# vLAR-group/unMORE

Measured on AMD Instinct MI355X. Metric: images/sec (train fwd+bwd) ObjectnessNet ViT-B/16 384x384, higher is better.
Workload: dtype bf16

## Files before the change

### include/umr.h

```cpp
#ifndef UMR_H
#define UMR_H
#include <stdint.h>

#ifdef __cplusplus
extern "C" {
#endif

typedef void* umr_stream_t;

enum umr_status { UMR_OK = 0, UMR_ERR_INVALID = -1, UMR_ERR_UNSUPPORTED = -2, UMR_ERR_HIP = -1000 };
enum umr_dtype { UMR_F32 = 0, UMR_BF16 = 1, UMR_BF16X3 = 2 };

int umr_version(void);
const char* umr_last_error_string(void);

enum umr_f32_mode { UMR_F32_EXACT = 0, UMR_F32_X3 = 1, UMR_F32_X3_FAST = 2 };
int umr_set_f32_mode(int mode);
int umr_get_f32_mode(void);

int umr_set_cu_budget(int cus);
int umr_get_cu_budget(void);

int umr_set_debug_option(const char* name, const char* value);
int umr_get_debug_option(const char* name, int* value, int* is_set);

enum umr_epi_flags {
    UMR_EPI_BIAS = 1, UMR_EPI_ADD_AUX = 2, UMR_EPI_MASK_RELU = 4, UMR_EPI_MASK_DGELU = 8,
    UMR_EPI_ADD_AUX2 = 16, UMR_EPI_OUT_F32 = 32, UMR_EPI_ROWBIAS = 64,
    UMR_EPI_OUT_X3 = 128,
    UMR_EPI_AUX_X3 = 256, UMR_EPI_AUX2_X3 = 512, UMR_EPI_C2_X3 = 1024
};
enum umr_act { UMR_ACT_NONE = 0, UMR_ACT_RELU = 1, UMR_ACT_GELU = 2, UMR_ACT_TANH = 3, UMR_ACT_SIGMOID = 5  };

typedef struct umr_gemm_desc {
    const void* A;
    const void* B;
    void* C;
    void* C2;
    const float* bias;
    const void* aux;
    const void* aux2;
    const float* rowbias;
    int64_t lda, ldb, ldc, ldc2, ldaux, ldaux2;
    int32_t M, N, K;
    int32_t dtype;
    int32_t flags, act, c2_mode, rows_per_batch;
    int32_t conv;
    int32_t nb, H, W, Cin, Ho, Wo;
    int32_t a_rows_in, a_rows_out, a_row_off;
    int32_t c_rows_in, c_rows_out, c_row_off;
    int32_t aux_mod;
    const float* red_w;
    float* red_out;
    int32_t red_c;
    int32_t no_store;
} umr_gemm_desc;

int umr_gemm_nt(const umr_gemm_desc* d, umr_stream_t stream);
int64_t umr_gemm_nt_workspace(void);
int umr_gemm_nt_splits(const umr_gemm_desc* d, int64_t workspace_bytes);
int64_t umr_gemm_nt_x3_workspace(const umr_gemm_desc* d);
int umr_gemm_nt_ws(const umr_gemm_desc* d, void* workspace, int64_t workspace_bytes, umr_stream_t stream);
int umr_gemm_nt_ws_status(void* workspace, umr_stream_t stream, int* bad_tickets);
int umr_split3(const float* src, void* dst, int64_t rows, int K, int64_t ld_src, int64_t ld_dst, umr_stream_t stream);
int umr_unsplit3(const void* src, float* dst, int64_t rows, int K, int64_t ld_src, int64_t ld_dst, umr_stream_t stream);
int umr_split3_rows(const float* src, void* dst, int64_t rows, int K, int64_t ld_src, int64_t ld_dst, int rows_in, int rows_out,
                    int row_off, umr_stream_t stream);
int umr_gemm_nt_rowreduce_ok(const umr_gemm_desc* d);

typedef struct umr_gemm_tn_desc {
    const void* dY;
    const void* X;
    float* dW;
    float* dbias;
    void* workspace;
    int64_t workspace_bytes;
    int64_t lddy, ldx, lddw;
    int32_t M, N, K;
    int32_t dtype;
    int32_t accumulate;
    int32_t conv, nb, H, W, Cin, Ho, Wo;
    int32_t dy_rows_in, dy_rows_out, dy_row_off;
    int32_t x_rows_in, x_rows_out, x_row_off;
} umr_gemm_tn_desc;

int64_t umr_gemm_tn_workspace(const umr_gemm_tn_desc* d);
int umr_gemm_tn(const umr_gemm_tn_desc* d, umr_stream_t stream);

int umr_layernorm_fwd(const void* x, const float* gamma, const float* beta, void* y, float* mean, float* rstd,
                      int M, int D, float eps, int dtype, umr_stream_t stream);
int64_t umr_layernorm_bwd_workspace(int M, int D);
int umr_layernorm_bwd(const void* dy, const void* x, const float* gamma, const float* mean, const float* rstd,
                      const void* dres, void* dx, float* dgamma, float* dbeta, int accumulate, void* workspace,
                      int64_t workspace_bytes, int M, int D, int dtype, umr_stream_t stream);
int umr_layernorm_bwd_rows(const void* dy, const void* x, const float* gamma, const float* mean, const float* rstd,
                           const void* dres, void* dx, void* workspace, int64_t workspace_bytes, int M, int D, int dtype,
                           umr_stream_t stream);
int umr_layernorm_bwd_params(const void* workspace, int64_t workspace_bytes, float* dgamma, float* dbeta, int accumulate,
                             int M, int D, umr_stream_t stream);

int64_t umr_attention_bwd_workspace(int B, int N, int heads);
int umr_attention_fwd(const void* qkv, void* out, float* lse, int B, int N, int heads, int head_dim, int dtype,
                      umr_stream_t stream);
int umr_attention_bwd(const void* qkv, const void* out, const void* dout, const float* lse, float* dsum_ws, void* dqkv,
                      int B, int N, int heads, int head_dim, int dtype, umr_stream_t stream);

int umr_patchify(const float* images, void* out, int B, int H, int W, int patch, int ldk, int dtype, umr_stream_t stream);
int umr_bilinear_fwd(const void* x, void* y, int B, int Hi, int Wi, int Ho, int Wo, int C, int align_corners, int dtype, umr_stream_t stream);
int umr_bilinear_bwd(const void* dy, void* dx, int B, int Hi, int Wi, int Ho, int Wo, int C, int align_corners, int dtype, umr_stream_t stream);
#define UMR_BILINEAR_RELU 1
#define UMR_BILINEAR_OUT_X3 2
int umr_bilinear_fwd_ex(const void* x, int64_t ldx, void* y, int64_t ldy, int B, int Hi, int Wi, int Ho, int Wo, int C, int align_corners,
                        int flags, int dtype, umr_stream_t stream);
int umr_bilinear_bwd_ex(const void* dy, int64_t lddy, void* dx, int64_t lddx, int B, int Hi, int Wi, int Ho, int Wo, int C,
                        int align_corners, int dtype, umr_stream_t stream);
int umr_pixel_shuffle(const void* src, void* dst, int B, int H, int W, int s, int C, int inverse, int dtype, umr_stream_t stream);
int umr_zero_stuff2(const void* dy, void* out, int B, int H, int W, int Ho, int Wo, int C, int dtype, umr_stream_t stream);
int umr_permute4(const void* src, void* dst, const int32_t* dst_dims, const int64_t* src_strides, int64_t src_offset,
                 int dtype_in, int dtype_out, int accumulate, umr_stream_t stream);
typedef struct umr_perm_entry {
    const void* src; void* dst; int32_t d[4]; int64_t sstride[4]; int64_t soff; int32_t dtype_in, dtype_out; int64_t blk_start;
    int32_t e[4]; int32_t ord[4];
    int64_t rowlen;
} umr_perm_entry;
int umr_permute4_batched(const umr_perm_entry* table_dev, int n, int64_t total_blocks, const int32_t* blk_entry_dev, umr_stream_t stream);
int umr_segsum(const void* x, void* out, int R, int reps, int64_t rep_stride, int64_t seg_stride, int C, int dtype_in,
               int out_f32, int accumulate, umr_stream_t stream);
int umr_fill_cls(void* tokens, const float* cls, const float* pos0, int B, int64_t batch_stride, int D, int dtype, umr_stream_t stream);
int umr_cast(const void* src, void* dst, int64_t n, float scale, int dtype_in, int dtype_out, umr_stream_t stream);
int umr_scale_by_device_scalar(const float* src, const float* scalar, float* dst, int64_t n, umr_stream_t stream);

int umr_head_out_fwd(const void* h, const float* w, const float* bias, float* out, int64_t M, int K, int Cout, int HW, int act,
                     int dtype, umr_stream_t stream);
int umr_head_out_finish(const float* partials, int nparts, const float* bias, float* out, int64_t M, int Cout, int HW, int act,
                        umr_stream_t stream);
int64_t umr_head_out_bwd_workspace(int64_t M, int K);
int umr_head_out_bwd(const void* h, const float* w, const float* dout, const float* yout, void* dh, float* dw, float* db,
                     void* workspace, int64_t workspace_bytes, int64_t M, int K, int Cout, int HW, int act, int relu_mask,
                     int dtype, umr_stream_t stream);

int64_t umr_loss_workspace(void);
int umr_objectness_loss(const float* pred_center, const float* pred_sdf, const float* gt_center, const float* gt_sdf,
                        const float* gt_saliency, float* d_center, float* d_sdf, float* out5, void* workspace, int B, int H,
                        int W, int center_l2, int sdf_l2, int use_grad, int use_bce, float grad_scale, umr_stream_t stream);

int umr_adam_step(float* p, const float* g, float* m, float* v, int64_t n, float lr, float beta1, float beta2, float eps,
                  int step, float grad_scale, umr_stream_t stream);
int umr_adam_set_hyper(float* hyper7_dev, float lr, float beta1, float beta2, float eps, int step, float grad_scale, umr_stream_t stream);
int umr_adam_step_hyper(float* p, const float* g, float* m, float* v, int64_t n, const float* hyper7_dev, umr_stream_t stream);
typedef struct umr_adam_pack_entry {
    float* p; const float* g; float* m; float* v; void* dst_lin; void* dst_t; int64_t n; int32_t N, K; int64_t blk_start;
} umr_adam_pack_entry;
int umr_adam_pack_step(const umr_adam_pack_entry* table_dev, int n_entries, int64_t total_blocks, const int32_t* blk_entry_dev,
                       const float* hyper7_dev, umr_stream_t stream);

int umr_crop_resize_bilinear(const float* image, const int32_t* boxes, float* out, int N, int H, int W, int S, umr_stream_t stream);
int umr_center_peaks(const float* sdf_maps, const float* center_fields, const double* filter50, double* score_out,
                     double* max_values, int64_t* argmax, int B, int H, int W, int border, int erode_kernel, int erode_rounds,
                     umr_stream_t stream);
int umr_center_peaks_certified(const float* sdf_maps, const float* center_fields, const double* filter50, double* max_values,
                               int64_t* argmax, int32_t* certified, int B, int H, int W, int border, int erode_kernel, int erode_rounds,
                               float eps, double singular_threshold, umr_stream_t stream);
int umr_boundary_deltas(const float* sdf_maps, float* deltas, int B, int H, int W, umr_stream_t stream);
int umr_mask_paste_stats(const float* sdf_maps, const float* center_fields, const int32_t* boxes, int N, int S, int H, int W,
                         int32_t* stats, float* maxima, umr_stream_t stream);
int umr_mask_paste(const float* sdf_maps, const float* center_fields, const int32_t* boxes, const int64_t* select, int K, int S, int H, int W,
                   uint8_t* masks, umr_stream_t stream);
int umr_rle_encode(const uint8_t* masks, int K, int H, int W, int64_t* sizes, const int64_t* offsets, uint8_t* chars, int64_t chars_capacity,
                   umr_stream_t stream);
int umr_mask_paste_rle(const float* sdf_maps, const float* center_fields, const int32_t* boxes, const int64_t* select, int K, int S, int H, int W,
                       int64_t* sizes, const int64_t* offsets, uint8_t* chars, int64_t chars_capacity, umr_stream_t stream);
int64_t umr_rle_decode_workspace(int K, int64_t total_chars, int64_t total_segments, int mode);
int umr_rle_decode(const uint8_t* chars, const int64_t* char_offsets, int K, int64_t total_chars, const int64_t* out_desc,
                   const int32_t* group_start, const int64_t* seg_offsets, int G, int64_t max_pixels, int64_t total_segments, uint8_t* out,
                   int64_t out_bytes, int value, int mode, int32_t* status, int32_t* info, void* workspace, int64_t workspace_bytes,
                   umr_stream_t stream);
int64_t umr_poly_rle_workspace(int64_t n_vertices, int n_polygons, int n_annotations, int64_t crossing_capacity);
int umr_poly_rle(const double* xy, const int64_t* poly_offsets, const int64_t* ann_polys, const int64_t* ann_sizes,
                 const int64_t* cross_offsets, int64_t n_vertices, int n_polygons, int n_annotations, int64_t crossing_capacity, int phases,
                 int64_t* sizes, const int64_t* offsets, uint8_t* chars, int64_t chars_capacity, void* workspace, int64_t workspace_bytes,
                 umr_stream_t stream);
int64_t umr_mask_iou_workspace(int K, int64_t total_chars, int64_t total_words);
int umr_mask_iou(const uint8_t* chars, const int64_t* char_offsets, int K, int64_t total_chars, const int64_t* unit_size,
                 const int32_t* unit_start, const int32_t* unit_nd, const int64_t* pair_offsets, const int64_t* word_offsets,
                 const uint8_t* crowd, int U, int64_t max_pixels, int max_d, int max_g, int64_t total_pairs, int64_t total_words,
                 int32_t* inter, double* iou, int32_t* area, int32_t* status, void* workspace, int64_t workspace_bytes,
                 umr_stream_t stream);
int umr_box_iou(const double* boxes, const int32_t* unit_start, const int32_t* unit_nd, const int64_t* pair_offsets, const uint8_t* crowd,
                int U, int K, int64_t max_pairs, int64_t total_pairs, double* iou, umr_stream_t stream);
int umr_coco_match(const double* iou, const int64_t* pair_offsets, int64_t total_pairs, const int32_t* unit_nd, const int32_t* unit_ng,
                   const int64_t* det_offsets, int64_t total_dets, const int64_t* gt_offsets, int64_t total_gts, const double* dt_area,
                   const double* gt_area, const uint8_t* gt_crowd, const double* area_rng, int A, const double* thr, int T, int max_det,
                   int U, uint8_t* dt_matched, int32_t* dt_gt, uint8_t* dt_ignore, uint8_t* gt_ignore, uint8_t* gt_matched,
                   umr_stream_t stream);
int umr_mask_components(const float* sdf_maps, const float* center_fields, int B, int S, int max_components, int32_t* counts, int32_t* boxes,
                        umr_stream_t stream);
int64_t umr_nms_workspace(int n);
int umr_nms(const float* boxes, const int64_t* order, int n, float iou_threshold, void* workspace, int64_t workspace_bytes,
            int64_t* keep, int32_t* n_keep, umr_stream_t stream);

int umr_linear_head_fwd(const void* x, const float* kw, const float* tapbias10, float* out, int B, int H, int W, int C, int act,
                        int dtype, umr_stream_t stream);
int umr_linear_head_bwd_data(const float* dout, const float* yout, const float* kw, void* dx, int B, int H, int W, int C, int act,
                             int accumulate, int dtype, umr_stream_t stream);
int64_t umr_linear_head_bwd_weight_workspace(int64_t M, int C);
int umr_linear_head_bwd_weight(const void* x, const float* dout, const float* yout, float* out, void* workspace,
                               int64_t workspace_bytes, int B, int H, int W, int C, int act, int dtype, umr_stream_t stream);
int64_t umr_linear_head_shift9_workspace(int64_t M);
int umr_linear_head_shift9(const float* dout, const float* yout, void* s9, float* nd, void* workspace, int64_t workspace_bytes,
                           int B, int H, int W, int act, int dtype, umr_stream_t stream);
int umr_linear_head_gather9(const float* taps, int64_t ldt, const float* tapbias10, float* out, int B, int H, int W, int act,
                            umr_stream_t stream);
int umr_small_gemm_f32(const float* A, const float* B, float* C, int M, int N, int K, int64_t sa_m, int64_t sa_k, int64_t sb_k,
                       int64_t sb_n, int64_t sc_m, int64_t sc_n, int accumulate, umr_stream_t stream);

int umr_im2col_nchw(const float* images, void* out, int B, int C, int H, int W, int KH, int KW, int stride, int pad, int ldk,
                    int dtype, umr_stream_t stream);
int umr_maxpool3x3s2(const void* x, void* y, int B, int H, int W, int C, int dtype, umr_stream_t stream);
int umr_bn_fold(const float* w, const float* gamma, const float* beta, const float* mean, const float* var, float eps, void* w_out,
                float* b_out, int Co, int K, int ldk, int dtype, umr_stream_t stream);

// ... 200 lines not shown
```

### unmore_amd/_lib.py

```python
import ctypes
import os
import re
import subprocess

_HERE = os.path.dirname(os.path.abspath(__file__))
HEADER = os.path.join(_HERE, "..", "include", "umr.h")
LIB_PATH = os.environ.get("UMR_LIB") or os.path.join(_HERE, "lib", "libumr.so")
CSRC = os.path.join(_HERE, "csrc")

F32, BF16, BF16X3 = 0, 1, 2
EPI_BIAS, EPI_ADD_AUX, EPI_MASK_RELU, EPI_MASK_DGELU, EPI_ADD_AUX2, EPI_OUT_F32, EPI_ROWBIAS, EPI_OUT_X3 = 1, 2, 4, 8, 16, 32, 64, 128
EPI_AUX_X3, EPI_AUX2_X3, EPI_C2_X3 = 256, 512, 1024
ACT_NONE, ACT_RELU, ACT_GELU, ACT_TANH = 0, 1, 2, 3
ACT_SIGMOID = 5
F32_EXACT, F32_X3, F32_X3_FAST = 0, 1, 2

_vp, _i32, _i64 = ctypes.c_void_p, ctypes.c_int32, ctypes.c_int64


class GemmDesc(ctypes.Structure):
    _fields_ = [("A", _vp), ("B", _vp), ("C", _vp), ("C2", _vp), ("bias", _vp), ("aux", _vp),
                ("aux2", _vp), ("rowbias", _vp),
                ("lda", _i64), ("ldb", _i64), ("ldc", _i64), ("ldc2", _i64), ("ldaux", _i64), ("ldaux2", _i64),
                ("M", _i32), ("N", _i32), ("K", _i32), ("dtype", _i32),
                ("flags", _i32), ("act", _i32), ("c2_mode", _i32), ("rows_per_batch", _i32),
                ("conv", _i32), ("nb", _i32), ("H", _i32), ("W", _i32), ("Cin", _i32), ("Ho", _i32), ("Wo", _i32),
                ("a_rows_in", _i32), ("a_rows_out", _i32), ("a_row_off", _i32),
                ("c_rows_in", _i32), ("c_rows_out", _i32), ("c_row_off", _i32), ("aux_mod", _i32),
                ("red_w", _vp), ("red_out", _vp), ("red_c", _i32), ("no_store", _i32)]


class GemmTnDesc(ctypes.Structure):
    _fields_ = [("dY", _vp), ("X", _vp), ("dW", _vp), ("dbias", _vp), ("workspace", _vp),
                ("workspace_bytes", _i64), ("lddy", _i64), ("ldx", _i64), ("lddw", _i64),
                ("M", _i32), ("N", _i32), ("K", _i32), ("dtype", _i32), ("accumulate", _i32),
                ("conv", _i32), ("nb", _i32), ("H", _i32), ("W", _i32), ("Cin", _i32), ("Ho", _i32), ("Wo", _i32),
                ("dy_rows_in", _i32), ("dy_rows_out", _i32), ("dy_row_off", _i32),
                ("x_rows_in", _i32), ("x_rows_out", _i32), ("x_row_off", _i32)]


class AdamPackEntry(ctypes.Structure):
    _fields_ = [("p", _vp), ("g", _vp), ("m", _vp), ("v", _vp), ("dst_lin", _vp), ("dst_t", _vp), ("n", _i64), ("N", _i32), ("K", _i32),
                ("blk_start", _i64)]


class BnBwdDesc(ctypes.Structure):
    _fields_ = [("dy", _vp), ("dpool", _vp), ("y", _vp), ("z", _vp * 2), ("mean", _vp * 2), ("rstd", _vp * 2), ("gamma", _vp * 2),
                ("dgamma", _vp * 2), ("dbeta", _vp * 2), ("dz", _vp * 2), ("g_out", _vp), ("workspace", _vp), ("workspace_bytes", _i64),
                ("rows_per_batch", _i64), ("pool_scale", ctypes.c_float), ("M", _i32), ("C", _i32), ("nbranch", _i32), ("dtype", _i32)]


class RaggedSrc(ctypes.Structure):
    _fields_ = [("f32", _vp), ("u8", _vp), ("H", _i32), ("W", _i32)]


class CpPair(ctypes.Structure):
    _fields_ = [("l_image", _vp), ("l_masks", _vp), ("l_boxes", _vp), ("u_image", _vp), ("u_masks", _vp), ("out_image", _vp), ("out_masks", _vp),
                ("word_off", _i64), ("inter_off", _i64), ("row_off", _i64), ("choice_off", _i64),
                ("Hl", _i32), ("Wl", _i32), ("Nl", _i32), ("Hu", _i32), ("Wu", _i32), ("Nu", _i32), ("nc", _i32), ("h_new", _i32), ("w_new", _i32),
                ("h_shift", _i32), ("w_shift", _i32), ("rh", ctypes.c_float), ("rw", ctypes.c_float), ("sx", ctypes.c_float), ("sy", ctypes.c_float),
                ("reserved", _i32)]


class MlImage(ctypes.Structure):
    _fields_ = [("masks", _vp), ("boxes", _vp), ("index", _vp), ("H", _i32), ("W", _i32), ("G", _i32), ("first", _i32), ("R", _i32),
                ("index64", _i32)]


class BlImage(ctypes.Structure):
    _fields_ = [("boxes", _vp), ("gt_boxes", _vp), ("gt_classes", _vp), ("gt_scores", _vp), ("first", _i32), ("R", _i32), ("G", _i32),
                ("chunk_first", _i32), ("height", ctypes.c_float), ("width", ctypes.c_float)]


class DpImage(ctypes.Structure):
    _fields_ = [("boxes", _vp), ("scores", _vp), ("mat_first", _i64), ("R", _i32), ("cand_first", _i32), ("out_first", _i32), ("cap", _i32),
                ("height", ctypes.c_float), ("width", ctypes.c_float)]


class PermEntry(ctypes.Structure):
    _fields_ = [("src", _vp), ("dst", _vp), ("d", _i32 * 4), ("sstride", _i64 * 4), ("soff", _i64), ("dtype_in", _i32), ("dtype_out", _i32),
                ("blk_start", _i64), ("e", _i32 * 4), ("ord", _i32 * 4), ("rowlen", _i64)]


MIRRORS = {"umr_gemm_desc": GemmDesc, "umr_gemm_tn_desc": GemmTnDesc, "umr_adam_pack_entry": AdamPackEntry, "umr_bn_bwd_desc": BnBwdDesc,
           "umr_ragged_src": RaggedSrc, "umr_cp_pair": CpPair, "umr_ml_image": MlImage, "umr_bl_image": BlImage, "umr_dp_image": DpImage,
           "umr_perm_entry": PermEntry}


def build(verbose=False, jobs=8):
    r = subprocess.run(["make", "-C", CSRC, f"-j{jobs}"], capture_output=True, text=True)
    if verbose or r.returncode != 0:
        print(r.stdout[-4000:])
        print(r.stderr[-8000:])
    if r.returncode != 0:
        raise RuntimeError("building libumr.so failed")
    return LIB_PATH


_lib = None
_count = [0]

_ARG = {"int": _i32, "int32_t": _i32, "int64_t": _i64, "float": ctypes.c_float, "double": ctypes.c_double, "umr_stream_t": _vp,
        "const char*": ctypes.c_char_p, "int*": ctypes.POINTER(ctypes.c_int)}
_RET = {"int": None, "int64_t": _i64, "const char*": ctypes.c_char_p}


def _ctype(decl, table, proto):
    c = re.sub(r"\s*\*\s*", "*", " ".join(decl.split()))
    if c not in table and not (table is _ARG and c.endswith("*")):
        raise RuntimeError(f"{HEADER}: no ctypes type for '{c}' in '{' '.join(proto.split())}'")
    return table.get(c, _vp)


def _read_header():
    if not os.path.exists(HEADER):
        raise RuntimeError(f"{HEADER} is missing: the ctypes binding of libumr.so is read from it")
    text = re.sub(r"/\*.*?\*/", " ", open(HEADER).read(), flags=re.S)
    text = re.sub(r"^[ \t]*#.*$", "", text, flags=re.M)
    text = re.sub(r"typedef\s+struct\s+\w+\s*\{.*?\}\s*\w+\s*;", "", text, flags=re.S)
    args, rets = {}, {}
    for proto in text.split(";"):
        if "(" not in proto:
            continue
        m = re.fullmatch(r"\s*(.*?)\b(umr_\w+)\s*\(([^()]*)\)\s*", proto, flags=re.S)
        if m is None:
            raise RuntimeError(f"{HEADER}: not a prototype this binding can read: '{' '.join(proto.split())}'")
        ret, name, params = m.groups()
        params = [] if params.strip() in ("", "void") else params.split(",")
        args[name] = [_ctype(re.sub(r"\w+\s*$", "", p), _ARG, proto) for p in params]
        rets[name] = _ctype(ret, _RET, proto)
    return args, {name: r for name, r in rets.items() if r is not None}


ARGTYPES, RESTYPES = _read_header()


def exported_symbols():
    return sorted(ARGTYPES)


def lib():
    global _lib
    if _lib is None:
        if not os.path.exists(LIB_PATH):
            raise RuntimeError(
                f"{LIB_PATH} is missing: build it with `python -c 'import __graft_entry__ as g; g.build()'` "
                "(the product has no CPU fallback)")
        _lib = ctypes.CDLL(LIB_PATH)
        for name, argtypes in ARGTYPES.items():
            fn = getattr(_lib, name)
            fn.argtypes = argtypes
            if name in RESTYPES:
                fn.restype = RESTYPES[name]
    return _lib


def check(status, what):
    _count[0] += 1
    if status != 0:
        raise RuntimeError(f"{what} failed with status {status}: {lib().umr_last_error_string().decode()}")
```

### unmore_amd/csrc/gemm_nt.hip

```cpp
#include "umr_common.h"
#include <type_traits>
#include "gemm_epilogue.h"
#include <stdlib.h>

namespace {

constexpr int BM = 128, BN = 128;
constexpr int UMR_SPLITK_COUNTERS = 4096;
constexpr int ROWB = 128;
constexpr int TILE_BYTES = BM * ROWB;
constexpr int STAGE_BYTES = 2 * TILE_BYTES;
constexpr int LDS_BYTES = 2 * STAGE_BYTES;

template <typename T> struct Tr;
template <> struct Tr<bf16_t> { static constexpr int EPC = 8, BK = 64; };
template <> struct Tr<float> { static constexpr int EPC = 4, BK = 32; };


template <typename T> struct Raw8;
template <> struct Raw8<bf16_t> {
    typedef bf16x8 type;
    static __device__ __forceinline__ type load(const bf16_t* q) { return *(const bf16x8*)q; }
    static __device__ __forceinline__ void cvt(type t, f32x4& a, f32x4& b) {
        a = f32x4{(float)t[0], (float)t[1], (float)t[2], (float)t[3]};
// ... 259 lines not shown
            const int old = __hip_atomic_fetch_add(counters + tile_id, 1, __ATOMIC_RELAXED, __HIP_MEMORY_SCOPE_AGENT);
            const bool bad = old < 0 || old >= splits;
            if (bad) {
                __hip_atomic_fetch_add(counters + (UMR_SPLITK_COUNTERS - 1), 1, __ATOMIC_RELAXED, __HIP_MEMORY_SCOPE_AGENT);
                __hip_atomic_store(counters + tile_id, 0, __ATOMIC_RELAXED, __HIP_MEMORY_SCOPE_AGENT);
            }
            if (fenced) {
                __builtin_amdgcn_fence(__ATOMIC_ACQUIRE, "agent");
                asm volatile("s_waitcnt vmcnt(0)" ::: "memory");
            } else {
                __builtin_amdgcn_fence(__ATOMIC_ACQUIRE, "workgroup");
            }
            const int last = !bad && old == splits - 1;
            if (last) __hip_atomic_store(counters + tile_id, 0, __ATOMIC_RELAXED, __HIP_MEMORY_SCOPE_AGENT);
            *(int*)smem = last;
        }
        __syncthreads();
        if (*(const int*)smem == 0) return;
        const unsigned long long* base = slabs + (int64_t)tile_id * splits * SLAB + tid * 2;
        auto ld4 = [&](const unsigned long long* q) {
            const f32x2 lo = __builtin_bit_cast(f32x2, __hip_atomic_load(q, __ATOMIC_RELAXED, __HIP_MEMORY_SCOPE_AGENT));
            const f32x2 hi = __builtin_bit_cast(f32x2, __hip_atomic_load(q + 1, __ATOMIC_RELAXED, __HIP_MEMORY_SCOPE_AGENT));
            return f32x4{lo[0], lo[1], hi[0], hi[1]};
        };
#pragma unroll
        for (int r = 0; r < 16; ++r) acc[r >> 2][r & 3] = ld4(base + r * 512);
        for (int q = 1; q < splits; ++q) {
            const unsigned long long* bq = base + (int64_t)q * SLAB;
            f32x4 v[16];
#pragma unroll
            for (int r = 0; r < 16; ++r) v[r] = ld4(bq + r * 512);
#pragma unroll
            for (int r = 0; r < 16; ++r) acc[r >> 2][r & 3] += v[r];
        }
    }

    constexpr int EP_LD = 132;
    float* stg = (float*)smem;
    auto stage_pass = [&](auto ptag) {
        constexpr int PASS = decltype(ptag)::value;
#pragma unroll
        for (int mh = 0; mh < 2; ++mh) {
            const int lr = wr * 32 + mh * 16 + frow;
#pragma unroll
            for (int ntl = 0; ntl < 4; ++ntl)
                *(f32x4*)(stg + lr * EP_LD + wc * 64 + ntl * 16 + fq * 4) = acc[PASS * 2 + mh][ntl];
        }
    };
    if constexpr (EPI == 0) {
        const int c8 = (tid & 15) * 8, n = n0 + c8;
        const bool n_ok = n < p.N;
        const bool use_aux = (p.flags & (UMR_EPI_ADD_AUX | UMR_EPI_MASK_RELU | UMR_EPI_MASK_DGELU)) != 0;
        const bool use_aux2 = (p.flags & UMR_EPI_ADD_AUX2) != 0;
        f32x4 bias0 = {0.f, 0.f, 0.f, 0.f}, bias1 = {0.f, 0.f, 0.f, 0.f};
        if ((p.flags & UMR_EPI_BIAS) && n_ok) { bias0 = *(const f32x4*)(p.bias + n); bias1 = *(const f32x4*)(p.bias + n + 4); }
        typename Raw8<T>::type ra[8], rb2[8];
        auto row_of = [&](int pass, int k) { const int lr = (tid >> 4) + k * 16; return m0 + (lr >> 5) * 64 + pass * 32 + (lr & 31); };
        auto prefetch = [&](auto ptag) {
            constexpr int PASS = decltype(ptag)::value;
#pragma unroll
            for (int k = 0; k < 4; ++k) {
                const int m = row_of(PASS, k);
                if (m < p.M && n_ok) {
                    if (use_aux) ra[PASS * 4 + k] = Raw8<T>::load((const T*)p.aux + (int64_t)m * p.ldaux + n);
                    if (use_aux2) rb2[PASS * 4 + k] = Raw8<T>::load((const T*)p.aux2 + (int64_t)m * p.ldaux2 + n);
                }
            }
        };
        auto pass = [&](auto ptag) {
            constexpr int PASS = decltype(ptag)::value;
            __syncthreads();
            stage_pass(ptag);
            __syncthreads();
#pragma unroll
            for (int k = 0; k < 4; ++k) {
                const int lr = (tid >> 4) + k * 16;
                const int m = row_of(PASS, k);
                if (m >= p.M || !n_ok) continue;
                f32x4 v0 = *(const f32x4*)(stg + lr * EP_LD + c8), v1 = *(const f32x4*)(stg + lr * EP_LD + c8 + 4);
                v0 += bias0; v1 += bias1;
                if (use_aux) {
                    f32x4 a0, a1;
                    Raw8<T>::cvt(ra[PASS * 4 + k], a0, a1);
                    if (p.flags & UMR_EPI_ADD_AUX) { v0 += a0; v1 += a1; }
                    else if (p.flags & UMR_EPI_MASK_RELU) {
#pragma unroll
                        for (int e = 0; e < 4; ++e) { v0[e] = a0[e] > 0.f ? v0[e] : 0.f; v1[e] = a1[e] > 0.f ? v1[e] : 0.f; }
                    } else if constexpr (sizeof(T) == 2) {
#pragma unroll
                        for (int e = 0; e < 4; ++e) { v0[e] *= dgelu_sel<T>(a0[e]); v1[e] *= dgelu_sel<T>(a1[e]); }
                    }
                }
                if (use_aux2) {
                    f32x4 a0, a1;
                    Raw8<T>::cvt(rb2[PASS * 4 + k], a0, a1);
                    v0 += a0; v1 += a1;
                }
                if (p.c2_mode == 2) Vec8<T>::store((T*)p.C2 + (int64_t)m * p.ldc2 + n, v0, v1);
                if (p.act == UMR_ACT_RELU) {
#pragma unroll
                    for (int e = 0; e < 4; ++e) { v0[e] = fmaxf(v0[e], 0.f); v1[e] = fmaxf(v1[e], 0.f); }
                } else if (p.act == UMR_ACT_GELU) {
                    if constexpr (sizeof(T) == 2) {
#pragma unroll
                        for (int e = 0; e < 4; ++e) { v0[e] = gelu_sel<T>(v0[e]); v1[e] = gelu_sel<T>(v1[e]); }
                    }
                }
                Vec8<T>::store((T*)p.C + (int64_t)m * p.ldc + n, v0, v1);
                if (p.c2_mode == 1) {
#pragma unroll
                    for (int e = 0; e < 4; ++e) { v0[e] = fmaxf(v0[e], 0.f); v1[e] = fmaxf(v1[e], 0.f); }
                    Vec8<T>::store((T*)p.C2 + (int64_t)m * p.ldc2 + n, v0, v1);
                }
            }
        };
        prefetch(std::integral_constant<int, 0>{});
        if constexpr (sizeof(T) == 2) prefetch(std::integral_constant<int, 1>{});
        pass(std::integral_constant<int, 0>{});
        if constexpr (sizeof(T) != 2) prefetch(std::integral_constant<int, 1>{});
        pass(std::integral_constant<int, 1>{});
    } else {
        const bool vec_ok = ((p.N & 7) == 0) && ((p.ldc & 7) == 0) && ((p.ldc2 & 7) == 0) && ((p.ldaux & 7) == 0) &&
                            ((p.ldaux2 & 7) == 0);
#pragma unroll 1
        for (int pass = 0; pass < 2; ++pass) {
            __syncthreads();
            if (pass == 0) stage_pass(std::integral_constant<int, 0>{});
            else stage_pass(std::integral_constant<int, 1>{});
            __syncthreads();
#pragma unroll 1
            for (int task = tid; task < 64 * 16; task += 256) {
                const int lr = task >> 4, c8 = (task & 15) * 8;
                const int trow = (lr >> 5) * 64 + pass * 32 + (lr & 31);
                const int m = m0 + trow, n = n0 + c8;
                if (m >= p.M || n >= p.N) continue;
                const f32x4 v0 = *(const f32x4*)(stg + lr * EP_LD + c8), v1 = *(const f32x4*)(stg + lr * EP_LD + c8 + 4);
                if (vec_ok) {
                    epilogue_store8<T>(p, m, n, v0, v1);
                } else {
                    epilogue_store<T>(p, m, n, v0);
                    if (n + 4 < p.N) epilogue_store<T>(p, m, n + 4, v1);
                }
            }
        }
    }
}

}

int umr_launch_gemm_nt256(const umr_gemm_desc* d, hipStream_t s);
int umr_launch_gemm_nt256p(const umr_gemm_desc* d, hipStream_t s);
int umr_launch_gemm_nt256p_ws(const umr_gemm_desc* d, void* ws, int64_t ws_bytes, hipStream_t s);
bool umr_nt256_rowreduce_path(const umr_gemm_desc* d);

static int tile_override() {
    return umr_opt_or(UMR_OPT_GEMM_TILE, 0);
}

static bool uses_256(const umr_gemm_desc* d) {
    if (d->dtype != UMR_BF16) return false;
    const int64_t t256 = (int64_t)((d->M + 255) / 256) * ((d->N + 255) / 256);
    const int ov = tile_override();
    const bool kfit = d->conv == 0 ? (d->K % 64 == 0) : (d->Cin % 64 == 0);
    constexpr int min_tiles = 300;
    constexpr int conv_min_tiles = 512;
    const bool big = kfit && d->N >= 192 &&
                     (t256 >= 2048 || (d->conv == 1 && t256 >= conv_min_tiles) || (d->conv == 0 && d->a_rows_in <= 0 && t256 >= min_tiles && (d->K >= 512 || t256 >= 1024)));
    return kfit && (ov == 256 || (ov == 0 && big));
}

extern "C" int umr_gemm_nt_rowreduce_ok(const umr_gemm_desc* d) {
    if (d == nullptr || d->M <= 0 || d->N <= 0 || d->K <= 0) return 0;
    return (uses_256(d) && umr_nt256_rowreduce_path(d)) ? 1 : 0;
}

static int gemm_nt_impl(const umr_gemm_desc* d, void* workspace, int64_t workspace_bytes, umr_stream_t stream);

extern "C" int umr_gemm_nt(const umr_gemm_desc* d, umr_stream_t stream) { return gemm_nt_impl(d, nullptr, 0, stream); }

extern "C" int umr_gemm_nt_ws_status(void* workspace, umr_stream_t stream, int* bad_tickets) {
    UMR_CHECK_ARG(workspace != nullptr && bad_tickets != nullptr, "gemm_nt_ws_status: null argument");
    hipStream_t s = (hipStream_t)stream;
    int* word = (int*)workspace + (UMR_SPLITK_COUNTERS - 1);
    int v = 0;
    hipError_t e_ = hipMemcpyAsync(&v, word, sizeof(int), hipMemcpyDeviceToHost, s);
    if (e_ == hipSuccess) e_ = hipStreamSynchronize(s);
    if (e_ == hipSuccess && v != 0) e_ = hipMemsetAsync(word, 0, sizeof(int), s);
    if (e_ != hipSuccess) return umr_set_error(UMR_ERR_HIP - (int)e_, hipGetErrorString(e_));
    *bad_tickets = v;
    return UMR_OK;
}

extern "C" int64_t umr_gemm_nt_workspace(void) { return (int64_t)UMR_SPLITK_COUNTERS * 4 + (int64_t)512 * BM * BN * 4; }

static int pick_splits(const umr_gemm_desc* d, int64_t tiles, bool have_ws);
static bool uses_256(const umr_gemm_desc* d);
int umr_x3_ksplit_of(const umr_gemm_desc* d, int64_t ws_bytes);

extern "C" int umr_gemm_nt_splits(const umr_gemm_desc* d, int64_t workspace_bytes) {
    if (d == nullptr || d->M <= 0 || d->N <= 0 || d->K <= 0 || workspace_bytes <= 0) return 1;
    if (d->dtype == UMR_BF16X3) return umr_x3_ksplit_of(d, workspace_bytes - (int64_t)UMR_SPLITK_COUNTERS * 4);
    if (d->dtype != UMR_BF16 && d->dtype != UMR_F32) return 1;
    if (uses_256(d)) return 1;
    return pick_splits(d, (int64_t)((d->M + BM - 1) / BM) * ((d->N + BN - 1) / BN), true);
}

extern "C" int umr_gemm_nt_ws(const umr_gemm_desc* d, void* workspace, int64_t workspace_bytes, umr_stream_t stream) {
    UMR_CHECK_ARG(workspace == nullptr || (workspace_bytes >= umr_gemm_nt_workspace() && ((uintptr_t)workspace & 15) == 0),
                  "gemm_nt_ws: workspace smaller than umr_gemm_nt_workspace() or not 16-byte aligned");
    return gemm_nt_impl(d, workspace, workspace_bytes, stream);
}

static int pick_splits(const umr_gemm_desc* d, int64_t tiles, bool have_ws) {
    if (!have_ws || tiles > UMR_SPLITK_COUNTERS) return 1;
    const int bk = d->dtype == UMR_BF16 ? 64 : 32;
    const int nt = d->conv == 0 ? (d->K + bk - 1) / bk : 9 * ((d->Cin + bk - 1) / bk);
    int want;
    const int forced = umr_opt(UMR_OPT_NT_SPLITK);
    if (forced != UMR_OPT_UNSET) {
        want = forced;
    } else {
        if (tiles > 170) return 1;
        if (d->dtype == UMR_BF16) {
            want = tiles <= 32 ? (nt / 8 < 4 ? nt / 8 : 4) : (nt >= 32 ? 2 : 1);
        } else {
            want = (int)(448 / tiles);
            const int per_min = tiles <= 32 ? 8 : 16;
            if (want > nt / per_min) want = nt / per_min;
            if (want > 8) want = 8;
        }
    }
    if (want > nt) want = nt;
    if (want < 2 || tiles * want > 512) return 1;
    const int per = (nt + want - 1) / want;
    return (nt + per - 1) / per;
}

template <typename T, int CV, int EPI, bool X3>
static void launch_nt(dim3 g, hipStream_t s, const umr_gemm_desc* d, int tiles_n, int splits, float* skws) {
    const int splits_arg = (splits > 1 && umr_opt_or(UMR_OPT_SPLITK_FENCE, 0) != 0) ? -splits : splits;
    hipLaunchKernelGGL((gemm_nt_kernel<T, CV, EPI, X3>), g, dim3(256), LDS_BYTES, s, *d, tiles_n, splits_arg, skws);
}

static int gemm_nt_impl(const umr_gemm_desc* d, void* workspace, int64_t workspace_bytes, umr_stream_t stream) {
    UMR_CHECK_ARG(d != nullptr, "gemm_nt: null descriptor");
    UMR_CHECK_ARG(d->A && d->B && (d->C || d->no_store), "gemm_nt: null operand");
    UMR_CHECK_ARG(d->M > 0 && d->N > 0 && d->K > 0, "gemm_nt: empty problem");
    if (d->dtype == UMR_BF16X3) {
        UMR_CHECK_ARG(d->conv == 0 || d->conv == 1, "gemm_nt (BF16X3): plain GEMM or stride-1 3x3 conv only");
        const int fl = d->flags;
        const bool out_f32 = (fl & UMR_EPI_OUT_F32) != 0, out_x3 = (fl & UMR_EPI_OUT_X3) != 0;
        const int kk = d->conv == 0 ? d->K : d->Cin;
        const bool red = d->red_w != nullptr;
        const int n_aux = ((fl & UMR_EPI_ADD_AUX) != 0) + ((fl & UMR_EPI_MASK_RELU) != 0) + ((fl & UMR_EPI_MASK_DGELU) != 0);
        auto ld_ok = [&](int64_t ld, bool planes) { return planes ? (ld % 8 == 0 && ld >= 3 * (int64_t)d->N) : (ld % 4 == 0 && ld >= d->N); };
        bool ok = (kk % 64 == 0) && (d->N % 8 == 0) && d->a_rows_in <= 0 && (d->ldb % 8 == 0) && (d->ldb >= 3 * (int64_t)d->K) &&
                  (d->act == UMR_ACT_NONE || d->act == UMR_ACT_RELU || d->act == UMR_ACT_GELU) && n_aux <= 1 &&
                  (!(fl & UMR_EPI_MASK_DGELU) || (d->act == UMR_ACT_NONE && d->c2_mode == 0 && !(fl & UMR_EPI_ADD_AUX2))) &&
                  (d->conv == 1 ? (d->K == 9 * d->Cin && (int64_t)d->nb * d->Ho * d->Wo == d->M && d->Ho == d->H && d->Wo == d->W && d->c_rows_in <= 0)
                                : (d->lda % 8 == 0 && d->lda >= 3 * (int64_t)d->K));
        if (red) {
            ok = ok && d->no_store && !out_f32 && !out_x3 && d->conv == 0 && d->red_out && (d->red_c == 1 || d->red_c == 2) && d->c2_mode == 0 &&
                 !(fl & ~UMR_EPI_BIAS) && d->act != UMR_ACT_GELU && d->c_rows_in <= 0 && d->aux_mod <= 0;
        } else {
            ok = ok && !d->no_store && d->C && (out_f32 != out_x3) && ld_ok(d->ldc, out_x3) &&
                 (d->c2_mode == 0 || ((d->c2_mode == 1 || d->c2_mode == 2) && d->C2 && ld_ok(d->ldc2, (fl & UMR_EPI_C2_X3) != 0))) &&
                 (n_aux == 0 || (d->aux && ld_ok(d->ldaux, (fl & UMR_EPI_AUX_X3) != 0))) &&
                 (!(fl & UMR_EPI_ADD_AUX2) || (d->aux2 && ld_ok(d->ldaux2, (fl & UMR_EPI_AUX2_X3) != 0))) &&
                 (!(fl & UMR_EPI_ROWBIAS) || (d->rowbias && d->rows_per_batch > 0)) && (d->aux_mod <= 0 || n_aux == 1);
        }
        if (!ok) return umr_set_error(UMR_ERR_UNSUPPORTED, "gemm_nt (BF16X3): needs K (conv: Cin) % 64 == 0, N % 8 == 0, no A-row remap, act in {none, ReLU, GELU}, "
                                                           "exactly one of OUT_F32 / OUT_X3 (or red_w with no_store and a bias / ReLU epilogue), strides that "
                                                           "fit the operand formats (include/umr.h)");
        UMR_CHECK_ARG(!(fl & UMR_EPI_BIAS) || d->bias, "gemm_nt: bias flag without pointer");
        UMR_CHECK_ARG((int64_t)((d->M + 191) / 192) * ((d->N + 255) / 256) * 32 < (1ll << 31), "gemm_nt: grid too large");
        char* xws = workspace ? (char*)workspace + (int64_t)UMR_SPLITK_COUNTERS * 4 : nullptr;
        const int64_t xws_bytes = workspace ? workspace_bytes - (int64_t)UMR_SPLITK_COUNTERS * 4 : 0;
        return umr_launch_gemm_nt256p_ws(d, xws, xws_bytes, (hipStream_t)stream);
    }
    UMR_CHECK_ARG(d->dtype == UMR_F32 || d->dtype == UMR_BF16, "gemm_nt: dtype");
    const int epc = d->dtype == UMR_BF16 ? 8 : 4;
    UMR_CHECK_ARG(d->conv >= 0 && d->conv <= 2, "gemm_nt: conv mode");
    if (d->conv == 0) {
        UMR_CHECK_ARG(d->K % epc == 0 && d->lda % epc == 0 && d->ldb % epc == 0, "gemm_nt: K/lda/ldb must be multiples of 16 bytes");
    } else {
        UMR_CHECK_ARG(d->Cin % epc == 0 && d->K == 9 * d->Cin && d->ldb % epc == 0, "gemm_nt: conv needs Cin % 16B == 0 and K == 9*Cin");
        UMR_CHECK_ARG((int64_t)d->nb * d->Ho * d->Wo == d->M, "gemm_nt: conv M != nb*Ho*Wo");
        const int s = d->conv == 2 ? 2 : 1;
        UMR_CHECK_ARG(d->Ho == (d->H - 1) / s + 1 && d->Wo == (d->W - 1) / s + 1, "gemm_nt: conv output size");
    }
    UMR_CHECK_ARG(!(d->flags & UMR_EPI_BIAS) || d->bias, "gemm_nt: bias flag without pointer");
    UMR_CHECK_ARG(!(d->flags & (UMR_EPI_ADD_AUX | UMR_EPI_MASK_RELU | UMR_EPI_MASK_DGELU)) || d->aux, "gemm_nt: aux flag without pointer");
    UMR_CHECK_ARG(!(d->flags & UMR_EPI_ADD_AUX2) || d->aux2, "gemm_nt: aux2 flag without pointer");
    UMR_CHECK_ARG(!(d->flags & UMR_EPI_ROWBIAS) || (d->rowbias && d->rows_per_batch > 0), "gemm_nt: rowbias");
    UMR_CHECK_ARG(d->c2_mode == 0 || d->C2, "gemm_nt: c2_mode without C2");
    const int tiles_m = (d->M + BM - 1) / BM, tiles_n = (d->N + BN - 1) / BN;
    int tiles_n_arg = tiles_n;
    const int64_t grid = (int64_t)tiles_m * tiles_n;
    UMR_CHECK_ARG(grid < (1ll << 31), "gemm_nt: grid too large");
    hipStream_t s = (hipStream_t)stream;
    if (d->red_w || d->no_store) {
        UMR_CHECK_ARG(umr_gemm_nt_rowreduce_ok(d) == 1, "gemm_nt: fused row reduction / no_store requested on a path that does not implement it (umr_gemm_nt_rowreduce_ok)");
        UMR_CHECK_ARG(!d->red_w || (d->red_out && (d->red_c == 1 || d->red_c == 2)), "gemm_nt: red_out / red_c");
    }
    if (uses_256(d)) return umr_launch_gemm_nt256(d, s);
    const int splits = pick_splits(d, grid, workspace != nullptr);
    float* skws = (float*)workspace;
    {
        const int oe = umr_opt(UMR_OPT_NT_ORDER);
        const bool mfast = oe != UMR_OPT_UNSET ? (oe == 'm') : (d->conv == 0 && d->a_rows_in <= 0 && (int64_t)d->N > (int64_t)d->M);
        if (mfast) tiles_n_arg = -tiles_m;
    }
    dim3 g((unsigned)(grid * splits)), b(256);
    const bool fast_ep = ((d->N & 7) == 0) && ((d->ldc & 7) == 0) && (d->c2_mode == 0 || (d->ldc2 & 7) == 0) &&
                         (!(d->flags & (UMR_EPI_ADD_AUX | UMR_EPI_MASK_RELU | UMR_EPI_MASK_DGELU)) || (d->ldaux & 7) == 0) &&
                         (!(d->flags & UMR_EPI_ADD_AUX2) || (d->ldaux2 & 7) == 0) && d->c_rows_in <= 0 && d->aux_mod <= 0 &&
                         !(d->flags & (UMR_EPI_ROWBIAS | UMR_EPI_OUT_F32)) &&
                         (!(d->flags & UMR_EPI_MASK_DGELU) || d->dtype == UMR_BF16) &&
                         (d->act == UMR_ACT_NONE || d->act == UMR_ACT_RELU || (d->act == UMR_ACT_GELU && d->dtype == UMR_BF16));
#define LAUNCH(T, CV)                                                                   \
    do {                                                                                \
        if (fast_ep) launch_nt<T, CV, 0, false>(g, s, d, tiles_n_arg, splits, skws);  \
        else launch_nt<T, CV, 1, false>(g, s, d, tiles_n_arg, splits, skws);          \
    } while (0)
#define LAUNCH_X3(CV)                                                                      \
    do {                                                                                   \
        if (fast_ep) launch_nt<float, CV, 0, true>(g, s, d, tiles_n_arg, splits, skws);  \
        else launch_nt<float, CV, 1, true>(g, s, d, tiles_n_arg, splits, skws);          \
    } while (0)
    const int f32_x3 = umr_f32_mode_now() != UMR_F32_EXACT;
    if (d->dtype == UMR_BF16) {
        if (d->conv == 0) LAUNCH(bf16_t, 0); else if (d->conv == 1) LAUNCH(bf16_t, 1); else LAUNCH(bf16_t, 2);
    } else if (f32_x3 && !((d->conv == 0 ? d->K : d->Cin) % 32)) {
        if (d->conv == 0) LAUNCH_X3(0); else if (d->conv == 1) LAUNCH_X3(1); else LAUNCH_X3(2);
    } else {
        if (d->conv == 0) LAUNCH(float, 0); else if (d->conv == 1) LAUNCH(float, 1); else LAUNCH(float, 2);
    }
#undef LAUNCH_X3
#undef LAUNCH
    {
        const hipError_t e_ = hipGetLastError();
        if (e_ != hipSuccess) {
            if (splits > 1) (void)hipMemsetAsync(workspace, 0, (size_t)UMR_SPLITK_COUNTERS * 4, s);
            return umr_set_error(UMR_ERR_HIP - (int)e_, hipGetErrorString(e_));
        }
    }
    return UMR_OK;
}
```

### unmore_amd/csrc/gemm_nt256.hip

```cpp
#include "umr_common.h"
#include "gemm_epilogue.h"
#include <stdlib.h>
#include <type_traits>

namespace {

constexpr int BM2 = 256, BN2 = 256, BK2 = 64;
constexpr int ROWB2 = 128;
constexpr int TILE2 = 256 * ROWB2;
constexpr int BUF2 = 2 * TILE2;
constexpr int LDS2 = 2 * BUF2;

typedef bf16_t T2;

template <int CONV>
__global__ __launch_bounds__(512, 2) void gemm_nt256_kernel(const umr_gemm_desc p, int tiles_n) {
    extern __shared__ __attribute__((aligned(16))) char smem[];
    constexpr int SZ = 2;
    constexpr unsigned OOB = 0x80000000u;
    const int tid = threadIdx.x, lane = tid & 63;
    const int w = __builtin_amdgcn_readfirstlane(tid >> 6);

    int bid = blockIdx.x;
    {
// ... 102 lines not shown
    auto stage_issue = [&](auto gtag, auto itag) {
        constexpr int G = decltype(gtag)::value, I = decltype(itag)::value;
        unsigned v = (G == 0) ? a_eff[0][I] : (G == 3) ? a_eff[1][I] : vo[G][I];
        if (st_tile >= nt) v = OOB;
        char* dst = smem + (st_tile & 1) * BUF2;
        if (G == 0 || G == 3) __builtin_amdgcn_raw_ptr_buffer_load_lds(rsA, UMR_LDS_PTR(dst + lds_row[G][I] * ROWB2), 16, v, soffA, 0, 0);
        else __builtin_amdgcn_raw_ptr_buffer_load_lds(rsB, UMR_LDS_PTR(dst + TILE2 + lds_row[G][I] * ROWB2), 16, v, soffB, 0, 0);
        if (G == 3 && I == 1) ++st_tile;
    };
#define STAGE_DMA(G, I) stage_issue(std::integral_constant<int, G>{}, std::integral_constant<int, I>{})

    f32x4 acc[8][4];
#pragma unroll
    for (int i = 0; i < 8; ++i)
#pragma unroll
        for (int j = 0; j < 4; ++j) acc[i][j] = f32x4{0.f, 0.f, 0.f, 0.f};

    const int wr = w >> 2, wc = w & 3;
    const int frow = lane & 15, fq = lane >> 4;
    int a_ad[2], b_ad[2];
#pragma unroll
    for (int ks = 0; ks < 2; ++ks) {
        const int q = ks * 4 + fq;
        const int sw = (frow >> 1) & 7;
        a_ad[ks] = (wr * 128 + frow) * ROWB2 + ((q ^ sw) << 4);
        b_ad[ks] = TILE2 + (wc * 64 + frow) * ROWB2 + ((q ^ sw) << 4);
    }
#define A_FRAG(ks, i) (*(const bf16x8*)(sbuf + a_ad[ks] + (i) * 16 * ROWB2))
#define B_FRAG(ks, i) (*(const bf16x8*)(sbuf + b_ad[ks] + (i) * 16 * ROWB2))

    bf16x8 fa[2][4], fb0[2][2], fb1[2][2];

#define PHASE_SYNC()                                               \
    asm volatile("s_waitcnt vmcnt(6)" ::: "memory");               \
    __builtin_amdgcn_s_barrier();                                  \
    asm volatile("s_waitcnt lgkmcnt(0)" ::: "memory");             \
    __builtin_amdgcn_sched_barrier(0);
#define MFMA(ACC, BF, AF) ACC = __builtin_amdgcn_mfma_f32_16x16x32_bf16(BF, AF, ACC, 0, 0, 0)
#define QUADRANT(M0, N0, FB, G)                                                                     \
    __builtin_amdgcn_s_setprio(1);                                                                  \
    MFMA(acc[M0 + 0][N0 + 0], FB[0][0], fa[0][0]); MFMA(acc[M0 + 0][N0 + 1], FB[0][1], fa[0][0]);   \
    MFMA(acc[M0 + 1][N0 + 0], FB[0][0], fa[0][1]); MFMA(acc[M0 + 1][N0 + 1], FB[0][1], fa[0][1]);   \
    __builtin_amdgcn_sched_barrier(0);                                                              \
    STAGE_DMA(G, 0);                                                                                \
    __builtin_amdgcn_sched_barrier(0);                                                              \
    MFMA(acc[M0 + 2][N0 + 0], FB[0][0], fa[0][2]); MFMA(acc[M0 + 2][N0 + 1], FB[0][1], fa[0][2]);   \
    MFMA(acc[M0 + 3][N0 + 0], FB[0][0], fa[0][3]); MFMA(acc[M0 + 3][N0 + 1], FB[0][1], fa[0][3]);   \
    MFMA(acc[M0 + 0][N0 + 0], FB[1][0], fa[1][0]); MFMA(acc[M0 + 0][N0 + 1], FB[1][1], fa[1][0]);   \
    __builtin_amdgcn_sched_barrier(0);                                                              \
    STAGE_DMA(G, 1);                                                                                \
    __builtin_amdgcn_sched_barrier(0);                                                              \
    MFMA(acc[M0 + 1][N0 + 0], FB[1][0], fa[1][1]); MFMA(acc[M0 + 1][N0 + 1], FB[1][1], fa[1][1]);   \
    MFMA(acc[M0 + 2][N0 + 0], FB[1][0], fa[1][2]); MFMA(acc[M0 + 2][N0 + 1], FB[1][1], fa[1][2]);   \
    MFMA(acc[M0 + 3][N0 + 0], FB[1][0], fa[1][3]); MFMA(acc[M0 + 3][N0 + 1], FB[1][1], fa[1][3]);   \
    __builtin_amdgcn_s_setprio(0);

    auto tile_body = [&](const char* sbuf) {
#pragma unroll
        for (int ks = 0; ks < 2; ++ks) {
#pragma unroll
            for (int i = 0; i < 2; ++i) fb0[ks][i] = B_FRAG(ks, i);
#pragma unroll
            for (int i = 0; i < 4; ++i) fa[ks][i] = A_FRAG(ks, i);
        }
        PHASE_SYNC();
        QUADRANT(0, 0, fb0, 2)
#pragma unroll
        for (int ks = 0; ks < 2; ++ks)
#pragma unroll
            for (int i = 0; i < 2; ++i) fb1[ks][i] = B_FRAG(ks, 2 + i);
        PHASE_SYNC();
        QUADRANT(0, 2, fb1, 3)
        stage_prep();
#pragma unroll
        for (int ks = 0; ks < 2; ++ks)
#pragma unroll
            for (int i = 0; i < 4; ++i) fa[ks][i] = A_FRAG(ks, 4 + i);
        PHASE_SYNC();
        QUADRANT(4, 2, fb1, 0)
        PHASE_SYNC();
        QUADRANT(4, 0, fb0, 1)
    };

    stage_prep();
    STAGE_DMA(0, 0); STAGE_DMA(0, 1); STAGE_DMA(1, 0); STAGE_DMA(1, 1);
    STAGE_DMA(2, 0); STAGE_DMA(2, 1); STAGE_DMA(3, 0); STAGE_DMA(3, 1);
    stage_prep();
    STAGE_DMA(0, 0); STAGE_DMA(0, 1); STAGE_DMA(1, 0); STAGE_DMA(1, 1);
    asm volatile("s_waitcnt vmcnt(8)" ::: "memory");
    __builtin_amdgcn_s_barrier();

#pragma unroll 1
    for (int t = 0; t < nt; ++t) tile_body(smem + (t & 1) * BUF2);
#undef QUADRANT
#undef MFMA
#undef PHASE_SYNC
#undef STAGE_DMA
#undef A_FRAG
#undef B_FRAG

    asm volatile("s_waitcnt vmcnt(0)" ::: "memory");
    constexpr int EP_LD = 260;
    float* stg = (float*)smem;
    const bool vec_ok = ((p.N & 7) == 0) && ((p.ldc & 7) == 0) && ((p.ldc2 & 7) == 0) && ((p.ldaux & 7) == 0) &&
                        ((p.ldaux2 & 7) == 0);
    auto stage_pass = [&](auto ptag) {
        constexpr int PASS = decltype(ptag)::value;
#pragma unroll
        for (int mh = 0; mh < 2; ++mh) {
            const int lr = wr * 32 + mh * 16 + frow;
#pragma unroll
            for (int ntl = 0; ntl < 4; ++ntl)
                *(f32x4*)(stg + lr * EP_LD + wc * 64 + ntl * 16 + fq * 4) = acc[PASS * 2 + mh][ntl];
        }
    };
#pragma unroll 1
    for (int pass = 0; pass < 4; ++pass) {
        __syncthreads();
        switch (pass) {
            case 0: stage_pass(std::integral_constant<int, 0>{}); break;
            case 1: stage_pass(std::integral_constant<int, 1>{}); break;
            case 2: stage_pass(std::integral_constant<int, 2>{}); break;
            default: stage_pass(std::integral_constant<int, 3>{}); break;
        }
        __syncthreads();
#pragma unroll 1
        for (int task = tid; task < 64 * 32; task += 512) {
            const int lr = task >> 5, c8 = (task & 31) * 8;
            const int trow = (lr >> 5) * 128 + pass * 32 + (lr & 31);
            const int m = m0 + trow, n = n0 + c8;
            if (m >= p.M || n >= p.N) continue;
            const f32x4 v0 = *(const f32x4*)(stg + lr * EP_LD + c8), v1 = *(const f32x4*)(stg + lr * EP_LD + c8 + 4);
            if (vec_ok) {
                epilogue_store8<T2>(p, m, n, v0, v1);
            } else {
                epilogue_store<T2>(p, m, n, v0);
                if (n + 4 < p.N) epilogue_store<T2>(p, m, n + 4, v1);
            }
        }
    }
}

}

int umr_launch_gemm_nt256p(const umr_gemm_desc* d, hipStream_t s);
bool umr_nt256p_fast_epilogue(const umr_gemm_desc* d);
bool umr_nt256p_plain_epilogue(const umr_gemm_desc* d);

bool umr_nt256_rowreduce_path(const umr_gemm_desc* d) {
    if (umr_opt_or(UMR_OPT_NT256_PERSIST, 1) == 0) return false;
    return ((d->conv == 0 && d->a_rows_in <= 0) || d->conv == 1) && umr_nt256p_plain_epilogue(d);
}

int umr_launch_gemm_nt256(const umr_gemm_desc* d, hipStream_t s) {
    {
        const int persist = umr_opt_or(UMR_OPT_NT256_PERSIST, 1);
        if (persist && ((d->conv == 0 && d->a_rows_in <= 0) || d->conv == 1)) return umr_launch_gemm_nt256p(d, s);
    }
    if (d->red_w || d->no_store) return umr_set_error(UMR_ERR_UNSUPPORTED, "gemm_nt: fused row reduction / no_store is only implemented by the persistent 256x256 path");
    const int tiles_m = (d->M + BM2 - 1) / BM2, tiles_n = (d->N + BN2 - 1) / BN2;
    const int64_t grid = (int64_t)tiles_m * tiles_n;
    dim3 g((unsigned)grid), b(512);
#define L256(CV)                                                                                                       \
    do {                                                                                                               \
        UMR_SET_MAX_LDS_ONCE((gemm_nt256_kernel<CV>), LDS2); \
        hipLaunchKernelGGL((gemm_nt256_kernel<CV>), g, b, LDS2, s, *d, tiles_n);                                        \
    } while (0)
    if (d->conv == 0) L256(0);
    else if (d->conv == 1) L256(1);
    else L256(2);
#undef L256
    UMR_LAUNCH_CHECK();
    return UMR_OK;
}
```

### unmore_amd/csrc/gemm_nt256p.hip

```cpp
#include "umr_common.h"
#include "gemm_epilogue.h"
#include <stdio.h>
#include <stdlib.h>
#include <type_traits>

namespace {

constexpr int BM2 = 256, BN2 = 256, BK2 = 64;
constexpr int ROWB2 = 128;
constexpr int TILE2 = 256 * ROWB2;
constexpr int BUF2 = 2 * TILE2;
constexpr int STG_OFF = 2 * BUF2;
constexpr int STG_BYTES = 32 * 256 * 4;
constexpr int LDS2P = STG_OFF + STG_BYTES;

typedef bf16_t T2;

__device__ __forceinline__ unsigned mul_dgelu_bf16x2(unsigned g, unsigned x) {
    const float lo = __builtin_bit_cast(float, g << 16) * dgelu_sel<bf16_t>(__builtin_bit_cast(float, x << 16));
    const float hi = __builtin_bit_cast(float, g & 0xFFFF0000u) * dgelu_sel<bf16_t>(__builtin_bit_cast(float, x & 0xFFFF0000u));
    typedef __attribute__((ext_vector_type(2))) __bf16 bf16x2;
    bf16x2 r;
    r[0] = (bf16_t)lo; r[1] = (bf16_t)hi;
    return __builtin_bit_cast(unsigned, r);
}

__device__ __forceinline__ unsigned add_bf16x2(unsigned x, unsigned y) {
    const float lo = __builtin_bit_cast(float, x << 16) + __builtin_bit_cast(float, y << 16);
    const float hi = __builtin_bit_cast(float, x & 0xFFFF0000u) + __builtin_bit_cast(float, y & 0xFFFF0000u);
    typedef __attribute__((ext_vector_type(2))) __bf16 bf16x2;
    bf16x2 r;
    r[0] = (bf16_t)lo; r[1] = (bf16_t)hi;
    return __builtin_bit_cast(unsigned, r);
}

__device__ __forceinline__ unsigned pos_mask_bf16x2(unsigned a) {
    typedef __attribute__((ext_vector_type(2))) short s16x2;
    const s16x2 one = {1, 1}, zero = {0, 0};
    s16x2 v = __builtin_bit_cast(s16x2, a);
    v = __builtin_elementwise_min(v, one);
    v = __builtin_elementwise_max(v, zero);
    v = zero - v;
    return __builtin_bit_cast(unsigned, v);
}

template <int CONV, int EPI, int AUXM, bool RED, bool X3 = false, bool P2 = true>
__global__ __launch_bounds__(512, 2) void gemm_nt256p_kernel(const umr_gemm_desc p, int tiles_n, int total_tiles, int stagger, int bm, int npairs = 6,
                                                             int kt_per_arg = 0) {
    const int sp = (X3 && kt_per_arg > 0) ? (int)blockIdx.y : 0;
    static_assert(X3 == (EPI == 5 || EPI == 6), "the plane-pair K loop and the f32 / plane epilogues (EPI 5, 6) go together");
    constexpr bool PH2 = P2;
    static_assert(CONV == 0 || P2, "the conv is instantiated in its two-phase form only");
    extern __shared__ __attribute__((aligned(16))) char smem[];
    constexpr int SZ = 2;
    constexpr unsigned OOB = 0x80000000u;
    const int tid = threadIdx.x, lane = tid & 63;
    const int w = __builtin_amdgcn_readfirstlane(tid >> 6);
    const bool ahead = (stagger != 0) && (w < 4);

    const int G = gridDim.x;
    const int pw = ((G & 7) == 0) ? (int)(blockIdx.x & 7) * (G >> 3) + (int)(blockIdx.x >> 3) : (int)blockIdx.x;
    if (pw >= total_tiles) return;
    const int n_my = (total_tiles - pw + G - 1) / G;

    const int lrow = lane >> 3, lchk = lane & 7;
    const int hw = (CONV != 0) ? p.Ho * p.Wo : 1;
    const int apix = X3 ? 3 * p.Cin : p.Cin;
    unsigned vo[4][2];
    int trow_a[2][2];
    unsigned a_tapmask[2][2];
    unsigned a_eff[2][2];
    int lds_row[4][2];
#pragma unroll
    for (int gi = 0; gi < 2; ++gi) {
#pragma unroll
        for (int i = 0; i < 2; ++i) {
            const int lr = (w * 2 + i) * 8 + lrow;
            {
                const int trow = (lr >> 6) * 128 + gi * 64 + (lr & 63);
                const int g = gi == 0 ? 0 : 3;
                lds_row[g][i] = (((w * 2 + i) * 8) >> 6) * 128 + gi * 64 + (((w * 2 + i) * 8) & 63);
                const int gch = lchk ^ ((trow >> 1) & 7);
                trow_a[gi][i] = trow;
                vo[g][i] = (CONV == 0) ? (unsigned)(((int64_t)trow * p.lda) * SZ + gch * 16)
                                       : (unsigned)((int64_t)trow * apix * SZ + gch * 16);
                a_eff[gi][i] = vo[g][i];
                a_tapmask[gi][i] = 0x1FFu;
            }
            {
                const int trow = (lr >> 5) * 64 + gi * 32 + (lr & 31);
                const int g = 1 + gi;
                lds_row[g][i] = (((w * 2 + i) * 8) >> 5) * 64 + gi * 32 + (((w * 2 + i) * 8) & 31);
                const int gch = lchk ^ ((trow >> 1) & 7);
                vo[g][i] = (unsigned)(((int64_t)trow * p.ldb) * SZ + gch * 16);
            }
        }
    }

    const int ktiles_per_tap = (CONV == 0) ? 0 : p.Cin / BK2;
    const int kt_total = (CONV == 0) ? p.K / BK2 : 9 * ktiles_per_tap;
    const int kb = sp * kt_per_arg;
    const int kt_mine = (X3 && kt_per_arg > 0) ? ((kt_total - kb < kt_per_arg) ? kt_total - kb : kt_per_arg) : kt_total;
    const int nt = kt_mine * (X3 ? npairs : 1);

    __amdgpu_buffer_rsrc_t rsA, rsB;
    int s_it = 0;
    int st_tile = 0, st_tap = 0, st_ci = 0, st_par = 0;
    int st_pp = 0, st_k = 0;
    unsigned soffA = 0, soffB = 0;
    auto clamp31 = [](int64_t v) -> int { return v > 0x7FFFFFFFll ? 0x7FFFFFFF : (v < 0 ? 0 : (int)v); };
    auto stage_setup = [&](int it) {
        const bool live = it < n_my;
        const int v = live ? it * G + pw : 0;
        const int tm = v / tiles_n, tn = v - tm * tiles_n;
        const int m0 = tm * bm, n0 = tn * BN2;
        st_tile = 0; st_pp = 0; st_k = kb;
        st_ci = (CONV == 0) ? 0 : kb / 9; st_tap = (CONV == 0) ? 0 : kb - st_ci * 9;
        rsB = __builtin_amdgcn_make_buffer_rsrc((void*)((const char*)p.B + (int64_t)n0 * p.ldb * SZ), 0,
                                                live ? clamp31((int64_t)(p.N - n0) * p.ldb * SZ) : 0, 0x00020000);
        if (CONV == 0) {
            rsA = __builtin_amdgcn_make_buffer_rsrc((void*)((const char*)p.A + (int64_t)m0 * p.lda * SZ), 0,
                                                    live ? clamp31((int64_t)((p.M - m0 < bm) ? (p.M - m0) : bm) * p.lda * SZ) : 0, 0x00020000);
        } else {
            rsA = __builtin_amdgcn_make_buffer_rsrc((void*)((const char*)p.A + ((int64_t)m0 - (p.W + 1)) * apix * SZ), 0,
                                                    live ? 0x7FFFFFFF : 0, 0x00020000);
#pragma unroll
            for (int gi = 0; gi < 2; ++gi)
#pragma unroll
                for (int i = 0; i < 2; ++i) {
                    const int m = m0 + trow_a[gi][i];
                    const int rem = m % hw;
                    const int oy = rem / p.Wo, ox = rem - oy * p.Wo;
                    unsigned mask = 0;
#pragma unroll
                    for (int tap = 0; tap < 9; ++tap) {
                        const int iy = oy - 1 + tap / 3, ix = ox - 1 + tap % 3;
                        if ((unsigned)iy < (unsigned)p.H && (unsigned)ix < (unsigned)p.W) mask |= 1u << tap;
                    }
                    a_tapmask[gi][i] = (live && m < p.M) ? mask : 0u;
                }
        }
    };
    auto stage_prep = [&]() {
        if (st_tile == nt) {
            ++s_it;
            stage_setup(s_it);
        }
        const int pa = X3 ? (((npairs == 6 ? 0x940 : 0x010) >> (2 * st_pp)) & 3) : 0;
        const int pb = X3 ? (((npairs == 6 ? 0x124 : 0x004) >> (2 * st_pp)) & 3) : 0;
        const bool next_k = !X3 || st_pp == npairs - 1;
        if (X3) st_pp = next_k ? 0 : st_pp + 1;
        if (CONV == 0) {
            const int kt = X3 ? st_k : st_tile;
            soffA = (unsigned)((kt * BK2 + pa * p.K) * SZ);
// ... 149 lines not shown
        PHASE_SYNC();
        QUADRANT_HI(2, fb1, 0)
        PHASE_SYNC();
        QUADRANT_HI(0, fb0, 1)
    };

#define READ_WAIT()                                                \
    asm volatile("s_waitcnt lgkmcnt(0)" ::: "memory");             \
    __builtin_amdgcn_sched_barrier(0);
#define END_SYNC_N(N)                                              \
    asm volatile("s_waitcnt vmcnt(" #N ")" ::: "memory");          \
    __builtin_amdgcn_s_barrier();                                  \
    __builtin_amdgcn_sched_barrier(0);
    auto tile_body2_ahead = [&](const char* sbuf) {
        stage_prep();
#pragma unroll
        for (int ks = 0; ks < 2; ++ks) {
#pragma unroll
            for (int i = 0; i < 2; ++i) fb0[ks][i] = B_FRAG(ks, i);
#pragma unroll
            for (int i = 0; i < 4; ++i) fa[ks][i] = A_FRAG(ks, i);
#pragma unroll
            for (int i = 0; i < 2; ++i) fb1[ks][i] = B_FRAG(ks, 2 + i);
        }
        READ_WAIT();
        QUADRANT_D(0, 0, fb0, STAGE_DMA(0, 0); STAGE_DMA(0, 1), STAGE_DMA(1, 0); STAGE_DMA(1, 1))
        QUADRANT_D(0, 2, fb1, STAGE_DMA(2, 0), STAGE_DMA(2, 1))
        END_SYNC_N(6);
#pragma unroll
        for (int ks = 0; ks < 2; ++ks)
#pragma unroll
            for (int i = 0; i < 4; ++i) fa[ks][i] = A_FRAG(ks, 4 + i);
        READ_WAIT();
        QUADRANT_HID(2, fb1, STAGE_DMA(3, 0), STAGE_DMA(3, 1))
        QUADRANT_HID(0, fb0, (void)0, (void)0)
        END_SYNC_N(2);
    };
    auto tile_body4_ahead = [&](const char* sbuf) {
#pragma unroll
        for (int ks = 0; ks < 2; ++ks) {
#pragma unroll
            for (int i = 0; i < 2; ++i) fb0[ks][i] = B_FRAG(ks, i);
#pragma unroll
            for (int i = 0; i < 4; ++i) fa[ks][i] = A_FRAG(ks, i);
        }
        READ_WAIT();
        QUADRANT(0, 0, fb0, 1)
        END_SYNC_N(6);
#pragma unroll
        for (int ks = 0; ks < 2; ++ks)
#pragma unroll
            for (int i = 0; i < 2; ++i) fb1[ks][i] = B_FRAG(ks, 2 + i);
        READ_WAIT();
        QUADRANT(0, 2, fb1, 2)
        END_SYNC_N(6);
#pragma unroll
        for (int ks = 0; ks < 2; ++ks)
#pragma unroll
            for (int i = 0; i < 4; ++i) fa[ks][i] = A_FRAG(ks, 4 + i);
        READ_WAIT();
        QUADRANT(4, 2, fb1, 3)
        END_SYNC_N(6);
        stage_prep();
        QUADRANT(4, 0, fb0, 0)
        END_SYNC_N(6);
    };

    if (PRIO_MODE == 1 && w >= 4) __builtin_amdgcn_s_setprio(1);
    stage_setup(0);
    stage_prep();
    STAGE_DMA(0, 0); STAGE_DMA(0, 1); STAGE_DMA(1, 0); STAGE_DMA(1, 1);
    STAGE_DMA(2, 0); STAGE_DMA(2, 1); STAGE_DMA(3, 0); STAGE_DMA(3, 1);
    if (ahead) {
        if (PH2) {
            asm volatile("s_waitcnt vmcnt(2)" ::: "memory");
        } else {
            stage_prep();
            STAGE_DMA(0, 0); STAGE_DMA(0, 1);
            asm volatile("s_waitcnt vmcnt(6)" ::: "memory");
        }
    } else {
        stage_prep();
        STAGE_DMA(0, 0); STAGE_DMA(0, 1); STAGE_DMA(1, 0); STAGE_DMA(1, 1);
        if (PH2) { STAGE_DMA(2, 0); STAGE_DMA(2, 1); }
        asm volatile("s_waitcnt vmcnt(8)" ::: "memory");
    }
    __builtin_amdgcn_s_barrier();

    const int er = lane >> 3, ec = lane & 7;
    const unsigned co_lane = ((unsigned)((w >> 2) * 128 + er) * (unsigned)p.ldc + (unsigned)((w & 3) * 64 + ec * 8)) * 2u;
    const unsigned ax_lane = ((unsigned)((w >> 2) * 128 + er) * (unsigned)p.ldaux + (unsigned)((w & 3) * 64 + ec * 8)) * 2u;
    constexpr int WST_BYTES = 2048;
    constexpr int RW_OFF = 8 * WST_BYTES;
    float* stg = (float*)(smem + STG_OFF);
    auto stage_rows = [&](auto mtag) {
        constexpr int MT = decltype(mtag)::value;
        const int lr = wr * 16 + frow;
#pragma unroll
        for (int ntl = 0; ntl < 4; ++ntl) {
            const int ch = (wc * 16 + ntl * 4 + fq) ^ frow;
            *(f32x4*)(stg + lr * 256 + ch * 4) = acc[MT][ntl];
        }
    };
    int c_par = 0;
    constexpr bool BIAS_INIT = (EPI == 3 || EPI == 4 || EPI == 5 || EPI == 6);
    f32x4 bqn[4];
    auto fetch_bias = [&](int it_) {
        const int v_ = it_ * G + pw;
        const int tn_ = v_ - (v_ / tiles_n) * tiles_n;
#pragma unroll
        for (int ntl = 0; ntl < 4; ++ntl) {
            const int n = tn_ * BN2 + wc * 64 + ntl * 16 + fq * 4;
            bqn[ntl] = f32x4{0.f, 0.f, 0.f, 0.f};
            if ((p.flags & UMR_EPI_BIAS) && it_ < n_my && n < p.N) bqn[ntl] = *(const f32x4*)(p.bias + n);
        }
    };
    if (BIAS_INIT) fetch_bias(0);
#pragma unroll 1
    for (int it = 0; it < n_my; ++it) {
#pragma unroll
        for (int i = 0; i < 8; ++i)
#pragma unroll
            for (int j = 0; j < 4; ++j) acc[i][j] = BIAS_INIT ? bqn[j] : f32x4{0.f, 0.f, 0.f, 0.f};
        if (RED && w < 2) {
            const int v_ = it * G + pw;
            const int n0_ = (v_ - (v_ / tiles_n) * tiles_n) * BN2;
            const __amdgpu_buffer_rsrc_t rsW = __builtin_amdgcn_make_buffer_rsrc(
                (void*)(p.red_w + (int64_t)w * p.N + n0_), 0, (w < p.red_c) ? clamp31((int64_t)(p.N - n0_) * 4) : 0, 0x00020000);
            const int rw_off = (EPI == 3) ? RW_OFF + (it & 1) * 2048 : 0;
            __builtin_amdgcn_raw_ptr_buffer_load_lds(rsW, UMR_LDS_PTR(smem + STG_OFF + rw_off + w * 1024), 16, (unsigned)(lane * 16), 0, 0, 0);
        }
        if (ahead) {
#pragma unroll 1
            for (int t = 0; t < nt; ++t) {
                if (PH2) tile_body2_ahead(smem + c_par * BUF2); else tile_body4_ahead(smem + c_par * BUF2);
                c_par ^= 1;
            }
        } else {
#pragma unroll 1
            for (int t = 0; t < nt; ++t) {
                tile_body(smem + c_par * BUF2);
                c_par ^= 1;
            }
        }
        const int v = it * G + pw;
        const int tm = v / tiles_n, tn = v - tm * tiles_n;
        const int m0 = tm * bm, n0 = tn * BN2;
        const int m_end = (p.M - m0 < bm) ? p.M : m0 + bm;
        if (EPI == 3) {
            fetch_bias(it + 1);
            typedef __attribute__((ext_vector_type(2))) short s16x2;
            typedef __attribute__((ext_vector_type(2))) unsigned u32x2;
            const short relu_lo = (p.act == UMR_ACT_RELU) ? (short)0 : (short)-32768;
            const s16x2 relu16 = {relu_lo, relu_lo};
            auto pack4 = [&](const f32x4& v) -> u32x2 {
                unsigned lo, hi;
                asm("v_cvt_pk_bf16_f32 %0, %1, %2" : "=v"(lo) : "v"(v[0]), "v"(v[1]));
                asm("v_cvt_pk_bf16_f32 %0, %1, %2" : "=v"(hi) : "v"(v[2]), "v"(v[3]));
                s16x2 a = __builtin_bit_cast(s16x2, lo), b = __builtin_bit_cast(s16x2, hi);
                if (AUXM == 0) {
                    a = __builtin_elementwise_max(a, relu16);
                    b = __builtin_elementwise_max(b, relu16);
                }
                return u32x2{__builtin_bit_cast(unsigned, a), __builtin_bit_cast(unsigned, b)};
            };
            bf16x8 rwh[2], rwl[2];
            float* ro_lane = nullptr;
            if (RED) {
#pragma unroll
                for (int pr = 0; pr < 2; ++pr) {
                    f32x4 a = {0.f, 0.f, 0.f, 0.f}, b = {0.f, 0.f, 0.f, 0.f};
                    if (frow < 2) {
                        const char* rwp = smem + STG_OFF + RW_OFF + (it & 1) * 2048 + frow * 1024;
                        a = *(const f32x4*)(rwp + (wc * 64 + (2 * pr) * 16 + fq * 4) * 4);
                        b = *(const f32x4*)(rwp + (wc * 64 + (2 * pr + 1) * 16 + fq * 4) * 4);
                    }
#pragma unroll
                    for (int e = 0; e < 8; ++e) {
                        const float x = e < 4 ? a[e] : b[e - 4];
                        const bf16_t hi = (bf16_t)x;
                        rwh[pr][e] = hi;
                        rwl[pr][e] = (bf16_t)(x - (float)hi);
                    }
                }
                if (fq == 0 && n0 + wc * 64 < p.N)
                    ro_lane = p.red_out + ((int64_t)(tn * 4 + wc) * p.M + (m0 + wr * 128 + frow)) * p.red_c;
            }
            auto row_reduce2 = [&](const bf16x8& a01, const bf16x8& a23, const bf16x8& b01, const bf16x8& b23, int mt_) {
                const f32x4 z = {0.f, 0.f, 0.f, 0.f};
                f32x4 ra = __builtin_amdgcn_mfma_f32_16x16x32_bf16(rwh[0], a01, z, 0, 0, 0);
                f32x4 rb = __builtin_amdgcn_mfma_f32_16x16x32_bf16(rwh[0], b01, z, 0, 0, 0);
                ra = __builtin_amdgcn_mfma_f32_16x16x32_bf16(rwl[0], a01, ra, 0, 0, 0);
                rb = __builtin_amdgcn_mfma_f32_16x16x32_bf16(rwl[0], b01, rb, 0, 0, 0);
                ra = __builtin_amdgcn_mfma_f32_16x16x32_bf16(rwh[1], a23, ra, 0, 0, 0);
                rb = __builtin_amdgcn_mfma_f32_16x16x32_bf16(rwh[1], b23, rb, 0, 0, 0);
                ra = __builtin_amdgcn_mfma_f32_16x16x32_bf16(rwl[1], a23, ra, 0, 0, 0);
                rb = __builtin_amdgcn_mfma_f32_16x16x32_bf16(rwl[1], b23, rb, 0, 0, 0);
                const int m = m0 + wr * 128 + mt_ * 16 + frow;
                if (ro_lane != nullptr) {
                    float* ro = ro_lane + (int64_t)(mt_ * 16) * p.red_c;
                    if (p.red_c == 2) {
                        if (m < m_end) *(f32x2*)ro = f32x2{ra[0], ra[1]};
                        if (m + 16 < m_end) *(f32x2*)(ro + 32) = f32x2{rb[0], rb[1]};
                    } else {
                        if (m < m_end) ro[0] = ra[0];
                        if (m + 16 < m_end) ro[16] = rb[0];
                    }
                }
            };
            const bool col_live = n0 + wc * 64 + ec * 8 < p.N;
            const __amdgpu_buffer_rsrc_t rsC = __builtin_amdgcn_make_buffer_rsrc(
                (void*)((T2*)p.C + (int64_t)m0 * p.ldc + n0), 0, p.no_store ? 0 : clamp31((int64_t)(m_end - m0) * p.ldc * 2), 0x00020000);
            const unsigned co_vo = col_live ? co_lane : OOB;
            __amdgpu_buffer_rsrc_t rsX = rsC;
            unsigned ax_vo = OOB;
            if (AUXM != 0) {
                rsX = __builtin_amdgcn_make_buffer_rsrc((void*)((T2*)p.aux + (int64_t)m0 * p.ldaux + n0), 0,
                                                        clamp31((int64_t)(m_end - m0) * p.ldaux * 2), 0x00020000);
                ax_vo = col_live ? ax_lane : OOB;
            }
            u32x4 axc[4][2];
            auto load_auxc = [&](auto btag) {
                constexpr int MB = decltype(btag)::value;
                if (MB < 8 && AUXM != 0) {
#pragma unroll
                    for (int k = 0; k < 2; ++k)
                        axc[MB & 3][k] = __builtin_amdgcn_raw_buffer_load_b128(rsX, ax_vo + (unsigned)((MB * 16 + k * 8) * p.ldaux * 2), 0, 0);
                }
            };
            load_auxc(std::integral_constant<int, 0>{});
            load_auxc(std::integral_constant<int, 1>{});
            char* wst = smem + STG_OFF + w * WST_BYTES;
            const int wsw = (frow >> 1) & 7;
            char* wst_w = wst + frow * 128 + (fq & 1) * 8;
            const char* wst_r0 = wst + er * 128 + ((ec ^ ((er >> 1) & 7)) << 4);
            const char* wst_r1 = wst + (er + 8) * 128 + ((ec ^ (((er >> 1) + 4) & 7)) << 4);
            auto blocks2 = [&](auto btag) {
                constexpr int MB = decltype(btag)::value;
                load_auxc(std::integral_constant<int, MB + 2>{});
                load_auxc(std::integral_constant<int, MB + 3>{});
                u32x2 pk[2][4];
#pragma unroll
                for (int mh = 0; mh < 2; ++mh)
#pragma unroll
                    for (int ntl = 0; ntl < 4; ++ntl) pk[mh][ntl] = pack4(acc[MB + mh][ntl]);
                if (RED) {
                    bf16x8 tq[2][2];
#pragma unroll
                    for (int mh = 0; mh < 2; ++mh)
#pragma unroll
                        for (int h = 0; h < 2; ++h)
                            tq[mh][h] = __builtin_bit_cast(bf16x8, u32x4{pk[mh][2 * h][0], pk[mh][2 * h][1], pk[mh][2 * h + 1][0], pk[mh][2 * h + 1][1]});
                    row_reduce2(tq[0][0], tq[0][1], tq[1][0], tq[1][1], MB);
                }
#pragma unroll
                for (int mh = 0; mh < 2; ++mh) {
#pragma unroll
                    for (int ntl = 0; ntl < 4; ++ntl) *(u32x2*)(wst_w + (((ntl * 2 + (fq >> 1)) ^ wsw) << 4)) = pk[mh][ntl];
                    asm volatile("" ::: "memory");
                    u32x4 o[2];
                    o[0] = *(const u32x4*)wst_r0;
                    o[1] = *(const u32x4*)wst_r1;
                    asm volatile("" ::: "memory");
#pragma unroll
                    for (int k = 0; k < 2; ++k) {
                        if (AUXM == 2) {
                            const u32x4 a = axc[(MB + mh) & 3][k];
#pragma unroll
                            for (int e = 0; e < 4; ++e) o[k][e] &= pos_mask_bf16x2(a[e]);
                        }
                        if (AUXM == 1) {
                            const u32x4 a = axc[(MB + mh) & 3][k];
#pragma unroll
                            for (int e = 0; e < 4; ++e) o[k][e] = add_bf16x2(o[k][e], a[e]);
                        }
                        const unsigned so = (unsigned)(((MB + mh) * 16 + k * 8) * p.ldc * 2);
                        __builtin_amdgcn_raw_buffer_store_b128(o[k], rsC, co_vo + so, 0, 0);
                    }
                }
            };
            if (RED && p.no_store) {
#pragma unroll
                for (int mt = 0; mt < 8; mt += 2) {
                    bf16x8 tq[2][2];
#pragma unroll
                    for (int mh = 0; mh < 2; ++mh)
#pragma unroll
                        for (int ntl = 0; ntl < 4; ++ntl) {
                            const bf16x4 t = __builtin_bit_cast(bf16x4, pack4(acc[mt + mh][ntl]));
#pragma unroll
                            for (int e = 0; e < 4; ++e) tq[mh][ntl >> 1][(ntl & 1) * 4 + e] = t[e];
                        }
                    row_reduce2(tq[0][0], tq[0][1], tq[1][0], tq[1][1], mt);
                }
            } else {
                blocks2(std::integral_constant<int, 0>{}); blocks2(std::integral_constant<int, 2>{});
                blocks2(std::integral_constant<int, 4>{}); blocks2(std::integral_constant<int, 6>{});
            }
        } else if (EPI == 4) {
            fetch_bias(it + 1);
            constexpr bool dgelu = (AUXM == 2);
            const bool two_out = !dgelu && p.c2_mode == 2;
            typedef __attribute__((ext_vector_type(2))) unsigned u32x2;
            const bool col_live = n0 + wc * 64 + ec * 8 < p.N;
            const __amdgpu_buffer_rsrc_t rsC = __builtin_amdgcn_make_buffer_rsrc(
                (void*)((T2*)p.C + (int64_t)m0 * p.ldc + n0), 0, clamp31((int64_t)(m_end - m0) * p.ldc * 2), 0x00020000);
            const unsigned co_vo = col_live ? co_lane : OOB;
            __amdgpu_buffer_rsrc_t rsC2 = rsC, rsX = rsC;
            unsigned c2_vo = OOB, ax_vo = OOB;
            if (two_out) {
                rsC2 = __builtin_amdgcn_make_buffer_rsrc((void*)((T2*)p.C2 + (int64_t)m0 * p.ldc2 + n0), 0,
                                                         clamp31((int64_t)(m_end - m0) * p.ldc2 * 2), 0x00020000);
                c2_vo = col_live ? ((unsigned)(wr * 128 + er) * (unsigned)p.ldc2 + (unsigned)(wc * 64 + ec * 8)) * 2u : OOB;
            }
            if (dgelu) {
                rsX = __builtin_amdgcn_make_buffer_rsrc((void*)((T2*)p.aux + (int64_t)m0 * p.ldaux + n0), 0,
                                                        clamp31((int64_t)(m_end - m0) * p.ldaux * 2), 0x00020000);
                ax_vo = col_live ? ax_lane : OOB;
            }
            u32x4 axc[4][2];
            auto load_auxc = [&](auto btag) {
                constexpr int MB = decltype(btag)::value;
                if (MB < 8 && dgelu) {
#pragma unroll
                    for (int k = 0; k < 2; ++k)
                        axc[MB & 3][k] = __builtin_amdgcn_raw_buffer_load_b128(rsX, ax_vo + (unsigned)((MB * 16 + k * 8) * p.ldaux * 2), 0, 0);
                }
            };
            load_auxc(std::integral_constant<int, 0>{});
            load_auxc(std::integral_constant<int, 1>{});
            char* wst = smem + STG_OFF + w * WST_BYTES;
            const int wsw = (frow >> 1) & 7;
            char* wst_w = wst + frow * 128 + (fq & 1) * 8;
            const char* wst_r0 = wst + er * 128 + ((ec ^ ((er >> 1) & 7)) << 4);
            const char* wst_r1 = wst + (er + 8) * 128 + ((ec ^ (((er >> 1) + 4) & 7)) << 4);
            auto pack4g = [&](const f32x4& v) -> u32x2 {
                unsigned lo, hi;
                asm("v_cvt_pk_bf16_f32 %0, %1, %2" : "=v"(lo) : "v"(v[0]), "v"(v[1]));
                asm("v_cvt_pk_bf16_f32 %0, %1, %2" : "=v"(hi) : "v"(v[2]), "v"(v[3]));
                return u32x2{lo, hi};
            };
            auto block4 = [&](auto btag) {
                constexpr int MB = decltype(btag)::value;
                load_auxc(std::integral_constant<int, MB + 2>{});
                if (two_out) {
#pragma unroll
                    for (int ntl = 0; ntl < 4; ++ntl) *(u32x2*)(wst_w + (((ntl * 2 + (fq >> 1)) ^ wsw) << 4)) = pack4g(acc[MB][ntl]);
                    asm volatile("" ::: "memory");
                    const u32x4 o0 = *(const u32x4*)wst_r0, o1 = *(const u32x4*)wst_r1;
                    asm volatile("" ::: "memory");
                    __builtin_amdgcn_raw_buffer_store_b128(o0, rsC2, c2_vo + (unsigned)((MB * 16) * p.ldc2 * 2), 0, 0);
                    __builtin_amdgcn_raw_buffer_store_b128(o1, rsC2, c2_vo + (unsigned)((MB * 16 + 8) * p.ldc2 * 2), 0, 0);
                }
#pragma unroll
                for (int ntl = 0; ntl < 4; ++ntl) {
                    f32x4 v = acc[MB][ntl];
                    if (!dgelu) {
#pragma unroll
                        for (int e = 0; e < 4; ++e) v[e] = gelu_sel<T2>(v[e]);
                    }
                    *(u32x2*)(wst_w + (((ntl * 2 + (fq >> 1)) ^ wsw) << 4)) = pack4g(v);
                }
                asm volatile("" ::: "memory");
                u32x4 o[2];
                o[0] = *(const u32x4*)wst_r0;
                o[1] = *(const u32x4*)wst_r1;
                asm volatile("" ::: "memory");
#pragma unroll
                for (int k = 0; k < 2; ++k) {
                    if (dgelu) {
                        const u32x4 a = axc[MB & 3][k];
#pragma unroll
                        for (int e = 0; e < 4; ++e) o[k][e] = mul_dgelu_bf16x2(o[k][e], a[e]);
                    }
                    __builtin_amdgcn_raw_buffer_store_b128(o[k], rsC, co_vo + (unsigned)((MB * 16 + k * 8) * p.ldc * 2), 0, 0);
                }
            };
            block4(std::integral_constant<int, 0>{}); block4(std::integral_constant<int, 1>{});
            block4(std::integral_constant<int, 2>{}); block4(std::integral_constant<int, 3>{});
            block4(std::integral_constant<int, 4>{}); block4(std::integral_constant<int, 5>{});
            block4(std::integral_constant<int, 6>{}); block4(std::integral_constant<int, 7>{});
        } else if (EPI == 5 || EPI == 6) {
            fetch_bias(it + 1);
            const float relu_floor = (p.act == UMR_ACT_RELU) ? 0.f : -INFINITY;
            const bool planes = (p.flags & UMR_EPI_OUT_X3) != 0;
            const bool maskf = (p.flags & UMR_EPI_MASK_RELU) != 0;
            const bool maskp = (p.flags & UMR_EPI_AUX_X3) != 0;
            if (RED) {
                f32x4 rw[2][4];
#pragma unroll
                for (int c = 0; c < 2; ++c)
#pragma unroll
                    for (int ntl = 0; ntl < 4; ++ntl)
                        rw[c][ntl] = *(const f32x4*)(smem + STG_OFF + c * 1024 + (wc * 64 + ntl * 16 + fq * 4) * 4);
#pragma unroll
                for (int mt = 0; mt < 8; ++mt) {
                    float rs0 = 0.f, rs1 = 0.f;
#pragma unroll
                    for (int ntl = 0; ntl < 4; ++ntl) {
                        const f32x4 v = acc[mt][ntl];
#pragma unroll
                        for (int e = 0; e < 4; ++e) {
                            const float t = fmaxf(v[e], relu_floor);
                            rs0 += t * rw[0][ntl][e];
                            rs1 += t * rw[1][ntl][e];
                        }
                    }
                    rs0 += __shfl_xor(rs0, 16, 64); rs0 += __shfl_xor(rs0, 32, 64);
                    rs1 += __shfl_xor(rs1, 16, 64); rs1 += __shfl_xor(rs1, 32, 64);
                    const int m = m0 + wr * 128 + mt * 16 + frow;
                    if (fq == 0 && m < m_end && n0 + wc * 64 < p.N) {
                        float* ro = p.red_out + ((int64_t)(tn * 4 + wc) * p.M + m) * p.red_c;
                        ro[0] = rs0;
                        if (p.red_c == 2) ro[1] = rs1;
                    }
                }
            } else {
#pragma unroll 1
            for (int mt = 0; mt < 8; ++mt) {
                if (mt > 0) __syncthreads();
                switch (mt) {
                    case 0: stage_rows(std::integral_constant<int, 0>{}); break;
                    case 1: stage_rows(std::integral_constant<int, 1>{}); break;
                    case 2: stage_rows(std::integral_constant<int, 2>{}); break;
                    case 3: stage_rows(std::integral_constant<int, 3>{}); break;
                    case 4: stage_rows(std::integral_constant<int, 4>{}); break;
                    case 5: stage_rows(std::integral_constant<int, 5>{}); break;
                    case 6: stage_rows(std::integral_constant<int, 6>{}); break;
                    default: stage_rows(std::integral_constant<int, 7>{}); break;
                }
                __syncthreads();
                constexpr int UNROLL_J = (EPI == 6) ? 1 : 2;
#pragma clang loop unroll_count(UNROLL_J)
                for (int j = 0; j < 2; ++j) {
                    const int lr = (tid >> 5) + j * 16, cg = tid & 31;
                    const int m = m0 + (lr >> 4) * 128 + mt * 16 + (lr & 15), n = n0 + cg * 8;
                    if (m >= m_end || n >= p.N) continue;
                    const int sw = lr & 15;
                    f32x4 v0 = *(const f32x4*)(stg + lr * 256 + (((2 * cg) ^ sw) << 2));
                    f32x4 v1 = *(const f32x4*)(stg + lr * 256 + (((2 * cg + 1) ^ sw) << 2));
                    if constexpr (EPI == 6) {
                        x3_epilogue_store8<false>(p, m, n, v0, v1);
                    } else {
#pragma unroll
                        for (int e = 0; e < 4; ++e) { v0[e] = fmaxf(v0[e], relu_floor); v1[e] = fmaxf(v1[e], relu_floor); }
                        if (maskf) {
                            f32x4 a0, a1;
                            if (maskp) {
                                const bf16x8 h = *(const bf16x8*)((const T2*)p.aux + (int64_t)m * p.ldaux + n);
                                a0 = f32x4{(float)h[0], (float)h[1], (float)h[2], (float)h[3]};
                                a1 = f32x4{(float)h[4], (float)h[5], (float)h[6], (float)h[7]};
                            } else {
                                const float* ap = (const float*)p.aux + (int64_t)m * p.ldaux + n;
                                a0 = *(const f32x4*)ap; a1 = *(const f32x4*)(ap + 4);
                            }
#pragma unroll
                            for (int e = 0; e < 4; ++e) { v0[e] = a0[e] > 0.f ? v0[e] : 0.f; v1[e] = a1[e] > 0.f ? v1[e] : 0.f; }
                        }
                        const int64_t mo = m + (int64_t)sp * p.M;
                        if (planes) x3_planes_store8((T2*)p.C + mo * p.ldc + n, p.N, v0, v1);
                        else { float* cp = (float*)p.C + mo * p.ldc + n; *(f32x4*)cp = v0; *(f32x4*)(cp + 4) = v1; }
                    }
                }
            }
            }
        } else {
            const bool vec_ok = ((p.N & 7) == 0) && ((p.ldc & 7) == 0) && ((p.ldc2 & 7) == 0) && ((p.ldaux & 7) == 0) &&
                                ((p.ldaux2 & 7) == 0);
#pragma unroll 1
            for (int mt = 0; mt < 8; ++mt) {
                if (mt > 0) __syncthreads();
                switch (mt) {
                    case 0: stage_rows(std::integral_constant<int, 0>{}); break;
                    case 1: stage_rows(std::integral_constant<int, 1>{}); break;
                    case 2: stage_rows(std::integral_constant<int, 2>{}); break;
                    case 3: stage_rows(std::integral_constant<int, 3>{}); break;
                    case 4: stage_rows(std::integral_constant<int, 4>{}); break;
                    case 5: stage_rows(std::integral_constant<int, 5>{}); break;
                    case 6: stage_rows(std::integral_constant<int, 6>{}); break;
                    default: stage_rows(std::integral_constant<int, 7>{}); break;
                }
                __syncthreads();
#pragma unroll 1
                for (int j = 0; j < 2; ++j) {
                    const int lr = (tid >> 5) + j * 16, cg = tid & 31;
                    const int m = m0 + (lr >> 4) * 128 + mt * 16 + (lr & 15), n = n0 + cg * 8;
                    if (m >= m_end || n >= p.N) continue;
                    const int sw = lr & 15;
                    const f32x4 v0 = *(const f32x4*)(stg + lr * 256 + (((2 * cg) ^ sw) << 2));
                    const f32x4 v1 = *(const f32x4*)(stg + lr * 256 + (((2 * cg + 1) ^ sw) << 2));
                    if (vec_ok) {
                        epilogue_store8<T2>(p, m, n, v0, v1);
                    } else {
                        epilogue_store<T2>(p, m, n, v0);
                        if (n + 4 < p.N) epilogue_store<T2>(p, m, n + 4, v1);
                    }
                }
            }
        }
        __syncthreads();
    }
    asm volatile("s_waitcnt vmcnt(0)" ::: "memory");
#undef QUADRANT
#undef QUADRANT_S
#undef QUADRANT_HI
#undef QUADRANT_HID
#undef QUADRANT_SD
#undef QUADRANT_D
#undef MFMA
#undef PHASE_SYNC
#undef PHASE_SYNC_N
#undef STAGE_DMA
#undef READ_WAIT
#undef END_SYNC_N
#undef A_FRAG
#undef B_FRAG
}

__global__ __launch_bounds__(256) void x3_splitk_finish_kernel(const umr_gemm_desc p, const float* __restrict__ slabs, int ksplit, int64_t slab_stride) {
    const int n8 = p.N >> 3;
    const int64_t total = (int64_t)p.M * n8;
    for (int64_t idx = (int64_t)blockIdx.x * blockDim.x + threadIdx.x; idx < total; idx += (int64_t)gridDim.x * blockDim.x) {
        const int m = (int)(idx / n8);
        const int n = (int)(idx - (int64_t)m * n8) * 8;
        const float* q = slabs + (int64_t)m * p.N + n;
        f32x4 v0 = *(const f32x4*)q, v1 = *(const f32x4*)(q + 4);
        for (int s_ = 1; s_ < ksplit; ++s_) {
            const float* qs = q + s_ * slab_stride;
            v0 += *(const f32x4*)qs; v1 += *(const f32x4*)(qs + 4);
        }
        x3_epilogue_store8<true>(p, m, n, v0, v1);
    }
}

int num_cus() {
    static const int n = [] {
        int dev = 0;
        hipDeviceProp_t prop;
        return (hipGetDevice(&dev) == hipSuccess && hipGetDeviceProperties(&prop, dev) == hipSuccess && prop.multiProcessorCount > 0)
                   ? prop.multiProcessorCount : 256;
    }();
    return n;
}

}

bool umr_nt256p_fast_epilogue(const umr_gemm_desc* d) {
    const bool vec_ok = ((d->N & 7) == 0) && ((d->ldc & 7) == 0) && ((d->ldaux & 7) == 0);
    const bool mask = (d->flags & UMR_EPI_MASK_RELU) != 0, add = (d->flags & UMR_EPI_ADD_AUX) != 0;
    return vec_ok && d->c2_mode == 0 && d->c_rows_in <= 0 && d->aux_mod <= 0 &&
           !(d->flags & (UMR_EPI_ROWBIAS | UMR_EPI_ADD_AUX2 | UMR_EPI_OUT_F32 | UMR_EPI_MASK_DGELU)) && !(mask && add) &&
           (d->act == UMR_ACT_NONE || (d->act == UMR_ACT_RELU && !mask && !add));
}
bool umr_nt256p_plain_epilogue(const umr_gemm_desc* d) {
    return umr_nt256p_fast_epilogue(d) && (!d->red_w || (d->conv == 0 && !(d->flags & (UMR_EPI_ADD_AUX | UMR_EPI_MASK_RELU))));
}

static bool umr_nt256p_gelu_epilogue(const umr_gemm_desc* d) {
    const bool vec_ok = ((d->N & 7) == 0) && ((d->ldc & 7) == 0) && ((d->ldaux & 7) == 0) && ((d->ldc2 & 7) == 0);
    const bool dg = (d->flags & UMR_EPI_MASK_DGELU) != 0;
    return vec_ok && (d->c2_mode == 0 || (d->c2_mode == 2 && !dg)) && d->c_rows_in <= 0 && d->aux_mod <= 0 && !d->red_w && !d->no_store &&
           !(d->flags & (UMR_EPI_ROWBIAS | UMR_EPI_ADD_AUX2 | UMR_EPI_OUT_F32 | UMR_EPI_MASK_RELU | UMR_EPI_ADD_AUX)) &&
           ((d->act == UMR_ACT_GELU && !dg) || (d->act == UMR_ACT_NONE && dg));
}

static void x3_plan(const umr_gemm_desc* d, int cus, int npairs, int64_t ws_bytes, int* bm_out, int* ks_out) {
    const int tiles_n = (d->N + BN2 - 1) / BN2;
    const int kt = d->conv == 0 ? d->K / BK2 : 9 * (d->Cin / BK2);
    const int bm_env = umr_opt_or(UMR_OPT_NT256_BM, 0);
    const int64_t slab = (int64_t)d->M * d->N * 4;
    int best_ks = 1, best_bm = BM2;
    double best_cost = 1e300;
    for (int bm = BM2; bm >= (d->conv == 0 ? 192 : BM2); bm -= 32) {
        if (d->conv == 0 && (bm_env == 256 || bm_env == 224 || bm_env == 192) && bm != bm_env) continue;
        const int64_t tiles = (int64_t)((d->M + bm - 1) / bm) * tiles_n;
        for (int ks = 1; ks <= 32 && ks * 2 <= kt + 1; ++ks) {
            if (d->red_w && ks > 1) break;
            if (ks > 1 && ((int64_t)ks * slab > ws_bytes)) break;
            const int per = (kt + ks - 1) / ks;
            if ((kt + per - 1) / per != ks) continue;
            const int64_t rounds = (tiles * ks + cus - 1) / cus;
            const double cost = (double)rounds * (per * npairs * (bm / 256.0) + 8.0) + (ks > 1 ? 8.0 + (double)ks * slab / 4.5e6 : 0.0);
            if (cost < best_cost * (ks > best_ks ? 0.90 : 0.98)) { best_cost = cost; best_ks = ks; best_bm = bm; }
        }
    }
    *bm_out = best_bm;
    *ks_out = best_ks;
}

extern "C" int64_t umr_gemm_nt_x3_workspace(const umr_gemm_desc* d) {
    if (d == nullptr || d->dtype != UMR_BF16X3 || d->M <= 0 || d->N <= 0 || d->K <= 0) return 0;
    int bm, ks;
    x3_plan(d, num_cus(), umr_f32_mode_now() == UMR_F32_X3_FAST ? 3 : 6, (int64_t)1 << 40, &bm, &ks);
    return ks > 1 ? (int64_t)ks * d->M * d->N * 4 : 0;
}

int umr_x3_ksplit_of(const umr_gemm_desc* d, int64_t ws_bytes) {
    if (ws_bytes <= 0) return 1;
    int bm, ks;
    x3_plan(d, num_cus(), umr_f32_mode_now() == UMR_F32_X3_FAST ? 3 : 6, ws_bytes, &bm, &ks);
    return ks;
}

int umr_launch_gemm_nt256p_ws(const umr_gemm_desc* d, void* ws, int64_t ws_bytes, hipStream_t s);
int umr_launch_gemm_nt256p(const umr_gemm_desc* d, hipStream_t s) { return umr_launch_gemm_nt256p_ws(d, nullptr, 0, s); }

int umr_launch_gemm_nt256p_ws(const umr_gemm_desc* d, void* ws, int64_t ws_bytes, hipStream_t s) {
    const int tiles_n = (d->N + BN2 - 1) / BN2;
    const int cus = num_cus();
    constexpr int stagger = 1;
    const int bm_env = umr_opt_or(UMR_OPT_NT256_BM, 0);
    int bm = BM2;
    if (d->conv == 0 && d->dtype == UMR_BF16) {
        if (bm_env == 256 || bm_env == 224 || bm_env == 192) bm = bm_env;
        else if ((int64_t)((d->M + BM2 - 1) / BM2) * tiles_n <= 16ll * cus) {
            double best = 1e300;
            for (int c = 256; c >= 192; c -= 32) {
                const int64_t t = (int64_t)((d->M + c - 1) / c) * tiles_n;
                const double cost = (double)((t + cus - 1) / cus) * (0.25 + 0.75 * c / 256.0);
                if (cost < best - 1e-9) { best = cost; bm = c; }
            }
        }
    }
    const int npairs_x3 = umr_f32_mode_now() == UMR_F32_X3_FAST ? 3 : 6;
    int ksplit = 1;
    if (d->dtype == UMR_BF16X3) x3_plan(d, cus, npairs_x3, ws != nullptr ? ws_bytes : 0, &bm, &ksplit);
    if (d->dtype == UMR_BF16X3 && umr_opt(UMR_OPT_X3_TRACE) != UMR_OPT_UNSET)
        fprintf(stderr, "x3 M=%d N=%d K=%d conv=%d Cin=%d ks=%d bm=%d flags=%u act=%d red=%d\n", d->M, d->N, d->K, d->conv, d->Cin, ksplit, bm,
                (unsigned)d->flags, d->act, d->red_w != nullptr);
    const int tiles_m = (d->M + bm - 1) / bm;
    const int64_t total = (int64_t)tiles_m * tiles_n;
    int64_t kf = total / ((int64_t)cus * 32);
    if (kf < 1) kf = 1;
    if (kf > 8) kf = 8;
    const int budget = umr_cu_budget_now();
    const int cub = (budget > 0 && budget < cus) ? budget : cus;
    if (cub < cus) kf = 1;
    int64_t grid64 = cub * kf;
    if (ksplit > 1) grid64 = (cub + ksplit - 1) / ksplit;
    if (total < grid64) grid64 = total;
    const int grid = (int)grid64;
    dim3 g((unsigned)grid, (unsigned)ksplit), b(512);
    const bool fast_ep = umr_nt256p_fast_epilogue(d);
    const int ph_e = umr_opt(UMR_OPT_NT256_PH2);
    const int kt_steps = (d->conv == 0 ? d->K / BK2 : 9 * (d->Cin / BK2)) * (d->dtype == UMR_BF16X3 ? npairs_x3 : 1) / (ksplit > 1 ? ksplit : 1);
    const bool two = ph_e != UMR_OPT_UNSET ? (ph_e != 0) : (kt_steps >= 8);
#define L256P(CV, EP, AX, RD)                                                                                          \
    do {                                                                                                               \
        if (CV == 1 || two) {                                                                                          \
            UMR_SET_MAX_LDS_ONCE((gemm_nt256p_kernel<CV, EP, AX, RD, false, true>), LDS2P);                            \
            hipLaunchKernelGGL((gemm_nt256p_kernel<CV, EP, AX, RD, false, true>), g, b, LDS2P, s, *d, tiles_n, (int)total, stagger, bm); \
        } else {                                                                                                       \
            UMR_SET_MAX_LDS_ONCE((gemm_nt256p_kernel<0, EP, AX, RD, false, false>), LDS2P);                            \
            hipLaunchKernelGGL((gemm_nt256p_kernel<0, EP, AX, RD, false, false>), g, b, LDS2P, s, *d, tiles_n, (int)total, stagger, bm); \
        }                                                                                                              \
    } while (0)
    if ((d->red_w || d->no_store) && !umr_nt256p_plain_epilogue(d))
        return umr_set_error(UMR_ERR_UNSUPPORTED, "gemm_nt: fused row reduction / no_store needs the fast epilogue class (no aux operand with the reduction)");
    const int auxm = (d->flags & UMR_EPI_ADD_AUX) ? 1 : (d->flags & UMR_EPI_MASK_RELU) ? 2 : 0;
#define L256PX(CV, EP)                                                                                                 \
    do {                                                                                                               \
        if (CV == 1 || two) {                                                                                          \
            UMR_SET_MAX_LDS_ONCE((gemm_nt256p_kernel<CV, EP, 0, false, true, true>), LDS2P);                           \
            hipLaunchKernelGGL((gemm_nt256p_kernel<CV, EP, 0, false, true, true>), g, b, LDS2P, s, *d, tiles_n, (int)total, stagger, bm, npairs, 0); \
        } else {                                                                                                       \
            UMR_SET_MAX_LDS_ONCE((gemm_nt256p_kernel<0, EP, 0, false, true, false>), LDS2P);                           \
            hipLaunchKernelGGL((gemm_nt256p_kernel<0, EP, 0, false, true, false>), g, b, LDS2P, s, *d, tiles_n, (int)total, stagger, bm, npairs, 0); \
        }                                                                                                              \
    } while (0)
    if (d->dtype == UMR_BF16X3) {
        const int npairs = npairs_x3;
        if (d->red_w) {
            if (two) {
                UMR_SET_MAX_LDS_ONCE((gemm_nt256p_kernel<0, 5, 0, true, true, true>), LDS2P);
                hipLaunchKernelGGL((gemm_nt256p_kernel<0, 5, 0, true, true, true>), g, b, LDS2P, s, *d, tiles_n, (int)total, stagger, bm, npairs, 0);
            } else {
                UMR_SET_MAX_LDS_ONCE((gemm_nt256p_kernel<0, 5, 0, true, true, false>), LDS2P);
                hipLaunchKernelGGL((gemm_nt256p_kernel<0, 5, 0, true, true, false>), g, b, LDS2P, s, *d, tiles_n, (int)total, stagger, bm, npairs, 0);
            }
        } else if (ksplit > 1) {
            umr_gemm_desc sd = *d;
            sd.C = ws; sd.ldc = d->N; sd.C2 = nullptr; sd.c2_mode = 0; sd.bias = nullptr; sd.aux = nullptr; sd.aux2 = nullptr; sd.rowbias = nullptr;
            sd.flags = UMR_EPI_OUT_F32; sd.act = UMR_ACT_NONE; sd.c_rows_in = 0; sd.aux_mod = 0;
            const umr_gemm_desc* dd = &sd;
            const int kt_all = d->conv == 0 ? d->K / BK2 : 9 * (d->Cin / BK2);
            const int kt_per = (kt_all + ksplit - 1) / ksplit;
#define L256PXS(CV)                                                                                                    \
    do {                                                                                                               \
        if (CV == 1 || two) {                                                                                          \
            UMR_SET_MAX_LDS_ONCE((gemm_nt256p_kernel<CV, 5, 0, false, true, true>), LDS2P);                            \
            hipLaunchKernelGGL((gemm_nt256p_kernel<CV, 5, 0, false, true, true>), g, b, LDS2P, s, *dd, tiles_n, (int)total, stagger, bm, npairs, kt_per); \
        } else {                                                                                                       \
            UMR_SET_MAX_LDS_ONCE((gemm_nt256p_kernel<0, 5, 0, false, true, false>), LDS2P);                            \
            hipLaunchKernelGGL((gemm_nt256p_kernel<0, 5, 0, false, true, false>), g, b, LDS2P, s, *dd, tiles_n, (int)total, stagger, bm, npairs, kt_per); \
        }                                                                                                              \
    } while (0)
            if (d->conv == 0) L256PXS(0); else L256PXS(1);
#undef L256PXS
            UMR_LAUNCH_CHECK();
            const int64_t tasks = (int64_t)d->M * (d->N >> 3);
            int64_t fg = (tasks + 255) / 256;
            if (fg > 8192) fg = 8192;
            hipLaunchKernelGGL(x3_splitk_finish_kernel, dim3((unsigned)fg), dim3(256), 0, s, *d, (const float*)ws, ksplit, (int64_t)d->M * d->N);
        } else {
            const bool lean = !(d->flags & ~(UMR_EPI_BIAS | UMR_EPI_OUT_F32 | UMR_EPI_OUT_X3 | UMR_EPI_MASK_RELU | UMR_EPI_AUX_X3)) && d->c2_mode == 0 &&
                              d->c_rows_in <= 0 && d->aux_mod <= 0 && d->act != UMR_ACT_GELU;
            if (d->conv == 0) { if (lean) L256PX(0, 5); else L256PX(0, 6); }
            else { if (lean) L256PX(1, 5); else L256PX(1, 6); }
        }
        UMR_LAUNCH_CHECK();
        return UMR_OK;
    }
#undef L256PX
    if (d->conv == 0) {
        if (fast_ep) {
            if (d->red_w) L256P(0, 3, 0, true);
            else if (auxm == 0) L256P(0, 3, 0, false);
            else if (auxm == 1) L256P(0, 3, 1, false);
            else L256P(0, 3, 2, false);
        } else if (umr_nt256p_gelu_epilogue(d)) { if (d->flags & UMR_EPI_MASK_DGELU) L256P(0, 4, 2, false); else L256P(0, 4, 0, false); }
        else L256P(0, 1, 0, false);
    } else {
        if (fast_ep) {
            if (auxm == 0) L256P(1, 3, 0, false);
            else if (auxm == 1) L256P(1, 3, 1, false);
            else L256P(1, 3, 2, false);
        } else L256P(1, 1, 0, false);
    }
#undef L256P
    UMR_LAUNCH_CHECK();
    return UMR_OK;
}
```

### unmore_amd/csrc/umr_api.hip

```cpp
#include "umr_common.h"
#include <string.h>

static thread_local char g_err[256] = "";

int umr_set_error(int code, const char* msg) {
    strncpy(g_err, msg ? msg : "", sizeof(g_err) - 1);
    g_err[sizeof(g_err) - 1] = 0;
    return code;
}

extern "C" int umr_version(void) { return 100; }
extern "C" const char* umr_last_error_string(void) { return g_err; }

#include <atomic>
#include <stdlib.h>
static std::atomic<int> g_f32_mode{-1};
int umr_f32_mode_now() {
    int m = g_f32_mode.load(std::memory_order_relaxed);
    if (m < 0) {
        const char* e = getenv("UMR_F32_X3");
        m = (e && atoi(e) == 0) ? UMR_F32_EXACT : UMR_F32_X3;
        g_f32_mode.store(m, std::memory_order_relaxed);
    }
    return m;
}
extern "C" int umr_set_f32_mode(int mode) {
    if (mode != UMR_F32_EXACT && mode != UMR_F32_X3 && mode != UMR_F32_X3_FAST) return umr_set_error(UMR_ERR_INVALID, "umr_set_f32_mode: unknown mode");
    g_f32_mode.store(mode, std::memory_order_relaxed);
    return UMR_OK;
}
extern "C" int umr_get_f32_mode(void) { return umr_f32_mode_now(); }

static std::atomic<int> g_cu_budget{-1};
int umr_cu_budget_now() {
    int b = g_cu_budget.load(std::memory_order_relaxed);
    if (b < 0) {
        const char* e = getenv("UMR_CU_BUDGET");
        b = e ? atoi(e) : 0;
        if (b < 0) b = 0;
        g_cu_budget.store(b, std::memory_order_relaxed);
    }
    return b;
}
extern "C" int umr_set_cu_budget(int cus) {
    if (cus < 0) return umr_set_error(UMR_ERR_INVALID, "umr_set_cu_budget: negative budget");
    g_cu_budget.store(cus, std::memory_order_relaxed);
    return UMR_OK;
}
extern "C" int umr_get_cu_budget(void) { return umr_cu_budget_now(); }

static const char* const g_opt_names[UMR_OPT_COUNT] = {
    "UMR_GEMM_TILE", "UMR_NT_SPLITK", "UMR_SPLITK_FENCE", "UMR_NT_ORDER", "UMR_NT256_PERSIST", "UMR_NT256_BM",
    "UMR_X3_TRACE", "UMR_NT256_PH2", "UMR_ATTN_BWD_FUSED", "UMR_BILINEAR_GY", "UMR_HEAD_OUT_BWD_GENERIC"};
static std::atomic<int> g_opt[UMR_OPT_COUNT];
static int opt_parse(const char* v) {
    if (!v) return UMR_OPT_UNSET;
    if ((v[0] >= '0' && v[0] <= '9') || v[0] == '-' || v[0] == '+') return atoi(v);
    return (int)(unsigned char)v[0];
}
static const bool g_opt_loaded = [] {
    for (int i = 0; i < UMR_OPT_COUNT; ++i) g_opt[i].store(opt_parse(getenv(g_opt_names[i])), std::memory_order_relaxed);
    return true;
}();
int umr_opt(int id) { return g_opt[id].load(std::memory_order_relaxed); }
extern "C" int umr_set_debug_option(const char* name, const char* value) {
    if (!name) return umr_set_error(UMR_ERR_INVALID, "umr_set_debug_option: null name");
    for (int i = 0; i < UMR_OPT_COUNT; ++i)
        if (strcmp(name, g_opt_names[i]) == 0) {
            g_opt[i].store(opt_parse(value), std::memory_order_relaxed);
            return UMR_OK;
        }
    return umr_set_error(UMR_ERR_INVALID, "umr_set_debug_option: unknown option");
}
extern "C" int umr_get_debug_option(const char* name, int* value, int* is_set) {
    if (!name) return umr_set_error(UMR_ERR_INVALID, "umr_get_debug_option: null name");
    for (int i = 0; i < UMR_OPT_COUNT; ++i)
        if (strcmp(name, g_opt_names[i]) == 0) {
            const int v = g_opt[i].load(std::memory_order_relaxed);
            if (is_set) *is_set = v != UMR_OPT_UNSET;
            if (value) *value = v == UMR_OPT_UNSET ? 0 : v;
            return UMR_OK;
        }
    return umr_set_error(UMR_ERR_INVALID, "umr_get_debug_option: unknown option");
}
```

### unmore_amd/csrc/umr_common.h

```cpp
#pragma once
#include <hip/hip_runtime.h>
#include <stdint.h>
#include "../../include/umr.h"

typedef __bf16 bf16_t;
typedef __attribute__((ext_vector_type(8))) __bf16 bf16x8;
typedef __attribute__((ext_vector_type(4))) __bf16 bf16x4;
typedef __attribute__((ext_vector_type(2))) __bf16 bf16x2;
typedef __attribute__((ext_vector_type(4))) float f32x4;
typedef __attribute__((ext_vector_type(2))) float f32x2;
typedef __attribute__((ext_vector_type(16))) float f32x16;
typedef __attribute__((ext_vector_type(2))) unsigned u32x2;
typedef __attribute__((ext_vector_type(4))) unsigned u32x4;

#define UMR_GLOBAL_PTR(p) ((const __attribute__((address_space(1))) void*)(p))
#define UMR_LDS_PTR(p) ((__attribute__((address_space(3))) void*)(p))

__device__ __forceinline__ void glds16(const void* gsrc, void* lds_wave_base) {
    __builtin_amdgcn_global_load_lds(UMR_GLOBAL_PTR(gsrc), UMR_LDS_PTR(lds_wave_base), 16, 0, 0);
}

template <typename T> __device__ __forceinline__ float to_f32(T v);
template <> __device__ __forceinline__ float to_f32<float>(float v) { return v; }
template <> __device__ __forceinline__ float to_f32<bf16_t>(bf16_t v) { return (float)v; }
template <typename T> __device__ __forceinline__ T from_f32(float v);
template <> __device__ __forceinline__ float from_f32<float>(float v) { return v; }
template <> __device__ __forceinline__ bf16_t from_f32<bf16_t>(float v) { return (bf16_t)v; }

template <typename T> struct Vec4;
template <> struct Vec4<float> {
    static __device__ __forceinline__ f32x4 load(const float* p) { return *(const f32x4*)p; }
    static __device__ __forceinline__ void store(float* p, f32x4 v) { *(f32x4*)p = v; }
};
template <> struct Vec4<bf16_t> {
    static __device__ __forceinline__ f32x4 load(const bf16_t* p) {
        bf16x4 t = *(const bf16x4*)p;
        f32x4 r = {(float)t[0], (float)t[1], (float)t[2], (float)t[3]};
        return r;
    }
    static __device__ __forceinline__ void store(bf16_t* p, f32x4 v) {
        bf16x4 t = {(bf16_t)v[0], (bf16_t)v[1], (bf16_t)v[2], (bf16_t)v[3]};
        *(bf16x4*)p = t;
    }
};

__device__ __forceinline__ float gelu_erf(float x) { return 0.5f * x * (1.0f + erff(x * 0.70710678118654752440f)); }
__device__ __forceinline__ float dgelu_erf(float x) {
    const float cdf = 0.5f * (1.0f + erff(x * 0.70710678118654752440f));
    const float pdf = 0.39894228040143267794f * __expf(-0.5f * x * x);
    return cdf + x * pdf;
}

__device__ __forceinline__ void erf_exp_fast(float x, float& erf_z, float& e) {
    const float z = fabsf(x) * 0.70710678118654752440f;
    const float t = __builtin_amdgcn_rcpf(1.0f + 0.3275911f * z);
    e = __builtin_amdgcn_exp2f(-0.72134752044448170368f * x * x);
    const float poly = t * (0.254829592f + t * (-0.284496736f + t * (1.421413741f + t * (-1.453152027f + t * 1.061405429f))));
    const float r = 1.0f - poly * e;
    erf_z = x < 0.f ? -r : r;
}
template <typename T> __device__ __forceinline__ float gelu_sel(float x) {
    if constexpr (sizeof(T) == 2) {
        float ez, e;
        erf_exp_fast(x, ez, e);
        return 0.5f * x * (1.0f + ez);
    } else {
        return gelu_erf(x);
    }
}
template <typename T> __device__ __forceinline__ float dgelu_sel(float x) {
    if constexpr (sizeof(T) == 2) {
        float ez, e;
        erf_exp_fast(x, ez, e);
        return 0.5f * (1.0f + ez) + x * 0.39894228040143267794f * e;
    } else {
        return dgelu_erf(x);
    }
}

template <typename V> __device__ __forceinline__ V wave_sum(V v) {
#pragma unroll
    for (int o = 32; o > 0; o >>= 1) v += __shfl_xor(v, o, 64);
    return v;
}
__device__ __forceinline__ float wave_max(float v) {
#pragma unroll
    for (int o = 32; o > 0; o >>= 1) v = fmaxf(v, __shfl_xor(v, o, 64));
    return v;
}

template <int ND, int NN>
__device__ __forceinline__ void block_sum_fixed(double (&d)[ND], long long (&n)[NN], double* red_d, long long* red_n) {
    const int tid = threadIdx.x, lane = tid & 63, wv = tid >> 6;
#pragma unroll
    for (int k = 0; k < ND; ++k) d[k] = wave_sum(d[k]);
#pragma unroll
    for (int k = 0; k < NN; ++k) n[k] = wave_sum(n[k]);
    __syncthreads();
    if (lane == 0) {
#pragma unroll
        for (int k = 0; k < ND; ++k) red_d[wv * ND + k] = d[k];
#pragma unroll
        for (int k = 0; k < NN; ++k) red_n[wv * NN + k] = n[k];
    }
    __syncthreads();
    if (tid == 0) {
#pragma unroll
        for (int k = 0; k < ND; ++k) d[k] = ((red_d[k] + red_d[ND + k]) + red_d[2 * ND + k]) + red_d[3 * ND + k];
#pragma unroll
        for (int k = 0; k < NN; ++k) n[k] = red_n[k] + red_n[NN + k] + red_n[2 * NN + k] + red_n[3 * NN + k];
    }
}

template <int ND, int NN> struct SumPartial {
    double d[ND];
    int32_t c[NN + (NN & 1)];
};
static_assert(sizeof(SumPartial<1, 5>) == 32 && sizeof(SumPartial<2, 7>) == 48, "the loss workspaces are sized by these records");

template <int ND, int NN, typename I>
__device__ __forceinline__ void partials_sum_fixed(const SumPartial<ND, NN>* __restrict__ partials, I n_partials, double (&d)[ND],
                                                   long long (&n)[NN], double* red_d, long long* red_n) {
#pragma unroll
    for (int k = 0; k < ND; ++k) d[k] = 0.0;
#pragma unroll
    for (int k = 0; k < NN; ++k) n[k] = 0;
    for (I i = threadIdx.x; i < n_partials; i += 256) {
        const SumPartial<ND, NN> q = partials[i];
#pragma unroll
        for (int k = 0; k < ND; ++k) d[k] += q.d[k];
#pragma unroll
        for (int k = 0; k < NN; ++k) n[k] += q.c[k];
    }
    block_sum_fixed(d, n, red_d, red_n);
}

static __device__ uint4 umr_zero_page[16];

#include <atomic>
#define UMR_SET_MAX_LDS_ONCE(fn, bytes)                                                                             \
    do {                                                                                                            \
        static std::atomic<bool> done_{false};                                                                      \
        if (!done_.load(std::memory_order_acquire)) {                                                               \
            (void)hipFuncSetAttribute((const void*)(fn), hipFuncAttributeMaxDynamicSharedMemorySize, (bytes));      \
            done_.store(true, std::memory_order_release);                                                           \
        }                                                                                                           \
    } while (0)

#include <limits.h>
enum {
    UMR_OPT_GEMM_TILE = 0, UMR_OPT_NT_SPLITK, UMR_OPT_SPLITK_FENCE, UMR_OPT_NT_ORDER, UMR_OPT_NT256_PERSIST, UMR_OPT_NT256_BM,
    UMR_OPT_X3_TRACE, UMR_OPT_NT256_PH2, UMR_OPT_ATTN_BWD_FUSED, UMR_OPT_BILINEAR_GY, UMR_OPT_HEAD_OUT_BWD_GENERIC, UMR_OPT_COUNT
};
#define UMR_OPT_UNSET INT_MIN
int umr_opt(int id);
static inline int umr_opt_or(int id, int dflt) { const int v = umr_opt(id); return v == UMR_OPT_UNSET ? dflt : v; }

int umr_set_error(int code, const char* msg);
int umr_f32_mode_now();
int umr_cu_budget_now();
#define UMR_CHECK_ARG(cond, msg) do { if (!(cond)) return umr_set_error(UMR_ERR_INVALID, msg); } while (0)
#define UMR_LAUNCH_CHECK() do { hipError_t e_ = hipGetLastError(); if (e_ != hipSuccess) return umr_set_error(UMR_ERR_HIP - (int)e_, hipGetErrorString(e_)); } while (0)

int umr_rle_parse_launch(const uint8_t* chars, const int64_t* char_offsets, int K, int64_t total_chars, const int64_t* out_desc,
                         const int32_t* group_start, int G, int64_t out_bytes, int32_t* status, int32_t* nruns, long long* num,
                         uint32_t* starts, hipStream_t stream);
```

### unmore_amd/engine.py

```python
import os

import torch

from . import _lib as L
from . import graphs
from . import ops
from .engine_x3 import X3Numerics, _drop_f, _f
from .packs import (ParamGroup, PackCache, _ACT, _pack_conv3, _pack_conv3_dgrad, _pack_convT, _pack_convT_dgrad, _pack_linear,
                    _pack_linear_t, _rep_bias, _unpack_conv3_grad)

CONFIGS = {
    "dpt_large": dict(D=1024, depth=24, heads=16, patch=16, pos_grid=24, hooks=[5, 11, 17, 23], features=[256, 512, 1024, 1024]),
    "dpt_base": dict(D=768, depth=12, heads=12, patch=16, pos_grid=24, hooks=[2, 5, 8, 11], features=[96, 192, 384, 768]),
    "dpt_small": dict(D=384, depth=12, heads=6, patch=16, pos_grid=24, hooks=[2, 5, 8, 11], features=[48, 96, 192, 384]),
    "dpt_large14": dict(D=1024, depth=24, heads=16, patch=14, pos_grid=37, hooks=[5, 11, 17, 23], features=[256, 512, 1024, 1024]),
    "dpt_tiny": dict(D=128, depth=4, heads=2, patch=16, pos_grid=24, hooks=[0, 1, 2, 3], features=[32, 64, 128, 128]),
}

_FUSE_HEAD_OUT = True
_COMMUTE_RESIZE = True


_WGRAD_STREAM = os.environ.get("UMR_WGRAD_STREAM", "auto")
_side_streams = {}


class WgradStream:

    def __init__(self, dev, on):
        self.on = bool(on)
        self.staged = graphs.staged() if self.on else None
        if self.on and self.staged is None:
            self.main = torch.cuda.current_stream(dev)
            key = (dev.index, self.main.cuda_stream)
            if key not in _side_streams:
                if len(_side_streams) > 16:
                    _side_streams.clear()
                _side_streams[key] = torch.cuda.Stream(device=dev)
            self.side = _side_streams[key]

    def run(self, fn, *used):
        if not self.on:
            return fn()
        if self.staged is not None:
            return self.staged.defer(fn, used)
        self.side.wait_stream(self.main)
        graphs.note_fork(self.main, self.side)
        with torch.cuda.stream(self.side):
            fn()
        for t in used:
            if t is not None:
                t.record_stream(self.side)

    def stage_end(self):
        if self.staged is not None:
            self.staged.boundary()

    def join(self):
        if self.on and self.staged is None:
            self.main.wait_stream(self.side)
        elif self.staged is not None:
            self.staged.join()

    @staticmethod
    def wanted(pixels):
        if _WGRAD_STREAM in ("0", "1"):
            return _WGRAD_STREAM == "1"
        return pixels <= graphs.AUTO_MAX_PIXELS


class PlainNumerics:

    def __init__(self, e, P):
        self.e, self.P = e, P

    def val(self, t):
        return t

    def to_dt(self, t):
        return t if self.e.dt == torch.float32 else ops.cast(t, self.e.dt)

    def mm(self, A, wname, kind, bias=None, *, conv=0, act=L.ACT_NONE, want="f", mask=None, dgelu=None, aux=None, aux2=None,
           rowbias=None, rows_per_batch=0, c2_mode=0, c2_want="f", out=None, c_remap=None, aux_mod=0):
        a_t = mask if mask is not None else (dgelu if dgelu is not None else aux)
        return ops.gemm_nt(A, self.e._w(self.P, wname, kind), bias, out=out, aux=a_t, aux2=aux2, rowbias=rowbias,
                           rows_per_batch=rows_per_batch, act=act, mask_relu=mask is not None, mask_dgelu=dgelu is not None,
                           c2_mode=c2_mode, conv=conv, c_remap=c_remap, aux_mod=aux_mod)

    def wgrad(self, dY, X, dW, dbias=None, *, conv=0, wg=None, then=None):
        def launch():
            r = ops.gemm_tn(dY, X, dW=dW, dbias=dbias, conv=conv)
            if then is not None:
                then(r)
            return r
        return launch() if wg is None else wg.run(launch, dY, X)

    def layernorm(self, x, gamma, beta):
        return ops.layernorm_fwd(x, gamma, beta)

    def readout(self, tok, wname, bias, save, B, g, Nt, D):
        P, dt = self.P, self.e.dt
        w_full = self.e.cache.get((wname, "lin", dt), P[wname], lambda: _pack_linear(P[wname], dt))
        rb = ops.gemm_nt(tok, w_full[:, D:], bias, M=B, lda=Nt * D, out_f32=True)
        if save:
            r, rpre = ops.gemm_nt(tok, w_full[:, :D], None, rowbias=rb, rows_per_batch=g, act=L.ACT_GELU, c2_mode=2, M=B * g,
                                  a_remap=(g, Nt, 1))
        else:
            r, rpre = ops.gemm_nt(tok, w_full[:, :D], None, rowbias=rb, rows_per_batch=g, act=L.ACT_GELU, M=B * g,
                                  a_remap=(g, Nt, 1)), None
        return dict(r=r, rpre=rpre)

    def readout_wgrad(self, d_rpre, rs, tok, dW, B, g, Nt):
        ops.gemm_tn(d_rpre, tok, dW=dW, x_remap=(g, Nt, 1), M=B * g)

    def hook_grad(self, d_rpre, sB, wname, dx, B, g, Nt, D):
        dt = self.e.dt
        w = self.P[wname].detach()
        wa_t = self.e.cache.get((wname, "lin_t_a", dt), self.P[wname], lambda: _pack_linear_t(w[:, :D], dt))
        wb_t = self.e.cache.get((wname, "lin_t_b", dt), self.P[wname], lambda: _pack_linear_t(w[:, D:], dt))
        if dx is None:
            dx = torch.zeros((B * Nt, D), dtype=dt, device=sB.device)
        ops.gemm_nt(d_rpre, wa_t, None, out=dx, aux=dx, c_remap=(g, Nt, 1))
        cls_rows = dx.view(B, Nt * D)[:, :D]
        ops.gemm_nt(sB, wb_t, None, out=cls_rows, aux=cls_rows)
        return dx

    def head_resize(self, h1l, shape_low, H, W, relu):
        return ops.bilinear_fwd(h1l.view(*shape_low, -1), H, W, True, relu=relu).view(shape_low[0] * H * W, -1)

    def head_tail(self, h2, w3name, b3, w4, b4, act, final, keep, pre, B, H, W):
        w3 = self.e._w(self.P, w3name, "lin")
        if _FUSE_HEAD_OUT and ops.gemm_nt(h2, w3, b3, act=act, query_rowreduce=True):
            h3, parts = ops.gemm_nt(h2, w3, b3, act=act, red_w=w4.contiguous(), no_store=not keep)
            out = ops.head_out_finish(parts, b4, B, H, W, final)
            return out, h3, (ops.head_out_finish(parts, b4, B, H, W, L.ACT_NONE) if pre else None)
        h3 = ops.gemm_nt(h2, w3, b3, act=act)
        out = ops.head_out_fwd(h3, w4, b4, B, H, W, final)
        return out, h3, (ops.head_out_fwd(h3, w4, b4, B, H, W, L.ACT_NONE) if pre else None)

    def heads_backward(self, S, d_center, d_sdf, G, wgrad_lin, wgrad_c3, done):
        e = self.e
        heads_bwd = e._heads_backward_lowres if S.get("path") is not None else e._heads_backward_fullres
        dpath = heads_bwd(self.P, S, d_center, d_sdf, G, wgrad_lin, wgrad_c3)
        done()
        return dpath

    def patch_wgrad(self, dx, patches, dW, dbias, B, g, Nt):
        return ops.gemm_tn(dx, patches, dW=dW, dbias=dbias, dy_remap=(g, Nt, 1), M=B * g)


class Engine:
    def __init__(self, cfg, head_layouts, compute_dtype=torch.float32, collapse_linear_heads=False, linear_head_backward=None):
        self.cfg = cfg
        self.linear_head_backward = linear_head_backward or "algebraic"
        assert self.linear_head_backward in ("algebraic", "gemm")
        self.center_layout, self.sdf_layout = head_layouts
        self.dt = compute_dtype
        self.cache = PackCache()
        assert collapse_linear_heads in (False, True, "auto")
        self.collapse_linear_heads = collapse_linear_heads

    def _linear_head_weights(self, P, name, idx, dev):
        W1, b1 = self._f32(P, f"{name}.{idx[0]}.weight"), self._f32(P, f"{name}.{idx[0]}.bias")
        W2, b2 = self._f32(P, f"{name}.{idx[1]}.weight"), self._f32(P, f"{name}.{idx[1]}.bias")
        W3, b3 = self._f32(P, f"{name}.{idx[2]}.weight"), self._f32(P, f"{name}.{idx[2]}.bias")
        W4, b4 = self._f32(P, f"{name}.{idx[3]}.weight"), self._f32(P, f"{name}.{idx[3]}.bias")
        C, C1, C3 = W1.shape[1], W1.shape[0], W3.shape[0]
        assert W4.shape[0] == 1 and W2.shape == (C1, C1, 3, 3) and all(t.is_contiguous() for t in (W1, W2, W3, W4))
        f = lambda n: torch.empty(n, dtype=torch.float32, device=dev)
        u, Vc, Kw, tb = f(C1), f(C1 * 9), f(9 * C), f(10)
        ops.small_gemm(W4, W3, u, 1, C1, C3, (0, 1), (C1, 1), (0, 1))
        ops.small_gemm(u, W2, Vc, 1, C1 * 9, C1, (0, 1), (C1 * 9, 1), (0, 1))
        ops.small_gemm(Vc, W1, Kw, 9, C, C1, (1, 9), (C, 1), (C, 1))
        ops.small_gemm(Vc, b1, tb, 9, 1, C1, (1, 9), (1, 0), (1, 0))
        ops.cast(b4, torch.float32, out=tb[9:10])
        ops.small_gemm(u, b2, tb[9:10], 1, 1, C1, (0, 1), (1, 0), (0, 0), accumulate=True)
        ops.small_gemm(W4, b3, tb[9:10], 1, 1, C3, (0, 1), (1, 0), (0, 0), accumulate=True)
        return u, Vc, Kw, tb

    def _collapse(self, lay, save):
        if lay["relu"] or (save and lay["final"] == "sine"):
            return False
        if self.collapse_linear_heads == "auto":
            return (not save) or self.linear_head_backward == "algebraic"
        return bool(self.collapse_linear_heads)

    def _linear_head_weights_cached(self, P, name, idx, dev):
        ps = [P[f"{name}.{i}.{t}"] for i in idx for t in ("weight", "bias")]

        def build():
            u, Vc, Kw, tb = self._linear_head_weights(P, name, idx, dev)
            return u, Vc, Kw, tb, self._tap_matrix(Kw)
        return self.cache.get((name, "collapsed", self.dt), ParamGroup(ps), build)

    def _tap_matrix(self, Kw):
        C = Kw.numel() // 9
        k16 = torch.zeros((16, C), dtype=torch.float32, device=Kw.device)
        k16[:9].copy_(Kw.view(9, C))
        return k16 if self.dt == torch.float32 else ops.cast(k16, self.dt)

    def _linear_head_forward_lowres(self, P, name, idx, path, H, W, act, save):
        if save:
            u, Vc, Kw, tb = self._linear_head_weights(P, name, idx, path.device)
            k16 = self._tap_matrix(Kw)
        else:
            u, Vc, Kw, tb, k16 = self._linear_head_weights_cached(P, name, idx, path.device)
        nb, ph, pw, C = path.shape
        taps = ops.gemm_nt(path.reshape(-1, C), k16, None, out_f32=(self.dt != torch.float32))
        taps = ops.bilinear_fwd(taps.view(nb, ph, pw, 16), H, W, True)
        out = ops.linear_head_gather9(taps, tb, act)
        return out, dict(algebraic=True, act=act, out=out, u=u, Vc=Vc, Kw=Kw)

    def _linear_head_forward(self, P, name, idx, feat, act):
        u, Vc, Kw, tb = self._linear_head_weights(P, name, idx, feat.device)
        out = ops.linear_head_fwd(feat, Kw, tb, act)
        return out, dict(collapsed=True, u=u, Vc=Vc, Kw=Kw, act=act)

    def _linear_head_backward(self, P, name, idx, feat, hs, dout, dfeat, G):
        W1, b1 = self._f32(P, f"{name}.{idx[0]}.weight"), self._f32(P, f"{name}.{idx[0]}.bias")
        W2, b2 = self._f32(P, f"{name}.{idx[1]}.weight"), self._f32(P, f"{name}.{idx[1]}.bias")
        W3, b3 = self._f32(P, f"{name}.{idx[2]}.weight"), self._f32(P, f"{name}.{idx[2]}.bias")
        W4 = self._f32(P, f"{name}.{idx[3]}.weight")
        C, C1, C3 = W1.shape[1], W1.shape[0], W3.shape[0]
        dev = feat.device
        if "u" not in hs:
            hs["u"], hs["Vc"], hs["Kw"], _ = self._linear_head_weights(P, name, idx, dev)
        act, u, Vc, Kw = hs["act"], hs["u"], hs["Vc"], hs["Kw"]
        dout = dout.contiguous()
        R = ops.linear_head_bwd_weight(feat, dout, hs["out"], act)
        Gm, n, D = R[:9 * C], R[9 * C:9 * C + 9], R[9 * C + 9:]
        if dfeat is None:
            dfeat = torch.empty_like(feat)
            ops.linear_head_bwd_data(dout, hs["out"], Kw, dfeat, act, False)
        else:
            ops.linear_head_bwd_data(dout, hs["out"], Kw, dfeat.view(feat.shape), act, True)
        self._linear_head_algebra(P, name, idx, hs, Gm, n, D, G)
        return dfeat

    def _linear_head_algebra(self, P, name, idx, hs, Gm, n, D, G):
        W1, b1 = self._f32(P, f"{name}.{idx[0]}.weight"), self._f32(P, f"{name}.{idx[0]}.bias")
# ... 101 lines not shown
            mm(patches, m + "patch_embed.proj.weight", "lin", b_(m + "patch_embed.proj.bias"), out=tokens, aux=pos_t, aux_mod=g,
               c_remap=(g, Nt, 1))
        else:
            wp = self._w(P, m + "patch_embed.proj.weight", "lin")
            wpad = torch.zeros((D, ldk), dtype=dt, device=dev)
            wpad[:, :K] = wp
            ops.gemm_nt(_f(patches), wpad, b_(m + "patch_embed.proj.bias"), out=tokens, aux=pos_t, aux_mod=g, c_remap=(g, Nt, 1))
        ops.fill_cls(tokens, b_(m + "cls_token").reshape(-1), pos[0].contiguous(), B, Nt * D, D)
        if save:
            S["patches"] = patches

        x = tokens
        acts, blocks = [], []
        for i in range(max(cfg["hooks"]) + 1):
            b = m + f"blocks.{i}."
            ln1, mean1, rstd1 = nx.layernorm(x, b_(b + "norm1.weight"), b_(b + "norm1.bias"))
            qkv = _f(mm(ln1, b + "attn.qkv.weight", "lin", b_(b + "attn.qkv.bias")))
            att, lse = ops.attention_fwd(qkv, B, Nt, heads, need_lse=save)
            att = val(att)
            x1 = _f(mm(att, b + "attn.proj.weight", "lin", b_(b + "attn.proj.bias"), aux=x))
            ln2, mean2, rstd2 = nx.layernorm(x1, b_(b + "norm2.weight"), b_(b + "norm2.bias"))
            if save:
                h, hpre = mm(ln2, b + "mlp.fc1.weight", "lin", b_(b + "mlp.fc1.bias"), act=L.ACT_GELU, c2_mode=2, want="p")
            else:
                h, hpre = mm(ln2, b + "mlp.fc1.weight", "lin", b_(b + "mlp.fc1.bias"), act=L.ACT_GELU, want="p"), None
            x2 = _f(mm(h, b + "mlp.fc2.weight", "lin", b_(b + "mlp.fc2.bias"), aux=x1))
            if save:
                blocks.append(dict(x=x, mean1=mean1, rstd1=rstd1, ln1=ln1, qkv=qkv, att=att, lse=lse, x1=x1, mean2=mean2,
                                   rstd2=rstd2, ln2=ln2, hpre=hpre, h=h))
            x = x2
            if i in cfg["hooks"]:
                acts.append(x)
        if save:
            S["blocks"] = blocks
            S["acts"] = acts

        pp = "backbone.pretrained."
        Fs = cfg["features"]
        layers, re_saved = [], []
        for k in range(4):
            a = pp + f"act_postprocess{k + 1}."
            rs = nx.readout(acts[k], a + "0.project.0.weight", b_(a + "0.project.0.bias"), save, B, g, Nt, D)
            F_ = Fs[k]
            f = mm(rs["r"], a + "3.weight", "lin", b_(a + "3.bias"), want=("f" if k == 3 else "p"))
            if k in (0, 1):
                s = 4 if k == 0 else 2
                bname = a + "4.bias"
                brep = self.cache.get((bname, "rep", s), P[bname], lambda: _rep_bias(P[bname], s * s))
                y = _f(mm(f, a + "4.weight", "ct", brep))
                lay = val(ops.pixel_shuffle(y, B, gh, gw, s, F_))
            elif k == 2:
                lay = f.view(B, gh, gw, F_)
            else:
                lay = mm(f.view(B, gh, gw, F_), a + "4.weight", "c3", b_(a + "4.bias"), conv=2)
                lay = lay.view(B, (gh - 1) // 2 + 1, (gw - 1) // 2 + 1, F_)
            layers.append(lay)
            if save:
                rs["f"] = f
                re_saved.append(rs)
        if save:
            S["re"] = re_saved

        sc = "backbone.scratch."
        rn, rn_relu = [], []
        for k in range(4):
            lay = layers[k]
            o, orl = mm(lay, sc + f"layer{k + 1}_rn.weight", "c3", None, conv=1, c2_mode=1, c2_want="p")
            shp = (lay.shape[0], lay.shape[1], lay.shape[2], 256)
            rn.append(o.view(*shp))
            rn_relu.append(orl.view(*shp))
        fus_saved = {}
        path = None
        for k in (4, 3, 2, 1):
            r_ = sc + f"refinenet{k}."
            x1_, x1_relu = rn[k - 1], rn_relu[k - 1]
            nb, hh, ww, _ = x1_.shape
            shp = (nb, hh, ww, 256)
            fs = {}
            if path is None:
                s_, s_relu = x1_, x1_relu
            else:
                assert path.shape == x1_.shape, "fusion skip/size mismatch"
                t1 = mm(x1_relu, r_ + "resConfUnit1.conv1.weight", "c3", b_(r_ + "resConfUnit1.conv1.bias"), conv=1, act=L.ACT_RELU,
                        want="p").view(*shp)
                s_, s_relu = mm(t1, r_ + "resConfUnit1.conv2.weight", "c3", b_(r_ + "resConfUnit1.conv2.bias"), conv=1, aux=x1_, aux2=path,
                                c2_mode=1, c2_want="p")
                s_, s_relu = s_.view(*shp), s_relu.view(*shp)
                fs.update(x1_relu=x1_relu, t1=t1)
            t2 = mm(s_relu, r_ + "resConfUnit2.conv1.weight", "c3", b_(r_ + "resConfUnit2.conv1.bias"), conv=1, act=L.ACT_RELU,
                    want="p").view(*shp)
            u = mm(t2, r_ + "resConfUnit2.conv2.weight", "c3", b_(r_ + "resConfUnit2.conv2.bias"), conv=1, aux=s_).view(*shp)
            if k > 1 and cfg["patch"] != 16:
                nxt = rn[k - 2].shape
                Ho, Wo = nxt[1], nxt[2]
            else:
                Ho, Wo = 2 * hh, 2 * ww
            if _COMMUTE_RESIZE:
                ul = mm(u.view(nb * hh * ww, 256), r_ + "out_conv.weight", "lin", b_(r_ + "out_conv.bias"))
                path = val(ops.bilinear_fwd(_f(ul).view(nb, hh, ww, 256), Ho, Wo, True))
                del ul
                src = ("u", u)
            else:
                up = val(ops.bilinear_fwd(_f(u), Ho, Wo, True))
                path = mm(up.view(nb * Ho * Wo, 256), r_ + "out_conv.weight", "lin", b_(r_ + "out_conv.bias")).view(nb, Ho, Wo, 256)
                src = ("up", up)
            if save:
                _drop_f(src[1])
                fs.update(s_relu=s_relu, t2=t2, in_hw=(hh, ww))
                fs[src[0]] = src[1]
                fus_saved[k] = fs
        if cfg["patch"] == 16:
            H, W = 2 * path.shape[1], 2 * path.shape[2]
            if save:
                S["H"], S["W"] = H, W
        lowres = _COMMUTE_RESIZE
        feat = val(ops.bilinear_fwd(_f(path), H, W, True)) if not lowres else None
        if save:
            S["fus"] = fus_saved
            S["rn_in"] = layers
            S["path1_hw"] = (path.shape[1], path.shape[2])
            S["feat"] = feat
            if lowres:
                S["path"] = path

        outs, heads_saved = [], []
        M = B * H * W
        low = tuple(path.shape[:3])
        for name, lay in (("center_field_prediction_head", self.center_layout), ("sdf_prediction_head", self.sdf_layout)):
            if name in skip:
                outs.append(None)
                continue
            idx = lay["conv_idx"]
            final = _ACT[lay["final"]]
            if self._collapse(lay, save):
                if lowres:
                    out, cs = self._linear_head_forward_lowres(P, name, idx, _f(path), H, W, final, save)
                else:
                    out, cs = self._linear_head_forward(P, name, idx, _f(feat), final)
                    cs["out"] = out
                outs.append(out)
                if save:
                    heads_saved.append(cs)
                continue
            act = L.ACT_RELU if lay["relu"] else L.ACT_NONE
            algebraic = save and not lay["relu"] and lay["final"] != "sine" and self.linear_head_backward == "algebraic"
            keep = save and not algebraic
            hw, hb = (lambda j: f"{name}.{idx[j]}.weight"), (lambda j: b_(f"{name}.{idx[j]}.bias"))
            if lowres:
                h1l = mm(path.view(low[0] * low[1] * low[2], 256), hw(0), "lin", hb(0))
                h1 = nx.head_resize(h1l, low, H, W, lay["relu"])
                del h1l
            else:
                h1 = mm(feat.view(M, 256), hw(0), "lin", hb(0), act=act, want="p")
            h2 = mm(h1.view(B, H, W, 512), hw(1), "c3", hb(1), conv=1, act=act, want="p")
            w4 = b_(hw(3))
            out, h3, zpre = nx.head_tail(h2, hw(2), hb(2), w4.reshape(w4.shape[0], -1), hb(3), act, final, keep,
                                         save and lay["final"] == "sine", B, H, W)
            outs.append(out)
            if algebraic:
                heads_saved.append(dict(algebraic=True, act=final, out=out))
            elif save:
                heads_saved.append(dict(h1=h1, h2=h2, h3=h3, out=(zpre if zpre is not None else out)))
            del h1, h2, h3
        if save:
            S["heads"] = heads_saved
        return outs[0], outs[1], S

    def _heads_backward_fullres(self, P, S, d_center, d_sdf, G, wgrad_lin, wgrad_c3):
        dt = self.dt
        B, H, W = S["B"], S["H"], S["W"]
        dev = d_center.device
        dfeat = None
        feat = S["feat"]
        merge_dfeat = all(not (hs_.get("collapsed") or hs_.get("algebraic")) for hs_ in S["heads"])
        dh1cat, w1cat = None, []
        for hi, (name, lay, dout) in enumerate((("center_field_prediction_head", self.center_layout, d_center),
                                               ("sdf_prediction_head", self.sdf_layout, d_sdf))):
            hs = S["heads"][hi]
            idx = lay["conv_idx"]
            if hs.get("collapsed") or hs.get("algebraic"):
                dfeat = self._linear_head_backward(P, name, idx, feat, hs, dout, dfeat, G)
                continue
            relu = lay["relu"]
            w4 = self._f32(P, f"{name}.{idx[3]}.weight")
            dh3 = ops.head_out_bwd(hs["h3"], w4.reshape(w4.shape[0], -1), dout.contiguous(), hs["out"], _ACT[lay["final"]], relu,
                                   G[f"{name}.{idx[3]}.weight"].view(w4.shape[0], -1), G[f"{name}.{idx[3]}.bias"])
            hs["h3"] = None
            wgrad_lin(f"{name}.{idx[2]}.weight", dh3, hs["h2"], f"{name}.{idx[2]}.bias")
            dh2 = ops.gemm_nt(dh3, self._w(P, f"{name}.{idx[2]}.weight", "lin_t"), None, aux=(hs["h2"] if relu else None), mask_relu=relu)
            del dh3
            h1 = hs["h1"].view(B, H, W, 512)
            wgrad_c3(f"{name}.{idx[1]}.weight", dh2, h1, f"{name}.{idx[1]}.bias")
            hs["h2"] = None
            c1 = hs["h1"].shape[-1]
            if merge_dfeat and dh1cat is None:
                dh1cat = torch.empty((B * H * W, 2 * c1), dtype=dt, device=dev)
            dh1 = ops.gemm_nt(dh2.view(B, H, W, 512), self._w(P, f"{name}.{idx[1]}.weight", "c3_d"), None, conv=1,
                              aux=(hs["h1"] if relu else None), mask_relu=relu,
                              out=(dh1cat[:, hi * c1:(hi + 1) * c1] if merge_dfeat else None))
            del dh2
            hs["h1"] = None
            wgrad_lin(f"{name}.{idx[0]}.weight", dh1, feat.view(-1, 256), f"{name}.{idx[0]}.bias")
            if merge_dfeat:
                w1cat.append(self._w(P, f"{name}.{idx[0]}.weight", "lin_t"))
            elif dfeat is None:
                dfeat = ops.gemm_nt(dh1, self._w(P, f"{name}.{idx[0]}.weight", "lin_t"), None)
            else:
                ops.gemm_nt(dh1, self._w(P, f"{name}.{idx[0]}.weight", "lin_t"), None, aux=dfeat, out=dfeat)
            del dh1
        if merge_dfeat:
            dfeat = ops.gemm_nt(dh1cat, torch.cat(w1cat, dim=1), None)
            del dh1cat
        S["feat"] = None
        ph, pw = S["path1_hw"]
        dpath = ops.bilinear_bwd(dfeat.view(B, H, W, 256), ph, pw, True)
        del dfeat
        return dpath

    def _heads_backward_lowres(self, P, S, d_center, d_sdf, G, wgrad_lin, wgrad_c3):
        dt = self.dt
        B, H, W = S["B"], S["H"], S["W"]
        path = S["path"]
        nb, ph, pw, C = path.shape
        pl = path.view(-1, C)
        Ml = pl.shape[0]
        dev = path.device
        widths = [64 if hs_.get("algebraic") else hs_["h1"].shape[-1] for hs_ in S["heads"]]
        K = sum(widths)
        dlow = torch.empty((Ml, K), dtype=dt, device=dev)
        bcat = torch.zeros((C, K), dtype=dt, device=dev)
        c0 = 0
        for hi, (name, lay, dout) in enumerate((("center_field_prediction_head", self.center_layout, d_center),
                                               ("sdf_prediction_head", self.sdf_layout, d_sdf))):
            hs = S["heads"][hi]
            idx = lay["conv_idx"]
            if hs.get("algebraic"):
                if "u" not in hs:
                    hs["u"], hs["Vc"], hs["Kw"], _ = self._linear_head_weights(P, name, idx, dev)
                s9, nd = ops.linear_head_shift9(dout.contiguous(), hs["out"], hs["act"], dt)
                ops.bilinear_bwd(s9, ph, pw, True, out=dlow[:, c0:c0 + 16].unflatten(0, (nb, ph, pw)))
                del s9
                dlow[:, c0 + 16:c0 + 64].zero_()
                gm = ops.gemm_tn(dlow[:, c0:c0 + 16], pl)
                self._linear_head_algebra(P, name, idx, hs, gm[:9].reshape(-1), nd[:9], nd[9:10], G)
                bcat[:, c0:c0 + 9].copy_(hs["Kw"].view(9, C).t())
                c0 += 64
                continue
            relu = lay["relu"]
            w4 = self._f32(P, f"{name}.{idx[3]}.weight")
            dh3 = ops.head_out_bwd(hs["h3"], w4.reshape(w4.shape[0], -1), dout.contiguous(), hs["out"], _ACT[lay["final"]], relu,
                                   G[f"{name}.{idx[3]}.weight"].view(w4.shape[0], -1), G[f"{name}.{idx[3]}.bias"])
            hs["h3"] = None
            wgrad_lin(f"{name}.{idx[2]}.weight", dh3, hs["h2"], f"{name}.{idx[2]}.bias")
            dh2 = ops.gemm_nt(dh3, self._w(P, f"{name}.{idx[2]}.weight", "lin_t"), None, aux=(hs["h2"] if relu else None), mask_relu=relu)
            del dh3
            c1 = hs["h1"].shape[-1]
            wgrad_c3(f"{name}.{idx[1]}.weight", dh2, hs["h1"].view(B, H, W, c1), f"{name}.{idx[1]}.bias")
            hs["h2"] = None
            dh1 = ops.gemm_nt(dh2.view(B, H, W, -1), self._w(P, f"{name}.{idx[1]}.weight", "c3_d"), None, conv=1,
                              aux=(hs["h1"] if relu else None), mask_relu=relu)
            del dh2
            hs["h1"] = None
            ops.bilinear_bwd(dh1.view(B, H, W, c1), ph, pw, True, out=dlow[:, c0:c0 + c1].unflatten(0, (nb, ph, pw)))
            del dh1
            wgrad_lin(f"{name}.{idx[0]}.weight", dlow[:, c0:c0 + c1], pl, f"{name}.{idx[0]}.bias")
            bcat[:, c0:c0 + c1].copy_(self._w(P, f"{name}.{idx[0]}.weight", "lin_t"))
            c0 += c1
        dpath = ops.gemm_nt(dlow, bcat, None).view(nb, ph, pw, C)
        S["path"] = None
        S["feat"] = None
        return dpath

    def backward(self, P, S, d_center, d_sdf, G, stage_cb=None, join_at_stages=False):
        cfg = self.cfg
        nx = S["numerics"](self, P)
        mm, val = nx.mm, nx.val
        B, H, W, gh, gw = S["B"], S["H"], S["W"], S["gh"], S["gw"]
        D, heads, p = cfg["D"], cfg["heads"], cfg["patch"]
        g, Nt = gh * gw, gh * gw + 1
        dev = d_center.device
        wg = WgradStream(dev, WgradStream.wanted(B * H * W))
        ln_via = wg.run if wg.staged is not None else None

        def cb(name):
            if join_at_stages:
                wg.join()
            if stage_cb is not None:
                stage_cb(name, wg)
            wg.stage_end()

        def wgrad_lin(name, dy, x, bias_name=None):
            nx.wgrad(dy, x, G[name].view(G[name].shape[0], -1), (G[bias_name] if bias_name else None), wg=wg)

        def wgrad_c3(name, dy, x_nhwc, bias_name=None, conv=1):
            co = G[name].shape[0]
            nx.wgrad(dy.view(-1, co), x_nhwc, None, (G[bias_name] if bias_name else None), conv=conv, wg=wg,
                     then=lambda dwp: _unpack_conv3_grad(dwp, G[name]))

        dpath = nx.heads_backward(S, d_center, d_sdf, G, wgrad_lin, wgrad_c3, lambda: cb("heads"))

        sc = "backbone.scratch."
        d_rn = {}
        for k in (1, 2, 3, 4):
            r_ = sc + f"refinenet{k}."
            fs = S["fus"][k]
            hh, ww = fs["in_hw"]
            nb, Hp, Wp = dpath.shape[0], dpath.shape[1], dpath.shape[2]
            shp = (nb, hh, ww, 256)
            if "u" in fs:
                dul = val(ops.bilinear_bwd(_f(dpath), hh, ww, True)).view(nb * hh * ww, 256)
                wgrad_lin(r_ + "out_conv.weight", dul, fs["u"].view(nb * hh * ww, 256), r_ + "out_conv.bias")
                du = mm(dul, r_ + "out_conv.weight", "lin_t", None).view(*shp)
                del dul
            else:
                dp2 = dpath.view(nb * Hp * Wp, 256)
                wgrad_lin(r_ + "out_conv.weight", dp2, fs["up"].view(nb * Hp * Wp, 256), r_ + "out_conv.bias")
                dup = _f(mm(dp2, r_ + "out_conv.weight", "lin_t", None))
                du = val(ops.bilinear_bwd(dup.view(nb, Hp, Wp, 256), hh, ww, True))
                del dup
            wgrad_c3(r_ + "resConfUnit2.conv2.weight", du, fs["t2"], r_ + "resConfUnit2.conv2.bias")
            dt2 = mm(du, r_ + "resConfUnit2.conv2.weight", "c3_d", None, conv=1, mask=fs["t2"], want="p").view(*shp)
            wgrad_c3(r_ + "resConfUnit2.conv1.weight", dt2, fs["s_relu"], r_ + "resConfUnit2.conv1.bias")
            ds = mm(dt2, r_ + "resConfUnit2.conv1.weight", "c3_d", None, conv=1, mask=fs["s_relu"], aux2=du, want="p").view(*shp)
            del dt2, du
            if "t1" in fs:
                wgrad_c3(r_ + "resConfUnit1.conv2.weight", ds, fs["t1"], r_ + "resConfUnit1.conv2.bias")
                dt1 = mm(ds, r_ + "resConfUnit1.conv2.weight", "c3_d", None, conv=1, mask=fs["t1"], want="p").view(*shp)
                wgrad_c3(r_ + "resConfUnit1.conv1.weight", dt1, fs["x1_relu"], r_ + "resConfUnit1.conv1.bias")
                dx1 = mm(dt1, r_ + "resConfUnit1.conv1.weight", "c3_d", None, conv=1, mask=fs["x1_relu"], aux2=ds, want="p").view(*shp)
                del dt1
                d_rn[k] = dx1
                dpath = ds
            else:
                d_rn[k] = ds
            S["fus"][k] = None

        cb("refine")
        pp = "backbone.pretrained."
        Fs = cfg["features"]
        d_hook = [None] * 4
        for k in range(4):
            lay_in = S["rn_in"][k]
            dr = d_rn.pop(k + 1)
            wgrad_c3(sc + f"layer{k + 1}_rn.weight", dr, lay_in, None)
            dl = mm(dr, sc + f"layer{k + 1}_rn.weight", "c3_d", None, conv=1, want=("p" if k == 2 else "f"))
            del dr
            a = pp + f"act_postprocess{k + 1}."
            F_ = Fs[k]
            rs = S["re"][k]
            f = rs["f"]
            if k in (0, 1):
                s = 4 if k == 0 else 2
                dyu = val(ops.pixel_shuffle(_f(dl).view(B, gh * s, gw * s, F_), B, gh, gw, s, F_, inverse=True))
                brep = torch.empty(s * s * F_, dtype=torch.float32, device=dev)
                dwp = nx.wgrad(dyu, f.view(B * g, F_), None, brep)
                gw_ = G[a + "4.weight"]
                ops.permute4(dwp, gw_, (F_, F_, s, s), (1, F_, s * F_ * F_, F_ * F_))
                ops.segsum(brep, 1, s * s, F_, 0, F_, out=G[a + "4.bias"].view(1, F_))
                df = mm(dyu, a + "4.weight", "ct_d", None, want="p")
                del dyu
            elif k == 2:
                df = dl.view(B * g, F_)
            else:
                ho, wo = (gh - 1) // 2 + 1, (gw - 1) // 2 + 1
                wgrad_c3(a + "4.weight", dl, f.view(B, gh, gw, F_), a + "4.bias", conv=2)
                stuffed = val(ops.zero_stuff2(_f(dl).view(B, ho, wo, F_), gh, gw))
                df = mm(stuffed, a + "4.weight", "c3_d", None, conv=1, want="p").view(B * g, F_)
                del stuffed
            del dl
            wgrad_lin(a + "3.weight", df, rs["r"], a + "3.bias")
            d_rpre = mm(df, a + "3.weight", "lin_t", None, dgelu=rs["rpre"], want="p")
            del df
            tok = S["acts"][k]
            wname = a + "0.project.0.weight"
            gfull = G[wname]
            nx.readout_wgrad(d_rpre, rs, tok, gfull[:, :D], B, g, Nt)
            sB32 = ops.segsum(_f(d_rpre), B, g, D, g * D, D)
            ops.segsum(sB32, 1, B, D, 0, D, out=G[a + "0.project.0.bias"].view(1, D))
            sB = nx.to_dt(sB32)
            ops.gemm_tn(sB, tok, dW=gfull[:, D:], M=B, ldx=Nt * D)
            d_hook[k] = (d_rpre, sB, wname)
            S["re"][k] = None

        cb("reassemble")

        m = "backbone.pretrained.model."
        dx = None
        hooks = cfg["hooks"]
        for i in range(max(hooks), -1, -1):
            if i in hooks:
                k = hooks.index(i)
                dx = nx.hook_grad(*d_hook[k], dx, B, g, Nt, D)
                d_hook[k] = None
            b = m + f"blocks.{i}."
            bs = S["blocks"][i]
            dxx = val(dx)
            wgrad_lin(b + "mlp.fc2.weight", dxx, bs["h"], b + "mlp.fc2.bias")
            dhp = mm(dxx, b + "mlp.fc2.weight", "lin_t", None, dgelu=bs["hpre"], want="p")
            wgrad_lin(b + "mlp.fc1.weight", dhp, bs["ln2"], b + "mlp.fc1.bias")
            dln2 = _f(mm(dhp, b + "mlp.fc1.weight", "lin_t", None))
            del dhp, dxx
            dx1 = ops.layernorm_bwd(dln2, bs["x1"], self._f32(P, b + "norm2.weight"), bs["mean2"], bs["rstd2"],
                                    G[b + "norm2.weight"], G[b + "norm2.bias"], dres=dx, params_via=ln_via)
            del dln2
            dx1x = val(dx1)
            wgrad_lin(b + "attn.proj.weight", dx1x, bs["att"], b + "attn.proj.bias")
            datt = _f(mm(dx1x, b + "attn.proj.weight", "lin_t", None))
# ... 31 lines not shown
```

### unmore_amd/ops.py

```python
import collections
import ctypes

import torch

from . import _lib as L
from . import graphs

_DT = {torch.float32: L.F32, torch.bfloat16: L.BF16}


_cur_dev = torch._C._cuda_getDevice
_raw_stream = torch._C._cuda_getCurrentRawStream


def _stream_id(device_index=None):
    return _raw_stream(_cur_dev() if device_index is None else device_index)


def _stream():
    return ctypes.c_void_p(_raw_stream(_cur_dev()))


def _p(t):
    return ctypes.c_void_p(t.data_ptr()) if t is not None else None


def _need_gpu(*ts):
    for t in ts:
        if t is not None and not t.is_cuda:
            raise RuntimeError("unmore_amd ops need GPU tensors (no CPU fallback in the product path)")


def _rowmajor2d(t):
    assert t.stride(-1) == 1, "innermost dimension must be contiguous"
    return t


def set_f32_mode(mode):
    prev = get_f32_mode()
    L.check(L.lib().umr_set_f32_mode({"exact": L.F32_EXACT, "x3": L.F32_X3, "x3_fast": L.F32_X3_FAST}[mode]), "umr_set_f32_mode")
    return prev


def get_f32_mode():
    return {L.F32_EXACT: "exact", L.F32_X3: "x3", L.F32_X3_FAST: "x3_fast"}[L.lib().umr_get_f32_mode()]


def set_cu_budget(cus):
    prev = int(L.lib().umr_get_cu_budget())
    L.check(L.lib().umr_set_cu_budget(int(cus)), "umr_set_cu_budget")
    return prev


def set_debug_option(name, value):
    import ctypes
    v, isset = ctypes.c_int(0), ctypes.c_int(0)
    L.check(L.lib().umr_get_debug_option(name.encode(), ctypes.byref(v), ctypes.byref(isset)), "umr_get_debug_option")
    L.check(L.lib().umr_set_debug_option(name.encode(), None if value is None else str(value).encode()), "umr_set_debug_option")
    return v.value if isset.value else None


def splitk_bad_tickets(device=None):
    import ctypes
    dev = torch.device("cuda", torch.cuda.current_device()) if device is None else device
    ws = _splitk_workspace(dev)
    n = ctypes.c_int(0)
    L.check(L.lib().umr_gemm_nt_ws_status(ctypes.c_void_p(ws.data_ptr()), ctypes.c_void_p(_stream_id(dev.index)), ctypes.byref(n)), "umr_gemm_nt_ws_status")
    return n.value


_ws_cache = {}


_WS_MAX_ENTRIES = 8


def _workspace(nbytes, device):
    if graphs.capturing():
        store = graphs.capture_store()
        key = ("ws", _stream_id(device.index), graphs.lane())
        buf = store.get(key)
        if buf is None or buf.numel() < nbytes:
            if buf is not None:
                store.setdefault("outgrown", []).append(buf)
            buf = store[key] = torch.empty(max(int(nbytes), 1 << 20), dtype=torch.uint8, device=device)
        return buf
    key = (device.index, _stream_id(device.index))
    buf = _ws_cache.pop(key, None)
    if buf is None or buf.numel() < nbytes:
        buf = torch.empty(max(int(nbytes), 1 << 20), dtype=torch.uint8, device=device)
    _ws_cache[key] = buf
    while len(_ws_cache) > _WS_MAX_ENTRIES:
        _ws_cache.pop(next(iter(_ws_cache)))
    return buf


_sk_cache = collections.OrderedDict()


def _splitk_workspace(device):
    if graphs.capturing():
        store = graphs.capture_store()
        key = ("sk", _stream_id(device.index), graphs.lane())
        buf = store.get(key)
        if buf is None:
            buf = store[key] = torch.empty(int(L.lib().umr_gemm_nt_workspace()), dtype=torch.uint8, device=device)
            buf[:16384].zero_()
        return buf
    key = (device.index, _stream_id(device.index))
    buf = _sk_cache.pop(key, None)
    if buf is None:
        buf = torch.empty(int(L.lib().umr_gemm_nt_workspace()), dtype=torch.uint8, device=device)
        buf[:16384].zero_()
    _sk_cache[key] = buf
    while len(_sk_cache) > _WS_MAX_ENTRIES:
        _sk_cache.pop(next(iter(_sk_cache)))
    return buf


def gemm_nt(A, B, bias=None, *, out=None, out2=None, aux=None, aux2=None, rowbias=None, rows_per_batch=0,
            act=L.ACT_NONE, mask_relu=False, mask_dgelu=False, c2_mode=0, out_f32=False,
            conv=0, M=None, lda=None, a_remap=None, c_remap=None, aux_mod=0, red_w=None, no_store=False, query_rowreduce=False,
            query_splits=False):
    _need_gpu(A, B)
    dt = _DT[A.dtype]
    assert B.dtype == A.dtype
    d = L.GemmDesc()
    N, K = B.shape[0], B.shape[1]
    if conv:
        nb, H, W, Cin = A.shape
        assert A.is_contiguous() and K == 9 * Cin
        s = 2 if conv == 2 else 1
        Ho, Wo = (H - 1) // s + 1, (W - 1) // s + 1
        M_ = nb * Ho * Wo
        d.nb, d.H, d.W, d.Cin, d.Ho, d.Wo = nb, H, W, Cin, Ho, Wo
        d.lda = Cin
    else:
        A2 = A if A.dim() == 2 else A.reshape(-1, A.shape[-1])
        M_ = A2.shape[0] if M is None else M
        d.lda = A2.stride(0) if lda is None else lda
        assert A2.stride(1) == 1
    odt = torch.float32 if out_f32 else A.dtype
    skip_c = no_store or query_rowreduce or query_splits
    if out is None and not skip_c:
        out = torch.empty((M_, N), dtype=odt, device=A.device)
    assert skip_c or (out.dtype == odt and out.stride(-1) == 1)
    flags = 0
    if bias is not None:
        assert bias.dtype == torch.float32
        flags |= L.EPI_BIAS
    if rowbias is not None:
        assert rowbias.dtype == torch.float32 and rowbias.is_contiguous()
        flags |= L.EPI_ROWBIAS
    if aux is not None:
        assert aux.dtype == A.dtype
        flags |= L.EPI_MASK_RELU if mask_relu else (L.EPI_MASK_DGELU if mask_dgelu else L.EPI_ADD_AUX)
    if aux2 is not None:
        assert aux2.dtype == A.dtype
        flags |= L.EPI_ADD_AUX2
    if out_f32:
        flags |= L.EPI_OUT_F32
    if c2_mode:
        if out2 is None:
            out2 = torch.empty((M_, N), dtype=A.dtype, device=A.device)
        assert out2.dtype == A.dtype
    o2d = None if out is None else (out.reshape(-1, N) if out.is_contiguous() else out)
    d.A, d.B, d.C, d.C2 = _p(A), _p(B), _p(out), _p(out2)
    d.bias, d.aux, d.aux2, d.rowbias = _p(bias), _p(aux), _p(aux2), _p(rowbias)
    d.ldb = B.stride(0)
    d.ldc = o2d.stride(0) if (o2d is not None and o2d.dim() == 2) else N
    d.ldc2 = (out2.reshape(-1, N).stride(0) if out2 is not None else 0)
    d.ldaux = (aux.reshape(-1, N).stride(0) if aux is not None else 0)
    d.ldaux2 = (aux2.reshape(-1, N).stride(0) if aux2 is not None else 0)
    d.M, d.N, d.K, d.dtype = M_, N, K, dt
    d.flags, d.act, d.c2_mode, d.rows_per_batch, d.conv = flags, act, c2_mode, rows_per_batch, conv
    if a_remap is not None:
        d.a_rows_in, d.a_rows_out, d.a_row_off = a_remap
    if c_remap is not None:
        d.c_rows_in, d.c_rows_out, d.c_row_off = c_remap
    d.aux_mod = aux_mod
    if query_rowreduce:
        return bool(L.lib().umr_gemm_nt_rowreduce_ok(ctypes.byref(d)))
    if query_splits:
        return int(L.lib().umr_gemm_nt_splits(ctypes.byref(d), int(L.lib().umr_gemm_nt_workspace()) if _wants_splitk_ws(d) else 0))
    partials = None
    if red_w is not None:
        assert red_w.dtype == torch.float32 and red_w.is_contiguous() and red_w.shape[1] == N and red_w.shape[0] in (1, 2)
        partials = torch.empty(((N + 63) // 64, M_, red_w.shape[0]), dtype=torch.float32, device=A.device)
        d.red_w, d.red_out, d.red_c = _p(red_w), _p(partials), red_w.shape[0]
    d.no_store = 1 if no_store else 0
    L.check(_timed_call(d), "umr_gemm_nt")
    if red_w is not None:
        return out, partials
    return (out, out2) if c2_mode else out


def split3(x, out=None, remap=None):
    _need_gpu(x)
    assert x.dtype == torch.float32 and x.stride(-1) == 1
    K = x.shape[-1]
    x2 = x.reshape(-1, K) if x.is_contiguous() else x
    assert x2.dim() == 2
    rows = x2.shape[0]
    ri, ro, off = (0, 0, 0)
    if remap is not None:
        ri, ro, off = remap
        assert rows % ro == 0 and off + ri <= ro
        rows = rows // ro * ri
        if out is None:
            out = torch.empty((rows, 3 * K), dtype=torch.bfloat16, device=x.device)
    if out is None:
        out = torch.empty(x.shape[:-1] + (3 * K,), dtype=torch.bfloat16, device=x.device)
    L.check(L.lib().umr_split3_rows(_p(x2), _p(out), rows, K, x2.stride(0), 3 * K, ri, ro, off, _stream()), "umr_split3")
    return out


def unsplit3(pl):
    _need_gpu(pl)
    assert pl.dtype == torch.bfloat16 and pl.is_contiguous() and pl.shape[-1] % 3 == 0
    K = pl.shape[-1] // 3
    out = torch.empty(pl.shape[:-1] + (K,), dtype=torch.float32, device=pl.device)
    rows = pl.numel() // (3 * K)
    L.check(L.lib().umr_unsplit3(_p(pl), _p(out), rows, K, 3 * K, K, _stream()), "umr_unsplit3")
    return out


def _x3_operand(t, N):
    if t.dtype == torch.bfloat16:
        t2 = t.reshape(-1, 3 * N)
        assert t2.stride(1) == 1
        return t2, t2.stride(0), True
    assert t.dtype == torch.float32
    t2 = t.reshape(-1, N)
    assert t2.stride(1) == 1
    return t2, t2.stride(0), False


_x3_ws_cache = collections.OrderedDict()


def _x3_workspace(d, device):
    extra = int(L.lib().umr_gemm_nt_x3_workspace(ctypes.byref(d)))
    if extra == 0:
        return None
    need = int(L.lib().umr_gemm_nt_workspace()) + extra
    if graphs.capturing():
        store = graphs.capture_store()
        key = ("x3ws", _stream_id(device.index), graphs.lane())
        buf = store.get(key)
        if buf is None or buf.numel() < need:
            if buf is not None:
                store.setdefault("outgrown", []).append(buf)
            buf = store[key] = torch.empty(need, dtype=torch.uint8, device=device)
        return buf
    key = (device.index, _stream_id(device.index))
    buf = _x3_ws_cache.pop(key, None)
    if buf is None or buf.numel() < need:
        buf = torch.empty(max(need, 64 << 20), dtype=torch.uint8, device=device)
    _x3_ws_cache[key] = buf
    while len(_x3_ws_cache) > _WS_MAX_ENTRIES:
        _x3_ws_cache.pop(next(iter(_x3_ws_cache)))
    return buf


def gemm_nt_x3(Ap, Bp, bias=None, *, act=L.ACT_NONE, conv=0, out_planes=False, out=None, red_w=None, mask=None, dgelu=None, aux=None,
               aux2=None, rowbias=None, rows_per_batch=0, c2_mode=0, c2_planes=False, c_remap=None, aux_mod=0):
    _need_gpu(Ap, Bp)
    assert Ap.dtype == torch.bfloat16 and Bp.dtype == torch.bfloat16 and Bp.dim() == 2 and Bp.is_contiguous()
    d = L.GemmDesc()
    N, K = Bp.shape[0], Bp.shape[1] // 3
    if conv:
        assert conv == 1
        nb, H, W, C3 = Ap.shape
        Cin = C3 // 3
        assert Ap.is_contiguous() and K == 9 * Cin
        M_ = nb * H * W
        d.nb, d.H, d.W, d.Cin, d.Ho, d.Wo = nb, H, W, Cin, H, W
        d.lda = C3
    else:
        A2 = Ap if Ap.dim() == 2 else Ap.reshape(-1, Ap.shape[-1])
        assert A2.stride(1) == 1 and A2.shape[1] == 3 * K
        M_ = A2.shape[0]
        d.lda = A2.stride(0)
    rows_out = M_
    if c_remap is not None:
        d.c_rows_in, d.c_rows_out, d.c_row_off = c_remap
        rows_out = None
    partials, out2 = None, None
    flags = 0
    if red_w is not None:
        assert red_w.dtype == torch.float32 and red_w.is_contiguous() and red_w.shape[1] == N and red_w.shape[0] in (1, 2) and not conv
        partials = torch.empty(((N + 63) // 64, M_, red_w.shape[0]), dtype=torch.float32, device=Ap.device)
        d.red_w, d.red_out, d.red_c, d.no_store = _p(red_w), _p(partials), red_w.shape[0], 1
        out = None
    else:
        if out is None:
            assert rows_out is not None
            out = torch.empty((rows_out, 3 * N if out_planes else N), dtype=torch.bfloat16 if out_planes else torch.float32, device=Ap.device)
        else:
            out_planes = out.dtype == torch.bfloat16
        flags |= L.EPI_OUT_X3 if out_planes else L.EPI_OUT_F32
        o2 = out if out.dim() == 2 else out.reshape(-1, out.shape[-1])
        assert o2.stride(1) == 1 and o2.shape[1] == (3 * N if out_planes else N)
        d.ldc = o2.stride(0)
    if bias is not None:
        assert bias.dtype == torch.float32
        flags |= L.EPI_BIAS
    if rowbias is not None:
        assert rowbias.dtype == torch.float32 and rowbias.is_contiguous() and rows_per_batch > 0
        flags |= L.EPI_ROWBIAS
        d.rowbias, d.rows_per_batch = _p(rowbias), rows_per_batch
    a_t, a_flag = None, 0
    for t, fl in ((mask, L.EPI_MASK_RELU), (dgelu, L.EPI_MASK_DGELU), (aux, L.EPI_ADD_AUX)):
        if t is not None:
            assert a_t is None, "one of mask / dgelu / aux"
            a_t, a_flag = t, fl
    keep = []
    if a_t is not None:
        t2, ld, pl = _x3_operand(a_t, N)
        flags |= a_flag | (L.EPI_AUX_X3 if pl else 0)
        d.aux, d.ldaux = _p(t2), ld
        keep.append(t2)
    if aux2 is not None:
        t2, ld, pl = _x3_operand(aux2, N)
        flags |= L.EPI_ADD_AUX2 | (L.EPI_AUX2_X3 if pl else 0)
        d.aux2, d.ldaux2 = _p(t2), ld
        keep.append(t2)
    if c2_mode:
        assert red_w is None and c_remap is None
        out2 = torch.empty((M_, 3 * N if c2_planes else N), dtype=torch.bfloat16 if c2_planes else torch.float32, device=Ap.device)
        flags |= L.EPI_C2_X3 if c2_planes else 0
        d.C2, d.ldc2, d.c2_mode = _p(out2), out2.stride(0), c2_mode
    d.aux_mod = aux_mod
    d.A, d.B, d.C, d.bias = _p(Ap), _p(Bp), _p(out), _p(bias)
    d.ldb = Bp.stride(0)
    d.M, d.N, d.K, d.dtype = M_, N, K, L.BF16X3
    d.flags, d.act, d.conv = flags, act, conv
    L.check(_timed_call(d), "umr_gemm_nt")
    if red_w is not None:
        return partials
    return (out, out2) if c2_mode else out


def gemm_tn(dY, X, *, dW=None, dbias=None, accumulate=False, conv=0, M=None, dy_remap=None, x_remap=None, lddy=None, ldx=None, x3=False):
    _need_gpu(dY, X)
    dt = L.BF16X3 if x3 else _DT[X.dtype]
    assert dY.dtype == X.dtype and (not x3 or X.dtype == torch.bfloat16)
# ... 612 lines not shown
```

Measured before the change: 349.0.

## Store head ReLU mask as packed sign bits for backward masking

The 3x3 conv+ReLU GEMM epilogue in the heads can now also emit a packed 1-bit-per-element sign mask through C2. The backward 1x1 dgrad then reads that bitmask instead of the full bf16 activation map to apply the ReLU mask. This cuts aux read traffic in the masked dgrad by roughly 16x for that operand. The cost is an extra byte store in the forward epilogue, plus new validity gating that falls back to the old path when shapes or layouts do not fit.

```diff
diff --git a/include/umr.h b/include/umr.h
--- a/include/umr.h
+++ b/include/umr.h
@@ -28,7 +28,8 @@
     UMR_EPI_BIAS = 1, UMR_EPI_ADD_AUX = 2, UMR_EPI_MASK_RELU = 4, UMR_EPI_MASK_DGELU = 8,
     UMR_EPI_ADD_AUX2 = 16, UMR_EPI_OUT_F32 = 32, UMR_EPI_ROWBIAS = 64,
     UMR_EPI_OUT_X3 = 128,
-    UMR_EPI_AUX_X3 = 256, UMR_EPI_AUX2_X3 = 512, UMR_EPI_C2_X3 = 1024
+    UMR_EPI_AUX_X3 = 256, UMR_EPI_AUX2_X3 = 512, UMR_EPI_C2_X3 = 1024,
+    UMR_EPI_MASK_RELU_BITS = 2048
 };
 enum umr_act { UMR_ACT_NONE = 0, UMR_ACT_RELU = 1, UMR_ACT_GELU = 2, UMR_ACT_TANH = 3, UMR_ACT_SIGMOID = 5  };
 
@@ -67,6 +68,7 @@
 int umr_split3_rows(const float* src, void* dst, int64_t rows, int K, int64_t ld_src, int64_t ld_dst, int rows_in, int rows_out,
                     int row_off, umr_stream_t stream);
 int umr_gemm_nt_rowreduce_ok(const umr_gemm_desc* d);
+int umr_gemm_nt_relu_bits_ok(const umr_gemm_desc* d);
 
 typedef struct umr_gemm_tn_desc {
     const void* dY;
diff --git a/unmore_amd/_lib.py b/unmore_amd/_lib.py
--- a/unmore_amd/_lib.py
+++ b/unmore_amd/_lib.py
@@ -11,6 +11,8 @@
 F32, BF16, BF16X3 = 0, 1, 2
 EPI_BIAS, EPI_ADD_AUX, EPI_MASK_RELU, EPI_MASK_DGELU, EPI_ADD_AUX2, EPI_OUT_F32, EPI_ROWBIAS, EPI_OUT_X3 = 1, 2, 4, 8, 16, 32, 64, 128
 EPI_AUX_X3, EPI_AUX2_X3, EPI_C2_X3 = 256, 512, 1024
+EPI_MASK_RELU_BITS = 2048
+C2_RELU_BITS = 3
 ACT_NONE, ACT_RELU, ACT_GELU, ACT_TANH = 0, 1, 2, 3
 ACT_SIGMOID = 5
 F32_EXACT, F32_X3, F32_X3_FAST = 0, 1, 2
diff --git a/unmore_amd/csrc/gemm_nt.hip b/unmore_amd/csrc/gemm_nt.hip
--- a/unmore_amd/csrc/gemm_nt.hip
+++ b/unmore_amd/csrc/gemm_nt.hip
@@ -435,6 +435,7 @@
 int umr_launch_gemm_nt256p(const umr_gemm_desc* d, hipStream_t s);
 int umr_launch_gemm_nt256p_ws(const umr_gemm_desc* d, void* ws, int64_t ws_bytes, hipStream_t s);
 bool umr_nt256_rowreduce_path(const umr_gemm_desc* d);
+bool umr_nt256_relu_bits_path(const umr_gemm_desc* d);
 
 static int tile_override() {
     return umr_opt_or(UMR_OPT_GEMM_TILE, 0);
@@ -455,6 +456,13 @@
 extern "C" int umr_gemm_nt_rowreduce_ok(const umr_gemm_desc* d) {
     if (d == nullptr || d->M <= 0 || d->N <= 0 || d->K <= 0) return 0;
     return (uses_256(d) && umr_nt256_rowreduce_path(d)) ? 1 : 0;
+}
+
+static bool wants_relu_bits(const umr_gemm_desc* d) { return (d->flags & UMR_EPI_MASK_RELU_BITS) != 0 || d->c2_mode == 3; }
+extern "C" int umr_gemm_nt_relu_bits_ok(const umr_gemm_desc* d) {
+    if (d == nullptr || d->M <= 0 || d->N <= 0 || d->K <= 0 || !wants_relu_bits(d)) return 0;
+    if (umr_opt_or(UMR_OPT_RELU_BITS, 1) == 0) return 0;
+    return (uses_256(d) && umr_nt256_relu_bits_path(d)) ? 1 : 0;
 }
 
 static int gemm_nt_impl(const umr_gemm_desc* d, void* workspace, int64_t workspace_bytes, umr_stream_t stream);
@@ -529,6 +537,9 @@
     UMR_CHECK_ARG(d != nullptr, "gemm_nt: null descriptor");
     UMR_CHECK_ARG(d->A && d->B && (d->C || d->no_store), "gemm_nt: null operand");
     UMR_CHECK_ARG(d->M > 0 && d->N > 0 && d->K > 0, "gemm_nt: empty problem");
+    if (wants_relu_bits(d) && umr_gemm_nt_relu_bits_ok(d) != 1)
+        return umr_set_error(UMR_ERR_UNSUPPORTED, "gemm_nt: c2_mode 3 / UMR_EPI_MASK_RELU_BITS requested on a path that does not implement the "
+                                                  "sign-bit forms (umr_gemm_nt_relu_bits_ok)");
     if (d->dtype == UMR_BF16X3) {
         UMR_CHECK_ARG(d->conv == 0 || d->conv == 1, "gemm_nt (BF16X3): plain GEMM or stride-1 3x3 conv only");
         const int fl = d->flags;
diff --git a/unmore_amd/csrc/gemm_nt256.hip b/unmore_amd/csrc/gemm_nt256.hip
--- a/unmore_amd/csrc/gemm_nt256.hip
+++ b/unmore_amd/csrc/gemm_nt256.hip
@@ -278,6 +278,11 @@
     return ((d->conv == 0 && d->a_rows_in <= 0) || d->conv == 1) && umr_nt256p_plain_epilogue(d);
 }
 
+bool umr_nt256_relu_bits_path(const umr_gemm_desc* d) {
+    if (umr_opt_or(UMR_OPT_NT256_PERSIST, 1) == 0) return false;
+    return ((d->conv == 0 && d->a_rows_in <= 0) || d->conv == 1) && umr_nt256p_fast_epilogue(d);
+}
+
 int umr_launch_gemm_nt256(const umr_gemm_desc* d, hipStream_t s) {
     {
         const int persist = umr_opt_or(UMR_OPT_NT256_PERSIST, 1);
diff --git a/unmore_amd/csrc/gemm_nt256p.hip b/unmore_amd/csrc/gemm_nt256p.hip
--- a/unmore_amd/csrc/gemm_nt256p.hip
+++ b/unmore_amd/csrc/gemm_nt256p.hip
@@ -1,5 +1,6 @@
 #include "umr_common.h"
 #include "gemm_epilogue.h"
+#include "relu_bits.h"
 #include <stdio.h>
 #include <stdlib.h>
 #include <type_traits>
@@ -455,13 +456,13 @@
             typedef __attribute__((ext_vector_type(2))) short s16x2;
             typedef __attribute__((ext_vector_type(2))) unsigned u32x2;
             const short relu_lo = (p.act == UMR_ACT_RELU) ? (short)0 : (short)-32768;
-            const s16x2 relu16 = {relu_lo, relu_lo};
+            const s16x2 relu16 = (AUXM == 4) ? s16x2{0, 0} : s16x2{relu_lo, relu_lo};
             auto pack4 = [&](const f32x4& v) -> u32x2 {
                 unsigned lo, hi;
                 asm("v_cvt_pk_bf16_f32 %0, %1, %2" : "=v"(lo) : "v"(v[0]), "v"(v[1]));
                 asm("v_cvt_pk_bf16_f32 %0, %1, %2" : "=v"(hi) : "v"(v[2]), "v"(v[3]));
                 s16x2 a = __builtin_bit_cast(s16x2, lo), b = __builtin_bit_cast(s16x2, hi);
-                if (AUXM == 0) {
+                if (AUXM == 0 || AUXM == 4) {
                     a = __builtin_elementwise_max(a, relu16);
                     b = __builtin_elementwise_max(b, relu16);
                 }
@@ -512,23 +513,38 @@
                 }
             };
             const bool col_live = n0 + wc * 64 + ec * 8 < p.N;
+            const int c_records = clamp31((int64_t)(m_end - m0) * p.ldc * 2);
             const __amdgpu_buffer_rsrc_t rsC = __builtin_amdgcn_make_buffer_rsrc(
-                (void*)((T2*)p.C + (int64_t)m0 * p.ldc + n0), 0, p.no_store ? 0 : clamp31((int64_t)(m_end - m0) * p.ldc * 2), 0x00020000);
+                (void*)((T2*)p.C + (int64_t)m0 * p.ldc + n0), 0, (AUXM != 4 && p.no_store) ? 0 : c_records, 0x00020000);
             const unsigned co_vo = col_live ? co_lane : OOB;
             __amdgpu_buffer_rsrc_t rsX = rsC;
             unsigned ax_vo = OOB;
-            if (AUXM != 0) {
+            if (AUXM == 1 || AUXM == 2) {
                 rsX = __builtin_amdgcn_make_buffer_rsrc((void*)((T2*)p.aux + (int64_t)m0 * p.ldaux + n0), 0,
                                                         clamp31((int64_t)(m_end - m0) * p.ldaux * 2), 0x00020000);
                 ax_vo = col_live ? ax_lane : OOB;
             }
+            if (AUXM == 3) {
+                rsX = __builtin_amdgcn_make_buffer_rsrc((void*)((const char*)p.aux + umr_relu_bits_offset(m0, n0, p.ldaux)), 0,
+                                                        clamp31((int64_t)(m_end - m0) * p.ldaux), 0x00020000);
+                ax_vo = col_live ? (unsigned)(wr * 128 + er) * (unsigned)p.ldaux + (unsigned)(wc * 8 + ec) : OOB;
+            }
+            __amdgpu_buffer_rsrc_t rsM = rsC;
+            if (AUXM == 4)
+                rsM = __builtin_amdgcn_make_buffer_rsrc((void*)((char*)p.C2 + umr_relu_bits_offset(m0, n0, p.ldc >> 3)), 0, c_records >> 4, 0x00020000);
             u32x4 axc[4][2];
+            unsigned axb[4][2];
             auto load_auxc = [&](auto btag) {
                 constexpr int MB = decltype(btag)::value;
-                if (MB < 8 && AUXM != 0) {
+                if (MB < 8 && (AUXM == 1 || AUXM == 2)) {
 #pragma unroll
                     for (int k = 0; k < 2; ++k)
                         axc[MB & 3][k] = __builtin_amdgcn_raw_buffer_load_b128(rsX, ax_vo + (unsigned)((MB * 16 + k * 8) * p.ldaux * 2), 0, 0);
+                }
+                if (MB < 8 && AUXM == 3) {
+#pragma unroll
+                    for (int k = 0; k < 2; ++k)
+                        axb[MB & 3][k] = __builtin_amdgcn_raw_buffer_load_b8(rsX, ax_vo + (unsigned)((MB * 16 + k * 8) * p.ldaux), 0, 0);
                 }
             };
             load_auxc(std::integral_constant<int, 0>{});
@@ -572,6 +588,11 @@
 #pragma unroll
                             for (int e = 0; e < 4; ++e) o[k][e] &= pos_mask_bf16x2(a[e]);
                         }
+                        if (AUXM == 3) {
+                            const unsigned b = axb[(MB + mh) & 3][k];
+#pragma unroll
+                            for (int e = 0; e < 4; ++e) o[k][e] &= umr_relu_bits_expand(b, e);
+                        }
                         if (AUXM == 1) {
                             const u32x4 a = axc[(MB + mh) & 3][k];
 #pragma unroll
@@ -579,6 +600,8 @@
                         }
                         const unsigned so = (unsigned)(((MB + mh) * 16 + k * 8) * p.ldc * 2);
                         __builtin_amdgcn_raw_buffer_store_b128(o[k], rsC, co_vo + so, 0, 0);
+                        if (AUXM == 4)
+                            __builtin_amdgcn_raw_buffer_store_b8((unsigned char)umr_relu_bits_pack<true>(o[k]), rsM, (co_vo + so) >> 4, 0, 0);
                     }
                 }
             };
@@ -849,9 +872,15 @@
 }
 
 bool umr_nt256p_fast_epilogue(const umr_gemm_desc* d) {
-    const bool vec_ok = ((d->N & 7) == 0) && ((d->ldc & 7) == 0) && ((d->ldaux & 7) == 0);
-    const bool mask = (d->flags & UMR_EPI_MASK_RELU) != 0, add = (d->flags & UMR_EPI_ADD_AUX) != 0;
-    return vec_ok && d->c2_mode == 0 && d->c_rows_in <= 0 && d->aux_mod <= 0 &&
+    const bool bits_in = (d->flags & UMR_EPI_MASK_RELU_BITS) != 0, bits_out = d->c2_mode == 3;
+    if (bits_in || bits_out) {
+        if ((d->N & 63) != 0 || d->red_w || d->no_store) return false;
+        if (bits_in && (d->conv != 0 || (d->flags & (UMR_EPI_MASK_RELU | UMR_EPI_ADD_AUX)) || bits_out || !d->aux || d->ldaux < umr_relu_bits_row_bytes(d->N))) return false;
+        if (bits_out && (d->act != UMR_ACT_RELU || !d->C2 || d->ldc2 * 8 != d->ldc || d->ldc >= (1 << 22))) return false;
+    }
+    const bool vec_ok = ((d->N & 7) == 0) && ((d->ldc & 7) == 0) && (bits_in || (d->ldaux & 7) == 0);
+    const bool mask = (d->flags & (UMR_EPI_MASK_RELU | UMR_EPI_MASK_RELU_BITS)) != 0, add = (d->flags & UMR_EPI_ADD_AUX) != 0;
+    return vec_ok && (d->c2_mode == 0 || bits_out) && d->c_rows_in <= 0 && d->aux_mod <= 0 &&
            !(d->flags & (UMR_EPI_ROWBIAS | UMR_EPI_ADD_AUX2 | UMR_EPI_OUT_F32 | UMR_EPI_MASK_DGELU)) && !(mask && add) &&
            (d->act == UMR_ACT_NONE || (d->act == UMR_ACT_RELU && !mask && !add));
 }
@@ -960,7 +989,10 @@
     } while (0)
     if ((d->red_w || d->no_store) && !umr_nt256p_plain_epilogue(d))
         return umr_set_error(UMR_ERR_UNSUPPORTED, "gemm_nt: fused row reduction / no_store needs the fast epilogue class (no aux operand with the reduction)");
-    const int auxm = (d->flags & UMR_EPI_ADD_AUX) ? 1 : (d->flags & UMR_EPI_MASK_RELU) ? 2 : 0;
+    if (((d->flags & UMR_EPI_MASK_RELU_BITS) || d->c2_mode == 3) && !(d->dtype == UMR_BF16 && fast_ep))
+        return umr_set_error(UMR_ERR_UNSUPPORTED, "gemm_nt: the sign-bit forms (c2_mode 3, UMR_EPI_MASK_RELU_BITS) need the bf16 fast epilogue class and N % 64 == 0");
+    const int auxm = (d->flags & UMR_EPI_ADD_AUX) ? 1 : (d->flags & UMR_EPI_MASK_RELU) ? 2 : (d->flags & UMR_EPI_MASK_RELU_BITS) ? 3 :
+                     (d->c2_mode == 3) ? 4 : 0;
 #define L256PX(CV, EP)                                                                                                 \
     do {                                                                                                               \
         if (CV == 1 || two) {                                                                                          \
@@ -1020,14 +1052,18 @@
             if (d->red_w) L256P(0, 3, 0, true);
             else if (auxm == 0) L256P(0, 3, 0, false);
             else if (auxm == 1) L256P(0, 3, 1, false);
-            else L256P(0, 3, 2, false);
+            else if (auxm == 2) L256P(0, 3, 2, false);
+            else if (auxm == 3) L256P(0, 3, 3, false);
+            else L256P(0, 3, 4, false);
         } else if (umr_nt256p_gelu_epilogue(d)) { if (d->flags & UMR_EPI_MASK_DGELU) L256P(0, 4, 2, false); else L256P(0, 4, 0, false); }
         else L256P(0, 1, 0, false);
     } else {
         if (fast_ep) {
             if (auxm == 0) L256P(1, 3, 0, false);
             else if (auxm == 1) L256P(1, 3, 1, false);
-            else L256P(1, 3, 2, false);
+            else if (auxm == 2) L256P(1, 3, 2, false);
+            else if (auxm == 4) L256P(1, 3, 4, false);
+            else return umr_set_error(UMR_ERR_UNSUPPORTED, "gemm_nt: the 3x3 conv reads its ReLU mask as a bf16 map only");
         } else L256P(1, 1, 0, false);
     }
 #undef L256P
diff --git a/unmore_amd/csrc/relu_bits.h b/unmore_amd/csrc/relu_bits.h
--- /dev/null
+++ b/unmore_amd/csrc/relu_bits.h
@@ -0,0 +1,26 @@
+#pragma once
+#include "umr_common.h"
+
+__host__ __device__ inline int64_t umr_relu_bits_row_bytes(int N) { return (int64_t)(N >> 3); }
+__host__ __device__ inline int64_t umr_relu_bits_offset(int64_t m, int n, int64_t ld) { return m * ld + (n >> 3); }
+
+template <bool NONNEG>
+__device__ __forceinline__ unsigned umr_relu_bits_pack(u32x4 c) {
+    typedef __attribute__((ext_vector_type(2))) short s16x2;
+    const s16x2 one = {1, 1}, zero = {0, 0};
+    const unsigned w[4] = {c[0], c[1], c[2], c[3]};
+    unsigned r = 0;
+#pragma unroll
+    for (int e = 0; e < 4; ++e) {
+        s16x2 v = __builtin_elementwise_min(__builtin_bit_cast(s16x2, w[e]), one);
+        if (!NONNEG) v = __builtin_elementwise_max(v, zero);
+        r |= __builtin_bit_cast(unsigned, v) << (2 * e);
+    }
+    return (r | (r >> 15)) & 0xFFu;
+}
+
+__device__ __forceinline__ unsigned umr_relu_bits_expand(unsigned byte, int e) {
+    const int lo = (int)(byte << (31 - 2 * e)) >> 31;
+    const int hi = (int)(byte << (30 - 2 * e)) >> 31;
+    return ((unsigned)lo & 0x0000FFFFu) | ((unsigned)hi & 0xFFFF0000u);
+}
diff --git a/unmore_amd/csrc/umr_api.hip b/unmore_amd/csrc/umr_api.hip
--- a/unmore_amd/csrc/umr_api.hip
+++ b/unmore_amd/csrc/umr_api.hip
@@ -51,7 +51,7 @@
 
 static const char* const g_opt_names[UMR_OPT_COUNT] = {
     "UMR_GEMM_TILE", "UMR_NT_SPLITK", "UMR_SPLITK_FENCE", "UMR_NT_ORDER", "UMR_NT256_PERSIST", "UMR_NT256_BM",
-    "UMR_X3_TRACE", "UMR_NT256_PH2", "UMR_ATTN_BWD_FUSED", "UMR_BILINEAR_GY", "UMR_HEAD_OUT_BWD_GENERIC"};
+    "UMR_X3_TRACE", "UMR_NT256_PH2", "UMR_ATTN_BWD_FUSED", "UMR_BILINEAR_GY", "UMR_HEAD_OUT_BWD_GENERIC", "UMR_RELU_BITS"};
 static std::atomic<int> g_opt[UMR_OPT_COUNT];
 static int opt_parse(const char* v) {
     if (!v) return UMR_OPT_UNSET;
diff --git a/unmore_amd/csrc/umr_common.h b/unmore_amd/csrc/umr_common.h
--- a/unmore_amd/csrc/umr_common.h
+++ b/unmore_amd/csrc/umr_common.h
@@ -150,7 +150,8 @@
 #include <limits.h>
 enum {
     UMR_OPT_GEMM_TILE = 0, UMR_OPT_NT_SPLITK, UMR_OPT_SPLITK_FENCE, UMR_OPT_NT_ORDER, UMR_OPT_NT256_PERSIST, UMR_OPT_NT256_BM,
-    UMR_OPT_X3_TRACE, UMR_OPT_NT256_PH2, UMR_OPT_ATTN_BWD_FUSED, UMR_OPT_BILINEAR_GY, UMR_OPT_HEAD_OUT_BWD_GENERIC, UMR_OPT_COUNT
+    UMR_OPT_X3_TRACE, UMR_OPT_NT256_PH2, UMR_OPT_ATTN_BWD_FUSED, UMR_OPT_BILINEAR_GY, UMR_OPT_HEAD_OUT_BWD_GENERIC, UMR_OPT_RELU_BITS,
+    UMR_OPT_COUNT
 };
 #define UMR_OPT_UNSET INT_MIN
 int umr_opt(int id);
diff --git a/unmore_amd/engine.py b/unmore_amd/engine.py
--- a/unmore_amd/engine.py
+++ b/unmore_amd/engine.py
@@ -86,6 +86,15 @@
         return ops.gemm_nt(A, self.e._w(self.P, wname, kind), bias, out=out, aux=a_t, aux2=aux2, rowbias=rowbias,
                            rows_per_batch=rows_per_batch, act=act, mask_relu=mask is not None, mask_dgelu=dgelu is not None,
                            c2_mode=c2_mode, conv=conv, c_remap=c_remap, aux_mod=aux_mod)
+
+    def conv_relu_with_bits(self, A, wname, bias, n_next):
+        w = self.e._w(self.P, wname, "c3")
+        kw = dict(conv=1, act=L.ACT_RELU)
+        bits = None
+        if A.dtype == torch.bfloat16 and ops.gemm_nt(A, w, bias, relu_bits_out=True, query_relu_bits=True, **kw):
+            if ops.relu_mask_bits_ok(A.shape[0] * A.shape[1] * A.shape[2], w.shape[0], n_next, A.dtype):
+                return ops.gemm_nt(A, w, bias, relu_bits_out=True, **kw)
+        return ops.gemm_nt(A, w, bias, **kw), bits
 
     def wgrad(self, dY, X, dW, dbias=None, *, conv=0, wg=None, then=None):
         def launch():
@@ -493,7 +502,11 @@
                 del h1l
             else:
                 h1 = mm(feat.view(M, 256), hw(0), "lin", hb(0), act=act, want="p")
-            h2 = mm(h1.view(B, H, W, 512), hw(1), "c3", hb(1), conv=1, act=act, want="p")
+            h2_bits = None
+            if keep and lay["relu"] and isinstance(nx, PlainNumerics):
+                h2, h2_bits = nx.conv_relu_with_bits(h1.view(B, H, W, 512), hw(1), hb(1), P[hw(2)].shape[0])
+            else:
+                h2 = mm(h1.view(B, H, W, 512), hw(1), "c3", hb(1), conv=1, act=act, want="p")
             w4 = b_(hw(3))
             out, h3, zpre = nx.head_tail(h2, hw(2), hb(2), w4.reshape(w4.shape[0], -1), hb(3), act, final, keep,
                                          save and lay["final"] == "sine", B, H, W)
@@ -501,11 +514,18 @@
             if algebraic:
                 heads_saved.append(dict(algebraic=True, act=final, out=out))
             elif save:
-                heads_saved.append(dict(h1=h1, h2=h2, h3=h3, out=(zpre if zpre is not None else out)))
-            del h1, h2, h3
+                heads_saved.append(dict(h1=h1, h2=h2, h2_bits=h2_bits, h3=h3, out=(zpre if zpre is not None else out)))
+            del h1, h2, h3, h2_bits
         if save:
             S["heads"] = heads_saved
         return outs[0], outs[1], S
+
+    @staticmethod
+    def _masked_dgrad_1x1(dh3, w3_t, hs, relu):
+        bits = hs.pop("h2_bits", None)
+        if relu and bits is not None:
+            return ops.gemm_nt(dh3, w3_t, None, mask_bits=bits)
+        return ops.gemm_nt(dh3, w3_t, None, aux=(hs["h2"] if relu else None), mask_relu=relu)
 
     def _heads_backward_fullres(self, P, S, d_center, d_sdf, G, wgrad_lin, wgrad_c3):
         dt = self.dt
@@ -528,7 +548,7 @@
                                    G[f"{name}.{idx[3]}.weight"].view(w4.shape[0], -1), G[f"{name}.{idx[3]}.bias"])
             hs["h3"] = None
             wgrad_lin(f"{name}.{idx[2]}.weight", dh3, hs["h2"], f"{name}.{idx[2]}.bias")
-            dh2 = ops.gemm_nt(dh3, self._w(P, f"{name}.{idx[2]}.weight", "lin_t"), None, aux=(hs["h2"] if relu else None), mask_relu=relu)
+            dh2 = self._masked_dgrad_1x1(dh3, self._w(P, f"{name}.{idx[2]}.weight", "lin_t"), hs, relu)
             del dh3
             h1 = hs["h1"].view(B, H, W, 512)
             wgrad_c3(f"{name}.{idx[1]}.weight", dh2, h1, f"{name}.{idx[1]}.bias")
@@ -593,7 +613,7 @@
                                    G[f"{name}.{idx[3]}.weight"].view(w4.shape[0], -1), G[f"{name}.{idx[3]}.bias"])
             hs["h3"] = None
             wgrad_lin(f"{name}.{idx[2]}.weight", dh3, hs["h2"], f"{name}.{idx[2]}.bias")
-            dh2 = ops.gemm_nt(dh3, self._w(P, f"{name}.{idx[2]}.weight", "lin_t"), None, aux=(hs["h2"] if relu else None), mask_relu=relu)
+            dh2 = self._masked_dgrad_1x1(dh3, self._w(P, f"{name}.{idx[2]}.weight", "lin_t"), hs, relu)
             del dh3
             c1 = hs["h1"].shape[-1]
             wgrad_c3(f"{name}.{idx[1]}.weight", dh2, hs["h1"].view(B, H, W, c1), f"{name}.{idx[1]}.bias")
diff --git a/unmore_amd/ops.py b/unmore_amd/ops.py
--- a/unmore_amd/ops.py
+++ b/unmore_amd/ops.py
@@ -121,7 +121,7 @@
 def gemm_nt(A, B, bias=None, *, out=None, out2=None, aux=None, aux2=None, rowbias=None, rows_per_batch=0,
             act=L.ACT_NONE, mask_relu=False, mask_dgelu=False, c2_mode=0, out_f32=False,
             conv=0, M=None, lda=None, a_remap=None, c_remap=None, aux_mod=0, red_w=None, no_store=False, query_rowreduce=False,
-            query_splits=False):
+            query_splits=False, relu_bits_out=None, mask_bits=None, query_relu_bits=False):
     _need_gpu(A, B)
     dt = _DT[A.dtype]
     assert B.dtype == A.dtype
@@ -141,7 +141,7 @@
         d.lda = A2.stride(0) if lda is None else lda
         assert A2.stride(1) == 1
     odt = torch.float32 if out_f32 else A.dtype
-    skip_c = no_store or query_rowreduce or query_splits
+    skip_c = no_store or query_rowreduce or query_splits or query_relu_bits
     if out is None and not skip_c:
         out = torch.empty((M_, N), dtype=odt, device=A.device)
     assert skip_c or (out.dtype == odt and out.stride(-1) == 1)
@@ -179,6 +179,25 @@
     if c_remap is not None:
         d.c_rows_in, d.c_rows_out, d.c_row_off = c_remap
     d.aux_mod = aux_mod
+    if mask_bits is not None:
+        assert aux is None and not (mask_relu or mask_dgelu), "mask_bits is the one aux operand"
+        assert mask_bits.dtype == torch.uint8 and mask_bits.dim() == 2 and mask_bits.stride(1) == 1 and mask_bits.shape[0] >= M_
+        d.flags = flags | L.EPI_MASK_RELU_BITS
+        d.aux, d.ldaux = _p(mask_bits), mask_bits.stride(0)
+    if relu_bits_out is not None and relu_bits_out is not False:
+        assert not c2_mode, "the sign bits go out through C2"
+        if relu_bits_out is True:
+            relu_bits_out = None if query_relu_bits else torch.empty((M_, d.ldc // 8), dtype=torch.uint8, device=A.device)[:, :N // 8]
+        else:
+            assert relu_bits_out.dtype == torch.uint8 and relu_bits_out.dim() == 2 and relu_bits_out.stride(1) == 1
+            assert relu_bits_out.shape[0] >= M_ and relu_bits_out.shape[1] >= (N + 7) // 8
+        d.c2_mode = L.C2_RELU_BITS
+        if relu_bits_out is not None:
+            d.C2, d.ldc2 = _p(relu_bits_out), relu_bits_out.stride(0)
+        else:
+            d.C2, d.ldc2 = ctypes.c_void_p(16), d.ldc // 8
+    if query_relu_bits:
+        return bool(L.lib().umr_gemm_nt_relu_bits_ok(ctypes.byref(d)))
     if query_rowreduce:
         return bool(L.lib().umr_gemm_nt_rowreduce_ok(ctypes.byref(d)))
     if query_splits:
@@ -192,7 +211,20 @@
     L.check(_timed_call(d), "umr_gemm_nt")
     if red_w is not None:
         return out, partials
+    if d.c2_mode == L.C2_RELU_BITS:
+        return out, relu_bits_out
     return (out, out2) if c2_mode else out
+
+
+def relu_mask_bits_ok(M, N, K, dtype):
+    if dtype not in _DT or N % 8:
+        return False
+    d = L.GemmDesc()
+    d.A = d.B = d.C = d.aux = ctypes.c_void_p(16)
+    d.lda, d.ldb, d.ldc, d.ldaux = K, K, N, N // 8
+    d.M, d.N, d.K, d.dtype = M, N, K, _DT[dtype]
+    d.flags = L.EPI_MASK_RELU_BITS
+    return bool(L.lib().umr_gemm_nt_relu_bits_ok(ctypes.byref(d)))
 
 
 def split3(x, out=None, remap=None):
```

Measured after the change: 349.8, median of 6. No clear change (+0.2%).
